# XiaokunSun/SemanticHuman

Measured on AMD Instinct MI355X. Metric: training meshes/sec at 6890 verts, batch=64, higher is better.
Workload: dtype f32

## Files before the change

include/sh_kernels.h:

```cpp
#ifndef SH_KERNELS_H
#define SH_KERNELS_H

#include <stddef.h>
#include <stdint.h>

#ifdef __cplusplus
extern "C" {
#endif

typedef void* sh_stream_t;

#if defined(__GNUC__)
#define SH_API __attribute__((visibility("default")))
#else
#define SH_API
#endif

enum sh_status {
    SH_OK = 0,
    SH_ERR_INVALID_ARG = -1,
    SH_ERR_UNSUPPORTED = -2,
    SH_ERR_WORKSPACE = -3,
    SH_ERR_LAUNCH = -4
};
// ... 64 lines not shown
                       float* dpre, int64_t dp_sv, int64_t dp_sb, int B, int R, int C, int act, int zero_row, int n_layers,
                       const float* const* weight, float* const* weight_t, const int* S, const int* Cin, const int* Cout,
                       sh_stream_t stream);

SH_API int sh_spmm(const int32_t* rowptr, const int32_t* col, const float* val,
            const float* x, int64_t x_sv, int64_t x_sb,
            float* y, int64_t y_sv, int64_t y_sb,
            const float* yprev, int64_t yp_sv, int64_t yp_sb, int act_prev, int zero_row,
            int B, int rows, int C, sh_stream_t stream);

typedef struct sh_csr_ref { const int32_t* rowptr; const int32_t* col; const float* val; } sh_csr_ref;
typedef struct sh_stack_step {
    int kind;
    int param;
    const int32_t* table;
    const int32_t* table_t;
    int R, S, n_in, cin, cout, act, zero_row;
    int n1, n2;
    sh_csr_ref sum1, sum2;
    sh_csr_ref m, mt;
    int m_rows, m_cols;
    int extend;
    const int32_t* rag_rows;
    const int32_t* rag_pos;
    int rag_L;
    const int32_t* fg_rows; const uint32_t* fg_pos; const int32_t* fg_out; int fg_n, fg_L;
    const int32_t* bg_rows; const uint32_t* bg_pos; const int32_t* bg_out; int bg_n, bg_L;
} sh_stack_step;

enum sh_stack_form {
    SH_FORM_FWD_P3 = 1,
    SH_FORM_FWD_GRP = 2,
    SH_FORM_FWD_IMG = 4,
    SH_FORM_FWD_IMG_ONLY = 8,
    SH_FORM_BWD_GIMG = 16,
    SH_FORM_BWD_THIN = 32,
    SH_FORM_BWD_P3 = 64,
    SH_FORM_BWD_RAG = 128,
    SH_FORM_BWD_GRP = 256,
    SH_FORM_BWD_RIDE = 512,
    SH_FORM_BWD_PRESUM_IMG = 1024,
    SH_FORM_BWD_P3W = 2048,
    SH_FORM_BWD_YIMG = 4096,
    SH_FORM_BWD_IN_IMG_ONLY = 8192,
    SH_FORM_BWD_GRAD_IMG_ONLY = 16384
};
SH_API int sh_stack_plan_f32(int n_steps, const sh_stack_step* steps, int c0, int B, int x_layout, int mma_mode, int keep_fp32,
                             int need_x_grad, int* forms);

SH_API int sh_stack_forward(int n_steps, const sh_stack_step* steps, const float* x, int x_layout, int rows0, int c0, int B,
                            const float* const* weights, const float* const* biases, float* const* outs, int out_layout,
                            int mma_mode, void* const* planes, const void* const* wfrag3, int keep_fp32, sh_stream_t stream);

SH_API int sh_stack_backward(int n_steps, const sh_stack_step* steps, const float* x, int x_layout, int rows0, int c0, int B,
                             const float* const* acts, const float* g, int out_layout, const float* const* weights,
                             float* const* gin, float* dpre_last, float* const* weight_t, void* const* workspace,
                             const size_t* workspace_bytes, float* const* dW, float* const* dbias, int need_x_grad,
                             int mma_mode, void* const* gin_planes, void* dpre_last_planes, const void* const* wfrag3_t,
                             const void* const* in_planes, int acts_fp32, sh_stream_t stream);

SH_API size_t sh_linear_workspace(int M, int N, int K);
SH_API int sh_linear_fwd(const float* x, const float* weight, const float* bias, float* y, int M, int N, int K,
                  void* workspace, size_t workspace_bytes, int mma_mode, sh_stream_t stream);
SH_API int sh_linear_bwd_data(const float* dy, const float* weight, float* dx, int M, int N, int K,
                       void* workspace, size_t workspace_bytes, int mma_mode, sh_stream_t stream);
SH_API int sh_linear_bwd_wgt(const float* dy, const float* x, float* dW, float* dbias, int M, int N, int K,
                      void* workspace, size_t workspace_bytes, int mma_mode, sh_stream_t stream);
SH_API int sh_linear_bwd_wgt_adam_ok(int M, int N, int K);
SH_API int sh_linear_bwd_wgt_adam(const void* dy, int dy_dtype, const void* x, int x_dtype, float* weight, void* weight_bf16, float* exp_avg,
                           float* exp_avg_sq, const float* step, const float* lr, double beta1, double beta2, double eps,
                           double weight_decay, float* dbias, int M, int N, int K, int mma_mode, sh_stream_t stream);

SH_API int sh_grouped_linear_fwd(int G, const float* x, int64_t x_rs, const int64_t* x_off, const float* const* w,
                          const float* const* bias, float* y, int64_t y_rs, const int64_t* y_off, int M,
                          const int* N, const int* K, sh_stream_t stream);
SH_API int sh_grouped_linear_bwd_data(int G, const float* dy, int64_t y_rs, const int64_t* y_off, const float* const* w,
                               float* dx, int64_t x_rs, const int64_t* x_off, int M, const int* N, const int* K,
                               sh_stream_t stream);
SH_API int sh_grouped_linear_bwd_wgt(int G, const float* dy, int64_t y_rs, const int64_t* y_off, const float* x,
                              int64_t x_rs, const int64_t* x_off, float* const* dW, float* const* dbias, int M,
                              const int* N, const int* K, sh_stream_t stream);

SH_API size_t sh_reduce_workspace(void);

SH_API int sh_l1_loss_fwd(const float* a, const float* b, int64_t n, float* loss, void* workspace, sh_stream_t stream);
SH_API int sh_l1_loss_bwd(const float* a, const float* b, int64_t n, const float* gscale, float* grad_b, sh_stream_t stream);

SH_API int sh_vertex_l2(const float* a, const float* b, int B, int N1, int N, float scale, float* out,
                 void* workspace, sh_stream_t stream);

SH_API int sh_edge_ratio_loss_fwd(const float* x_hat, const float* x, const int32_t* faces, int B, int N1, int F,
                           float* loss, void* workspace, sh_stream_t stream);
SH_API int sh_edge_ratio_loss_bwd(const float* x_hat, const float* x, const int32_t* faces,
                           const int32_t* vptr, const int32_t* vcorner, int B, int N1, int F,
                           const float* gscale, float* grad, sh_stream_t stream);

SH_API size_t sh_recon_loss_workspace(void);
SH_API int sh_recon_loss_fwd(const float* x_hat, const float* x, const int32_t* faces, int B, int N1, int F, float edge_w,
                      float* total, float* parts, void* workspace, sh_stream_t stream);
SH_API int sh_recon_loss_bwd(const float* x_hat, const float* x, const int32_t* vptr, const int32_t* vnbr, int B, int N1, int F,
                      float edge_w, const float* gscale, float* grad, sh_stream_t stream);

SH_API int sh_part_pairdist_tile_rows(void);
SH_API int sh_part_pairdist_loss_fwd(const float* x_rec, const float* x_gt, const float* bone, const float* scale,
                              const int32_t* part_ptr, const int32_t* part_vert, const int32_t* tile_ptr,
                              const int32_t* flags, const float* w_part, int B, int N1, int P, int T, int max_part,
                              int w_mode, float w_threshold, int relat, float* loss, float* part_sum, float* part_cnt,
                              void* workspace, size_t workspace_bytes, sh_stream_t stream);
SH_API int sh_part_pairdist_loss_bwd(const float* x_rec, const float* x_gt, const float* bone, const float* scale,
                              const int32_t* part_ptr, const int32_t* part_vert, const int32_t* tile_ptr,
                              const int32_t* flags, const float* w_part, int B, int N1, int P, int T, int max_part,
                              int w_mode, float w_threshold, int relat, const float* part_cnt, const float* gscale,
                              float* grad, sh_stream_t stream);
SH_API int sh_part_pairdist_loss_fwd_grad(const float* x_rec, const float* x_gt, const float* bone, const float* scale,
                                   const int32_t* part_ptr, const int32_t* part_vert, const int32_t* tile_ptr, const int32_t* flags,
                                   const float* w_part, int B, int N1, int P, int T, int max_part, int w_mode, float w_threshold,
                                   int relat, float* loss, float* part_sum, float* part_cnt, float* grad_raw, void* workspace,
                                   size_t workspace_bytes, sh_stream_t stream);
SH_API int sh_part_pairdist_loss_bwd_scale(const float* grad_raw, const int32_t* part_ptr, const int32_t* part_vert,
                                   const float* w_part, const float* part_cnt, const float* gscale, int B, int N1, int P,
                                   int n_part_verts, float* grad, sh_stream_t stream);

SH_API int sh_measure_girth(const float* v, int64_t v_sb, const int32_t* ring_ptr, const int32_t* ring_a,
                     const int32_t* ring_b, const float* ring_f, int B, int P, float* girth, sh_stream_t stream);
SH_API int sh_bone_length(const float* kps, const int32_t* bones, int B, int K, int P, float* length, sh_stream_t stream);
SH_API int sh_measure_girth_bwd(const float* v, int64_t v_sb, const int32_t* ring_ptr, const int32_t* ring_a, const int32_t* ring_b,
                                const float* ring_f, const int32_t* pt_ring, const int32_t* vt_ptr, const int32_t* vt_pt,
                                const float* vt_w, int n_vt, const float* g_girth, int B, int P, int rows, float* g_v, sh_stream_t stream);
SH_API int sh_bone_length_bwd(const float* kps, const int32_t* bones, const int32_t* jt_ptr, const int32_t* jt_bone, const float* jt_w,
                              int n_jt, const float* g_len, int B, int K, int P, float* g_kps, sh_stream_t stream);
SH_API int sh_joint_regress_bwd(const float* g_kps, const float* J, int B, int N, int K, int rows, float* g_x, sh_stream_t stream);

SH_API int sh_nearest_points_chunks(int B, int nq, int nt);
SH_API size_t sh_nearest_points_workspace(int B, int nq, int nt, int chunks);
SH_API int sh_nearest_points(const float* q, int64_t q_sb, int nq, const int32_t* q_count, const float* t, int64_t t_sb, int nt,
                             const int32_t* t_count, const uint8_t* t_mask, int64_t mask_sb, int B, int chunks, int32_t* idx,
                             float* d2, void* workspace, size_t workspace_bytes, sh_stream_t stream);
SH_API int sh_chamfer_fwd(const float* d2_sm, int M, const int32_t* s_count, const float* d2_ms, int rows, int n,
                          const uint8_t* v_mask, int64_t mask_sb, float tau2, float w_ms, int B, float* loss, int32_t* counts,
                          sh_stream_t stream);
SH_API int sh_chamfer_bwd(const float* x, int64_t x_sb, int rows, int n, const float* s, int64_t s_sb, int M, const int32_t* s_count,
                          const int32_t* idx_sm, const float* d2_sm, const int32_t* idx_ms, const float* d2_ms, const uint8_t* v_mask,
                          int64_t mask_sb, const int32_t* counts, float tau2, float w_ms, const float* gL, int B, float* g_x,
                          sh_stream_t stream);

#define SH_SURFACE_MARGIN (1.0f + 0x1p-10f)
SH_API int sh_nearest_surface_chunks(int B, int nq, int nF);
SH_API size_t sh_nearest_surface_workspace(int B, int nq, int nF, int chunks);
SH_API int sh_nearest_surface(const float* q, int64_t q_sb, int nq, const int32_t* q_count, const float* x, int64_t x_sb, int n,
                              const int32_t* faces, int nF, const uint8_t* v_mask, int64_t mask_sb, const float* bound, int B,
                              int chunks, int cull, int32_t* face, float* d2, float* uv, uint64_t* stats, void* workspace,
                              size_t workspace_bytes, sh_stream_t stream);
SH_API int sh_chamfer_surface_bwd(const float* x, int64_t x_sb, int rows, int n, const float* s, int64_t s_sb, int M,
                                  const int32_t* s_count, const int32_t* faces, int nF, const int32_t* face, const float* d2,
                                  const float* uv, const int32_t* idx_ms, const float* d2_ms, const uint8_t* v_mask, int64_t mask_sb,
                                  const int32_t* counts, float tau2, float w_ms, const float* gL, int B, float* g_x,
                                  sh_stream_t stream);

enum sh_align_mode { SH_ALIGN_TRANSLATION = 0, SH_ALIGN_RIGID = 1, SH_ALIGN_SIMILARITY = 2 };
#define SH_ALIGN_RANGE 2048
#define SH_ALIGN_PARTIAL 19
#define SH_ALIGN_MOMENTS 20
#define SH_ALIGN_JACOBI_SWEEPS 12
SH_API int sh_align_ranges(int M, int n, float w_ms);
SH_API size_t sh_align_partials_bytes(int B, int M, int n, float w_ms);
SH_API int sh_align_moments(const float* s, int64_t s_sb, int M, const int32_t* s_count, const float* x, int64_t x_sb, int rows, int n,
                            const uint8_t* v_mask, int64_t mask_sb, const int32_t* idx_sm, const float* d2_sm, const int32_t* idx_ms,
                            const float* d2_ms, float tau2, float w_ms, int B, double* partials, size_t partials_bytes,
                            sh_stream_t stream);
SH_API int sh_align_solve(const double* partials, int M, int n, const int32_t* s_count, float w_ms, int mode, int B,
                          const float* pose_in, const float* scale_in, float* pose_out, float* scale_out, float* inc, double* mom,
                          sh_stream_t stream);
SH_API int sh_transform_points(const float* src, int64_t src_sb, int M, const int32_t* count, const float* pose, int B, float* dst,
                               sh_stream_t stream);

enum sh_norm_flags {
    SH_NORM_ZEROMEAN = 1, SH_NORM_ZEROROOT = 2, SH_NORM_ONELENGTH = 4, SH_NORM_SMALL = 8, SH_NORM_GASS = 16, SH_NORM_NORMAL = 32
};
SH_API int sh_dataset_normalize(const float* raw, float* out, int n, int N, int dummy_rows, unsigned flags,
                         const float* j_root, const float* mean, const float* stdv, const float* center,
                         const float* scale, sh_stream_t stream);
SH_API int sh_gather_meshes(const float* src, int64_t row_elems, const int64_t* idx, int b, float* out, sh_stream_t stream);

SH_API int sh_adam_step(int n_tensors, float* const* params, const float* const* grads, float* const* exp_avg,
                 float* const* exp_avg_sq, float* const* steps, const int64_t* numel, const float* lr,
                 double beta1, double beta2, double eps, double weight_decay, sh_stream_t stream);
SH_API int sh_adam_bump(int n_tensors, float* const* steps, sh_stream_t stream);

SH_API int sh_joint_regress(const float* x, int64_t x_bs, const float* J, int B, int N, int K, float* kps, sh_stream_t stream);
SH_API int sh_joint_l1_loss_fwd(const float* x, int64_t x_bs, const float* J, const int32_t* keep, const float* target, int B,
                                int N, int K, int Kk, float* kps, float* loss, sh_stream_t stream);
SH_API int sh_joint_l1_loss_bwd(const float* kps, const int32_t* keep, const float* target, const float* J, int B, int N1, int N,
                                int K, int Kk, const float* gscale, float* grad, sh_stream_t stream);
SH_API int sh_part_volume_loss_fwd(const float* x_rec, const float* x_gt, int64_t x_bs, const int32_t* faces,
                                   const int32_t* pf_ptr, const int32_t* pf, int B, int P, float* vol, float* loss,
                                   sh_stream_t stream);
SH_API int sh_part_volume_loss_bwd(const float* x_rec, int64_t x_bs, const int32_t* faces, const int32_t* face_slot,
                                   const int32_t* vptr, const int32_t* vcorner, const float* vol, int B, int P, int N1,
                                   const float* gscale, float* grad, sh_stream_t stream);
SH_API int sh_zpart_reg(const float* z, const float* measure, const int32_t* part_idx, const int32_t* measure_idx, int B, int P,
                        int L, int M, int n, int relat, float* loss, float* dz, const float* gscale, sh_stream_t stream);
SH_API int sh_kps2skl(const float* kps, int B, int J, const int32_t* i0, const int32_t* i1, const int32_t* i2, int n_bones, int mode,
                      float* out, sh_stream_t stream);
SH_API int sh_skl2kps(const float* skl, int B, int n_bones, int mode, const int32_t* head, const int32_t* tail, int n_joints,
                      const int32_t* keep, int n_keep, float* out, sh_stream_t stream);
SH_API int sh_weighted_sum(int n, const float* const* terms, const float* weights, float* out, const float* gscale, float* grads,
                           sh_stream_t stream);

enum sh_dtype { SH_DTYPE_F32 = 0, SH_DTYPE_BF16 = 1 };

SH_API size_t sh_conv_wfrag_bytes(int S, int Cg, int Nout);
SH_API int sh_conv_wfrag_prep_multi(int n_layers, const float* const* weight, void* const* wfrag, const int* S,
                                    const int* Cin, const int* Cout, const int* transpose, sh_stream_t stream);

SH_API int sh_spiral_conv_fwd_bf16(const void* x, int x_dtype, int64_t x_sv, int64_t x_sb, const int32_t* table,
                                   const void* wfrag, const float* bias, void* y, int y_dtype, int64_t y_sv, int64_t y_sb,
                                   int B, int R, int S, int Cin, int Cout, int act, int zero_row, sh_stream_t stream);
SH_API int sh_spiral_conv_bwd_data_bf16(const void* dpre, int dp_dtype, int64_t dp_sv, int64_t dp_sb,
                                        const int32_t* table_t, const void* wfrag_t, void* dx, int dx_dtype,
                                        int64_t dx_sv, int64_t dx_sb, const void* yprev, int64_t yp_sv, int64_t yp_sb,
                                        int act_prev, int zero_row, int B, int n_in, int S, int Cin, int Cout,
                                        sh_stream_t stream);

SH_API int sh_spiral_conv_bwd_wgt_thin_ok(int B, int n_in, int S, int Cin, int Cout, int path_dtype);
SH_API int sh_spiral_conv_bwd_wgt_thin(const float* dpre_ext, int64_t dp_sv, int64_t dp_sb, const void* x, int x_dtype, int64_t x_sv,
                                int64_t x_sb, const int32_t* table_t, void* workspace, size_t workspace_bytes,
                                const float* weight, void* dx, int64_t dx_sv, int64_t dx_sb, void* dx_planes, int act_prev,
                                int zero_prev, int B, int R, int n_in, int S, int Cin, int Cout, int path_dtype, sh_stream_t stream);

SH_API size_t sh_spiral_conv_bwd_wgt_workspace_bf16(int B, int R, int S, int Cin, int Cout);
SH_API int sh_spiral_conv_bwd_wgt_bf16(const void* dpre, int dp_dtype, int64_t dp_sv, int64_t dp_sb, const void* x, int x_dtype,
                                       int64_t x_sv, int64_t x_sb, const int32_t* table, void* workspace,
                                       size_t workspace_bytes, int B, int R, int S, int Cin, int Cout, sh_stream_t stream);
SH_API int sh_spiral_conv_bwd_wgt_reduce_multi_bf16(int n_layers, const void* const* workspaces, float* const* dW,
                                                    float* const* dbias, const int* B, const int* R, const int* S,
                                                    const int* Cin, const int* Cout, sh_stream_t stream);

SH_API size_t sh_linear_workspace_bf16(int M, int N, int K);
SH_API int sh_cast_f32_to_bf16(const float* src, void* dst, int64_t n, sh_stream_t stream);
SH_API int sh_linear_fwd_bf16(const void* x, int x_dtype, const void* weight_bf16, const float* bias, void* y, int y_dtype,
// ... 92 lines not shown
```

semantichuman_amd/_lib.py:

```python
from __future__ import annotations

import ctypes
import os
from ctypes import c_char_p, c_float, c_int, c_int64, c_size_t, c_void_p

_HERE = os.path.dirname(os.path.abspath(__file__))
LIB_PATH = os.environ.get("SH_KERNEL_LIB") or os.path.join(_HERE, "lib", "libsh_kernels.so")

ACT_IDS = {"identity": 0, "relu": 1, "elu": 2, "leaky_relu": 3, "sigmoid": 4, "tanh": 5}

_P, _I, _L = c_void_p, c_int, c_int64
SIGNATURES = {
    "sh_version": (c_int, []),
    "sh_last_error": (c_char_p, []),
    "sh_build_id": (c_char_p, []),
    "sh_clock_probe": (c_int, [_P, _I, _I, _P]),
    "sh_profile_enable": (c_int, [_I]),
    "sh_profile_count": (c_int, []),
    "sh_profile_get": (c_int, [_I, c_char_p, _I, ctypes.POINTER(c_float)]),
    "sh_spiral_conv_fwd": (c_int, [_P, _L, _L, _P, _P, _P, _P, _L, _L, _I, _I, _I, _I, _I, _I, _I, _I, _P]),
    "sh_spiral_conv_bwd_data": (c_int, [_P, _L, _L, _P, _P, _P, _L, _L, _P, _L, _L, _I, _I, _I, _I, _I, _I, _I, _I, _P]),
    "sh_spiral_conv_bwd_data_z": (c_int, [_P, _L, _L, _I, _P, _P, _P, _L, _L, _P, _L, _L, _I, _I, _I, _I, _I, _I, _I, _I, _P]),
    "sh_weight_transpose": (c_int, [_P, _P, _I, _I, _I, _P]),
    "sh_spiral_conv_bwd_wgt_workspace": (c_size_t, [_I, _I, _I, _I, _I]),
    "sh_spiral_conv_bwd_wgt": (c_int, [_P, _L, _L, _P, _L, _L, _P, _P, _P, _P, c_size_t, _I, _I, _I, _I, _I, _I, _P]),
    "sh_spiral_conv_bwd_wgt_presum": (c_int, [_P, _L, _L, _P, _L, _L, _P, _P, _P, _P, c_size_t, _P, _P, _P, _P, _P, _I, _I, _I, _I, _I, _I, _I, _P]),
    "sh_spiral_conv_bwd_wgt_reduce_multi": (c_int, [_I, _P, _P, _P, _P, _P, _P, _P, _P, _P]),
    "sh_weight_transpose_multi": (c_int, [_I, _P, _P, _P, _P, _P, _P]),
    "sh_act_backward": (c_int, [_P, _L, _L, _P, _L, _L, _P, _L, _L, _I, _I, _I, _I, _I, _P]),
    "sh_act_backward_tr": (c_int, [_P, _L, _L, _P, _L, _L, _P, _L, _L, _I, _I, _I, _I, _I, _I, _P, _P, _P, _P, _P, _P]),
    "sh_spmm": (c_int, [_P, _P, _P, _P, _L, _L, _P, _L, _L, _P, _L, _L, _I, _I, _I, _I, _I, _P]),
    "sh_stack_plan_f32": (c_int, [_I, _P, _I, _I, _I, _I, _I, _I, _P]),
    "sh_stack_forward": (c_int, [_I, _P, _P, _I, _I, _I, _I, _P, _P, _P, _I, _I, _P, _P, _I, _P]),
    "sh_stack_backward": (c_int, [_I, _P, _P, _I, _I, _I, _I, _P, _P, _I, _P, _P, _P, _P, _P, _P, _P, _P, _I, _I, _P, _P, _P, _P, _I, _P]),
    "sh_linear_workspace": (c_size_t, [_I, _I, _I]),
    "sh_linear_fwd": (c_int, [_P, _P, _P, _P, _I, _I, _I, _P, c_size_t, _I, _P]),
    "sh_linear_bwd_data": (c_int, [_P, _P, _P, _I, _I, _I, _P, c_size_t, _I, _P]),
    "sh_linear_bwd_wgt": (c_int, [_P, _P, _P, _P, _I, _I, _I, _P, c_size_t, _I, _P]),
    "sh_linear_bwd_wgt_adam_ok": (c_int, [_I, _I, _I]),
    "sh_linear_bwd_wgt_adam": (c_int, [_P, _I, _P, _I] + [_P] * 6 + [ctypes.c_double] * 4 + [_P, _I, _I, _I, _I, _P]),
    "sh_adam_bump": (c_int, [_I, _P, _P]),
    "sh_grouped_linear_fwd": (c_int, [_I, _P, _L, _P, _P, _P, _P, _L, _P, _I, _P, _P, _P]),
    "sh_grouped_linear_bwd_data": (c_int, [_I, _P, _L, _P, _P, _P, _L, _P, _I, _P, _P, _P]),
    "sh_grouped_linear_bwd_wgt": (c_int, [_I, _P, _L, _P, _P, _L, _P, _P, _P, _I, _P, _P, _P]),
    "sh_reduce_workspace": (c_size_t, []),
    "sh_l1_loss_fwd": (c_int, [_P, _P, _L, _P, _P, _P]),
    "sh_l1_loss_bwd": (c_int, [_P, _P, _L, _P, _P, _P]),
    "sh_vertex_l2": (c_int, [_P, _P, _I, _I, _I, c_float, _P, _P, _P]),
    "sh_edge_ratio_loss_fwd": (c_int, [_P, _P, _P, _I, _I, _I, _P, _P, _P]),
    "sh_edge_ratio_loss_bwd": (c_int, [_P, _P, _P, _P, _P, _I, _I, _I, _P, _P, _P]),
    "sh_spiral_conv_bwd_wgt_thin_ok": (c_int, [_I, _I, _I, _I, _I, _I]),
    "sh_spiral_conv_bwd_wgt_thin": (c_int, [_P, _L, _L, _P, _I, _L, _L, _P, _P, c_size_t, _P, _P, _L, _L, _P, _I, _I, _I, _I, _I, _I, _I, _I, _I, _P]),
    "sh_recon_loss_workspace": (c_size_t, []),
    "sh_recon_loss_fwd": (c_int, [_P, _P, _P, _I, _I, _I, c_float, _P, _P, _P, _P]),
    "sh_recon_loss_bwd": (c_int, [_P, _P, _P, _P, _I, _I, _I, c_float, _P, _P, _P]),
    "sh_part_pairdist_tile_rows": (c_int, []),
    "sh_part_pairdist_loss_fwd": (c_int, [_P] * 9 + [_I] * 6 + [c_float, _I, _P, _P, _P, _P, c_size_t, _P]),
    "sh_part_pairdist_loss_bwd": (c_int, [_P] * 9 + [_I] * 6 + [c_float, _I, _P, _P, _P, _P]),
    "sh_part_pairdist_loss_fwd_grad": (c_int, [_P] * 9 + [_I] * 6 + [c_float, _I, _P, _P, _P, _P, _P, c_size_t, _P]),
    "sh_part_pairdist_loss_bwd_scale": (c_int, [_P] * 6 + [_I] * 4 + [_P, _P]),
    "sh_measure_girth": (c_int, [_P, _L, _P, _P, _P, _P, _I, _I, _P, _P]),
    "sh_bone_length": (c_int, [_P, _P, _I, _I, _I, _P, _P]),
    "sh_measure_girth_bwd": (c_int, [_P, _L, _P, _P, _P, _P, _P, _P, _P, _P, _I, _P, _I, _I, _I, _P, _P]),
    "sh_bone_length_bwd": (c_int, [_P, _P, _P, _P, _P, _I, _P, _I, _I, _I, _P, _P]),
    "sh_joint_regress_bwd": (c_int, [_P, _P, _I, _I, _I, _I, _P, _P]),
    "sh_nearest_points_chunks": (c_int, [_I, _I, _I]),
    "sh_nearest_points_workspace": (c_size_t, [_I, _I, _I, _I]),
    "sh_nearest_points": (c_int, [_P, _L, _I, _P, _P, _L, _I, _P, _P, _L, _I, _I, _P, _P, _P, c_size_t, _P]),
    "sh_chamfer_fwd": (c_int, [_P, _I, _P, _P, _I, _I, _P, _L, c_float, c_float, _I, _P, _P, _P]),
    "sh_chamfer_bwd": (c_int, [_P, _L, _I, _I, _P, _L, _I, _P, _P, _P, _P, _P, _P, _L, _P, c_float, c_float, _P, _I, _P, _P]),
    "sh_nearest_surface_chunks": (c_int, [_I, _I, _I]),
    "sh_nearest_surface_workspace": (c_size_t, [_I, _I, _I, _I]),
    "sh_nearest_surface": (c_int, [_P, _L, _I, _P, _P, _L, _I, _P, _I, _P, _L, _P, _I, _I, _I, _P, _P, _P, _P, _P, c_size_t, _P]),
    "sh_chamfer_surface_bwd": (c_int, [_P, _L, _I, _I, _P, _L, _I, _P, _P, _I, _P, _P, _P, _P, _P, _P, _L, _P, c_float, c_float, _P, _I, _P, _P]),
    "sh_align_ranges": (c_int, [_I, _I, c_float]),
    "sh_align_partials_bytes": (c_size_t, [_I, _I, _I, c_float]),
    "sh_align_moments": (c_int, [_P, _L, _I, _P, _P, _L, _I, _I, _P, _L, _P, _P, _P, _P, c_float, c_float, _I, _P, c_size_t, _P]),
    "sh_align_solve": (c_int, [_P, _I, _I, _P, c_float, _I, _I, _P, _P, _P, _P, _P, _P, _P]),
    "sh_transform_points": (c_int, [_P, _L, _I, _P, _P, _I, _P, _P]),
    "sh_dataset_normalize": (c_int, [_P, _P, _I, _I, _I, ctypes.c_uint, _P, _P, _P, _P, _P, _P]),
    "sh_gather_meshes": (c_int, [_P, _L, _P, _I, _P, _P]),
    "sh_adam_step": (c_int, [_I, _P, _P, _P, _P, _P, _P, _P] + [ctypes.c_double] * 4 + [_P]),
    "sh_joint_regress": (c_int, [_P, _L, _P, _I, _I, _I, _P, _P]),
    "sh_joint_l1_loss_fwd": (c_int, [_P, _L, _P, _P, _P, _I, _I, _I, _I, _P, _P, _P]),
    "sh_joint_l1_loss_bwd": (c_int, [_P, _P, _P, _P, _I, _I, _I, _I, _I, _P, _P, _P]),
    "sh_part_volume_loss_fwd": (c_int, [_P, _P, _L, _P, _P, _P, _I, _I, _P, _P, _P]),
    "sh_part_volume_loss_bwd": (c_int, [_P, _L, _P, _P, _P, _P, _P, _I, _I, _I, _P, _P, _P]),
    "sh_zpart_reg": (c_int, [_P, _P, _P, _P, _I, _I, _I, _I, _I, _I, _P, _P, _P, _P]),
    "sh_kps2skl": (c_int, [_P, _I, _I, _P, _P, _P, _I, _I, _P, _P]),
    "sh_skl2kps": (c_int, [_P, _I, _I, _I, _P, _P, _I, _P, _I, _P, _P]),
    "sh_weighted_sum": (c_int, [_I, _P, _P, _P, _P, _P, _P]),
    "sh_conv_wfrag_bytes": (c_size_t, [_I, _I, _I]),
    "sh_conv_wfrag_prep_multi": (c_int, [_I, _P, _P, _P, _P, _P, _P, _P]),
    "sh_spiral_conv_fwd_bf16": (c_int, [_P, _I, _L, _L, _P, _P, _P, _P, _I, _L, _L, _I, _I, _I, _I, _I, _I, _I, _P]),
# ... 162 lines not shown
```

semantichuman_amd/csrc/adam.hip:

```cpp
#include "sh_bf16.h"
#include "sh_adam.h"

#include <math.h>

namespace {

constexpr int AT = 60;
constexpr int ACH = 4096;
constexpr int ANT = 256;

struct AdamArgs {
    float* p[AT];
    const float* g[AT];
    float* m[AT];
    float* v[AT];
    float* step[AT];
    __bf16* shadow[AT];
    long n[AT];
    int blk_start[AT + 1];
    int nt, nontemporal;
    const float* lr;
    double beta1, beta2;
    float w1, b2, w2, eps, wd;
};

__global__ __launch_bounds__(ANT) void adam_kernel(const AdamArgs a) {
    __shared__ float sh[2];
    int t = 0;
    while (t + 1 < a.nt && (int)blockIdx.x >= a.blk_start[t + 1]) ++t;
    const long base = (long)((int)blockIdx.x - a.blk_start[t]) * ACH;
    const long n = a.n[t];
    if (threadIdx.x == 0) {
        sh_adam_coeffs(a.beta1, a.beta2, a.step[t][0], a.lr[0], sh[0], sh[1]);
    }
    __syncthreads();
    const float step_size = sh[0], bc2_sqrt = sh[1];
    float* __restrict__ p = a.p[t];
    const float* __restrict__ g = a.g[t];
    float* __restrict__ m = a.m[t];
    float* __restrict__ v = a.v[t];
    __bf16* __restrict__ sw = a.shadow[t];
    const bool vec = ((reinterpret_cast<uintptr_t>(p) | reinterpret_cast<uintptr_t>(g) | reinterpret_cast<uintptr_t>(m) |
                       reinterpret_cast<uintptr_t>(v)) & 15) == 0;
    if (vec && base + ACH <= n) {
#pragma unroll
        for (int i = 0; i < ACH / (4 * ANT); ++i) {
            const long o = base + 4L * (threadIdx.x + i * ANT);
            f32x4 pp, mm, vv, gg;
            if (a.nontemporal) {
                pp = __builtin_nontemporal_load(reinterpret_cast<const f32x4*>(p + o));
                mm = __builtin_nontemporal_load(reinterpret_cast<const f32x4*>(m + o));
                vv = __builtin_nontemporal_load(reinterpret_cast<const f32x4*>(v + o));
                gg = __builtin_nontemporal_load(reinterpret_cast<const f32x4*>(g + o));
            } else {
                pp = *reinterpret_cast<f32x4*>(p + o); mm = *reinterpret_cast<f32x4*>(m + o); vv = *reinterpret_cast<f32x4*>(v + o);
                gg = *reinterpret_cast<const f32x4*>(g + o);
            }
#pragma unroll
            for (int j = 0; j < 4; ++j) {
                float p1 = pp[j], m1 = mm[j], v1 = vv[j];
                adam_update(p1, gg[j], m1, v1, a.w1, a.b2, a.w2, a.eps, a.wd, step_size, bc2_sqrt);
                pp[j] = p1; mm[j] = m1; vv[j] = v1;
            }
            if (sw) *reinterpret_cast<bf16x4*>(sw + o) = sh_to_bf16x4(pp);
            if (a.nontemporal) {
                __builtin_nontemporal_store(pp, reinterpret_cast<f32x4*>(p + o));
                __builtin_nontemporal_store(mm, reinterpret_cast<f32x4*>(m + o));
                __builtin_nontemporal_store(vv, reinterpret_cast<f32x4*>(v + o));
            } else {
                *reinterpret_cast<f32x4*>(p + o) = pp;
                *reinterpret_cast<f32x4*>(m + o) = mm;
                *reinterpret_cast<f32x4*>(v + o) = vv;
            }
        }
    } else {
        constexpr int PER = ACH / ANT;
        float pp[PER], mm[PER], vv[PER], gg[PER];
#pragma unroll
        for (int i = 0; i < PER; ++i) {
            const long o = base + threadIdx.x + (long)i * ANT;
            const bool ok = o < n;
            pp[i] = ok ? p[o] : 0.f; mm[i] = ok ? m[o] : 0.f; vv[i] = ok ? v[o] : 0.f; gg[i] = ok ? g[o] : 0.f;
        }
#pragma unroll
        for (int i = 0; i < PER; ++i) {
            const long o = base + threadIdx.x + (long)i * ANT;
            if (o < n) {
                adam_update(pp[i], gg[i], mm[i], vv[i], a.w1, a.b2, a.w2, a.eps, a.wd, step_size, bc2_sqrt);
                p[o] = pp[i]; m[o] = mm[i]; v[o] = vv[i];
                if (sw) sw[o] = (__bf16)pp[i];
            }
        }
    }
}

__global__ void adam_bump_kernel(const AdamArgs a) {
    if ((int)threadIdx.x < a.nt) a.step[threadIdx.x][0] += 1.f;
}

}

extern "C" {

static int adam_impl(int n_tensors, float* const* params, const float* const* grads, float* const* exp_avg, float* const* exp_avg_sq,
                     float* const* steps, void* const* shadow, const int64_t* numel, const float* lr, double beta1, double beta2,
                     double eps, double weight_decay, sh_stream_t stream) {
    SH_REQUIRE(n_tensors >= 0, SH_ERR_INVALID_ARG, "sh_adam_step: negative tensor count");
    if (n_tensors == 0) return SH_OK;
    SH_REQUIRE(params && grads && exp_avg && exp_avg_sq && steps && numel && lr, SH_ERR_INVALID_ARG, "sh_adam_step: null pointer");
    SH_REQUIRE(beta1 >= 0 && beta1 < 1 && beta2 >= 0 && beta2 < 1 && eps >= 0 && weight_decay >= 0, SH_ERR_INVALID_ARG,
               "sh_adam_step: hyper-parameter out of range");
    hipStream_t st = static_cast<hipStream_t>(stream);
    static const int nontemporal = sh_env_int("SH_ADAM_NT", 1, 0, 1);
    for (int t0 = 0; t0 < n_tensors; t0 += AT) {
        AdamArgs a{};
        a.nt = n_tensors - t0 < AT ? n_tensors - t0 : AT;
        long blocks = 0;
        for (int i = 0; i < a.nt; ++i) {
            const int k = t0 + i;
            SH_REQUIRE(steps[k] && numel[k] >= 0 && (numel[k] == 0 || (params[k] && grads[k] && exp_avg[k] && exp_avg_sq[k])), SH_ERR_INVALID_ARG,
                       "sh_adam_step: tensor %d has a null pointer or a negative element count", k);
            a.p[i] = params[k]; a.g[i] = grads[k]; a.m[i] = exp_avg[k]; a.v[i] = exp_avg_sq[k]; a.step[i] = steps[k];
            a.shadow[i] = shadow ? static_cast<__bf16*>(shadow[k]) : nullptr;
            SH_REQUIRE(!a.shadow[i] || (reinterpret_cast<uintptr_t>(a.shadow[i]) & 7) == 0, SH_ERR_INVALID_ARG, "sh_adam_step_bf16: shadow %d misaligned", k);
            a.n[i] = numel[k];
            a.blk_start[i] = (int)blocks;
            blocks += (numel[k] + ACH - 1) / ACH;
            SH_REQUIRE(blocks < (1L << 31), SH_ERR_UNSUPPORTED, "sh_adam_step: too many elements in one launch");
        }
        a.blk_start[a.nt] = (int)blocks;
        a.nontemporal = nontemporal;
        a.lr = lr; a.beta1 = beta1; a.beta2 = beta2;
        a.w1 = (float)(1.0 - beta1); a.b2 = (float)beta2; a.w2 = (float)(1.0 - beta2); a.eps = (float)eps; a.wd = (float)weight_decay;
        if (blocks > 0) {
            long numel_sum = 0;
            for (int i = 0; i < a.nt; ++i) numel_sum += a.n[i];
            ShProfScope ps(st, "adam_kernel|tensors=%d blocks=%ld numel=%ld", a.nt, blocks, numel_sum);
            SH_LAUNCH_PS(ps, adam_kernel, dim3((unsigned)blocks), dim3(ANT), 0, st, a);
        }
        hipLaunchKernelGGL(adam_bump_kernel, dim3(1), dim3(64), 0, st, a);
        SH_CHECK_LAUNCH("adam_step");
    }
    return SH_OK;
}

int sh_adam_bump(int n_tensors, float* const* steps, sh_stream_t stream) {
    SH_REQUIRE(n_tensors >= 0, SH_ERR_INVALID_ARG, "sh_adam_bump: negative tensor count");
    if (n_tensors == 0) return SH_OK;
    SH_REQUIRE(steps, SH_ERR_INVALID_ARG, "sh_adam_bump: null pointer");
    hipStream_t st = static_cast<hipStream_t>(stream);
    for (int t0 = 0; t0 < n_tensors; t0 += AT) {
        AdamArgs a{};
        a.nt = n_tensors - t0 < AT ? n_tensors - t0 : AT;
        for (int i = 0; i < a.nt; ++i) {
            SH_REQUIRE(steps[t0 + i], SH_ERR_INVALID_ARG, "sh_adam_bump: tensor %d has a null step pointer", t0 + i);
            a.step[i] = steps[t0 + i];
        }
        hipLaunchKernelGGL(adam_bump_kernel, dim3(1), dim3(64), 0, st, a);
        SH_CHECK_LAUNCH("adam_bump");
    }
    return SH_OK;
}

int sh_adam_step(int n_tensors, float* const* params, const float* const* grads, float* const* exp_avg, float* const* exp_avg_sq,
                 float* const* steps, const int64_t* numel, const float* lr, double beta1, double beta2, double eps,
                 double weight_decay, sh_stream_t stream) {
    return adam_impl(n_tensors, params, grads, exp_avg, exp_avg_sq, steps, nullptr, numel, lr, beta1, beta2, eps, weight_decay, stream);
}

int sh_adam_step_bf16(int n_tensors, float* const* params, const float* const* grads, float* const* exp_avg, float* const* exp_avg_sq,
                      float* const* steps, void* const* shadow_bf16, const int64_t* numel, const float* lr, double beta1, double beta2,
                      double eps, double weight_decay, sh_stream_t stream) {
    return adam_impl(n_tensors, params, grads, exp_avg, exp_avg_sq, steps, shadow_bf16, numel, lr, beta1, beta2, eps, weight_decay, stream);
}

}
```

semantichuman_amd/csrc/linear.hip:

```cpp
#include "sh_bf16.h"
#include "sh_adam.h"

#include <type_traits>

namespace {

constexpr int LT = 64;
constexpr int LK = 32;
constexpr int LTHREADS = 256;

struct SGParams {
    const float* a; long a_sm, a_sr;
    const float* b; long b_sn, b_sr;
    float* c; long c_sm, c_sn;
    const float* bias;
    float* slab;
    int M, N, R;
    int rchunk, nsplit, n_mtiles, n_ntiles;
    int a_mode, b_mode;
};

__device__ __forceinline__ void sg_load(const float* base, long s_row, long s_r, int mode, int row0, int nrows, int r0, int rend,
                                        int tid, f32x4 (&reg)[2], unsigned& mask) {
    mask = 0;
// ... 155 lines not shown
        for (; k + 48 < nsplit; k += 64) {
            const float a = slab[(long)k * mn + i], b = slab[(long)(k + 16) * mn + i];
            const float d = slab[(long)(k + 32) * mn + i], e = slab[(long)(k + 48) * mn + i];
            s += (a + b) + (d + e);
        }
        for (; k < nsplit; k += 16) s += slab[(long)k * mn + i];
    }
    red[ry][ox] = s;
    __syncthreads();
    if (ry == 0 && i < mn) {
        float t = 0.f;
#pragma unroll
        for (int k = 0; k < 16; ++k) t += red[k][ox];
        c[i] = t + (bias ? bias[i % N] : 0.f);
    }
}

__global__ __launch_bounds__(256) void colsum_kernel(const float* __restrict__ x, int M, int N, float* __restrict__ out) {
    const int n = blockIdx.x * 256 + threadIdx.x;
    if (n >= N) return;
    float s = 0.f;
    for (int m = 0; m < M; ++m) s += x[(long)m * N + n];
    out[n] = s;
}

#ifndef SH_LS_DEPTH
#define SH_LS_DEPTH 2
#endif
constexpr int LS_DEPTH = SH_LS_DEPTH;

template <int J, int D, class F>
__device__ __forceinline__ bool ls_run_steps(int s, int n, F&& f) {
    f(s + J, std::integral_constant<int, J>{});
    if constexpr (J + 1 < D) {
        if (s + J + 1 >= n) return true;
        return ls_run_steps<J + 1, D>(s, n, f);
    }
    return false;
}

struct LSParams {
    const float* a;
    const float* w;
    const float* bias;
    float* out;
    float* slab;
    float* dbias;
    int M, N, K;
    int range, nsplit, groups;
    float* am;
    float* av;
    __bf16* shadow;
    ShAdamHyper ad;
};

template <int MT>
__global__ __launch_bounds__(LTHREADS) void linear_fwd_stream_kernel(const LSParams p) {
    const int lane = threadIdx.x & 63, wave = sh_wave_id();
    const int item = sh_xcd_remap(blockIdx.x, gridDim.x) * 4 + wave;
    if (item >= p.groups * p.nsplit) return;
    const int ng = item % p.groups, sp = item / p.groups;
    const int n0 = ng * 64, k_begin = sp * p.range;
    const int nsteps = (min(p.K, k_begin + p.range) - k_begin) >> 4;
    const int lr = lane & 15, kq = lane >> 4;
    const float* xrow[MT];
    const float* wrow[4];
#pragma unroll
    for (int mt = 0; mt < MT; ++mt) xrow[mt] = p.a + (long)min(16 * mt + lr, p.M - 1) * p.K + k_begin + 4 * kq;
#pragma unroll
    for (int nt = 0; nt < 4; ++nt) wrow[nt] = p.w + (long)(n0 + 16 * nt + lr) * p.K + k_begin + 4 * kq;
    f32x4 xa[LS_DEPTH][MT], wb[LS_DEPTH][4], acc[MT][4];
#pragma unroll
    for (int mt = 0; mt < MT; ++mt)
#pragma unroll
        for (int nt = 0; nt < 4; ++nt) acc[mt][nt] = (f32x4){0.f, 0.f, 0.f, 0.f};
    auto load = [&](int s, f32x4 (&x4)[MT], f32x4 (&w4)[4]) {
        const int off = 16 * (s < nsteps ? s : nsteps - 1);
#pragma unroll
        for (int mt = 0; mt < MT; ++mt) x4[mt] = *reinterpret_cast<const f32x4*>(xrow[mt] + off);
#pragma unroll
        for (int nt = 0; nt < 4; ++nt) w4[nt] = __builtin_nontemporal_load(reinterpret_cast<const f32x4*>(wrow[nt] + off));
    };
    auto mma = [&](const f32x4 (&x4)[MT], const f32x4 (&w4)[4]) {
#pragma unroll
        for (int t = 0; t < 4; ++t)
#pragma unroll
            for (int nt = 0; nt < 4; ++nt)
#pragma unroll
                for (int mt = 0; mt < MT; ++mt) acc[mt][nt] = __builtin_amdgcn_mfma_f32_16x16x4f32(w4[nt][t], x4[mt][t], acc[mt][nt], 0, 0, 0);
    };
    auto step = [&](int s, auto J) {
        constexpr int j = decltype(J)::value;
        load(s + LS_DEPTH - 1, xa[(j + LS_DEPTH - 1) % LS_DEPTH], wb[(j + LS_DEPTH - 1) % LS_DEPTH]);
        __builtin_amdgcn_sched_barrier(0);
        mma(xa[j], wb[j]);
    };
    if (nsteps > 0) {
#pragma unroll
        for (int d = 0; d < LS_DEPTH - 1; ++d) load(d, xa[d], wb[d]);
        for (int s = 0; s < nsteps; s += LS_DEPTH)
            if (ls_run_steps<0, LS_DEPTH>(s, nsteps, step)) break;
    }
#pragma unroll
    for (int mt = 0; mt < MT; ++mt) {
        const int m = 16 * mt + lr;
        if (m >= p.M) continue;
#pragma unroll
// ... 178 lines not shown
        }
    }
}

template <int MT>
__global__ __launch_bounds__(LTHREADS) void linear_bwd_data_stream_kernel(const LSParams p) {
    const int lane = threadIdx.x & 63, wave = sh_wave_id();
    const int item = sh_xcd_remap(blockIdx.x, gridDim.x) * 4 + wave;
    if (item >= p.groups * p.nsplit) return;
    const int kg = item % p.groups, sp = item / p.groups;
    const int k0 = kg * 64, n_begin = sp * p.range;
    const int nsteps = (min(p.N, n_begin + p.range) - n_begin) >> 4;
    const int la = lane & 15, rr = lane >> 4;
    const float* drow[MT];
#pragma unroll
    for (int mt = 0; mt < MT; ++mt) drow[mt] = p.a + (long)min(16 * mt + la, p.M - 1) * p.N + n_begin + 4 * rr;
    const float* wbase = p.w + (long)(n_begin + 4 * rr) * p.K + k0 + 4 * la;
    f32x4 dq[LS_DEPTH][MT], wq[LS_DEPTH][4], acc[4][MT];
#pragma unroll
    for (int t = 0; t < 4; ++t)
#pragma unroll
        for (int mt = 0; mt < MT; ++mt) acc[t][mt] = (f32x4){0.f, 0.f, 0.f, 0.f};
    auto load = [&](int s, f32x4 (&d4)[MT], f32x4 (&w4)[4]) {
        const int nb = 16 * (s < nsteps ? s : nsteps - 1);
#pragma unroll
        for (int mt = 0; mt < MT; ++mt) d4[mt] = *reinterpret_cast<const f32x4*>(drow[mt] + nb);
#pragma unroll
        for (int e = 0; e < 4; ++e) w4[e] = __builtin_nontemporal_load(reinterpret_cast<const f32x4*>(wbase + (long)(nb + e) * p.K));
    };
    auto mma = [&](const f32x4 (&d4)[MT], const f32x4 (&w4)[4]) {
#pragma unroll
        for (int e = 0; e < 4; ++e)
#pragma unroll
            for (int t = 0; t < 4; ++t)
#pragma unroll
                for (int mt = 0; mt < MT; ++mt) acc[t][mt] = __builtin_amdgcn_mfma_f32_16x16x4f32(w4[e][t], d4[mt][e], acc[t][mt], 0, 0, 0);
    };
    auto step = [&](int s, auto J) {
        constexpr int j = decltype(J)::value;
        load(s + LS_DEPTH - 1, dq[(j + LS_DEPTH - 1) % LS_DEPTH], wq[(j + LS_DEPTH - 1) % LS_DEPTH]);
        __builtin_amdgcn_sched_barrier(0);
        mma(dq[j], wq[j]);
    };
    if (nsteps > 0) {
#pragma unroll
        for (int d = 0; d < LS_DEPTH - 1; ++d) load(d, dq[d], wq[d]);
        for (int s = 0; s < nsteps; s += LS_DEPTH)
            if (ls_run_steps<0, LS_DEPTH>(s, nsteps, step)) break;
    }
#pragma unroll
    for (int mt = 0; mt < MT; ++mt) {
        const int m = 16 * mt + la;
        if (m >= p.M) continue;
        float* dst = (p.nsplit > 1 ? p.slab + ((long)sp * p.M + m) * p.K : p.out + (long)m * p.K) + k0 + 16 * rr;
#pragma unroll
        for (int jj = 0; jj < 4; ++jj)
            *reinterpret_cast<f32x4*>(dst + 4 * jj) = (f32x4){acc[0][mt][jj], acc[1][mt][jj], acc[2][mt][jj], acc[3][mt][jj]};
    }
}

template <int MT>
__global__ __launch_bounds__(LTHREADS) void linear_bwd_data_x3_kernel(const LSParams p) {
    const int lane = threadIdx.x & 63, wave = sh_wave_id();
    const int item = sh_xcd_remap(blockIdx.x, gridDim.x) * 4 + wave;
    if (item >= p.groups * p.nsplit) return;
    const int kg = item % p.groups, sp = item / p.groups;
    const int k0 = kg * 64, n_begin = sp * p.range;
    const int nsteps = (min(p.N, n_begin + p.range) - n_begin) >> 5;
    const int la = lane & 15, rr = lane >> 4;
    const float* drow[MT];
#pragma unroll
    for (int mt = 0; mt < MT; ++mt) drow[mt] = p.a + (long)min(16 * mt + la, p.M - 1) * p.N + n_begin + 4 * rr;
    const float* wbase = p.w + (long)(n_begin + 4 * rr) * p.K + k0 + 4 * la;
    f32x4 dq[2][MT][2], wq[2][8], acc[4][MT];
#pragma unroll
    for (int t = 0; t < 4; ++t)
#pragma unroll
        for (int mt = 0; mt < MT; ++mt) acc[t][mt] = (f32x4){0.f, 0.f, 0.f, 0.f};
    auto load = [&](int s, f32x4 (&d4)[MT][2], f32x4 (&w4)[8]) {
        const int nb = 32 * (s < nsteps ? s : nsteps - 1);
#pragma unroll
        for (int mt = 0; mt < MT; ++mt) {
            d4[mt][0] = *reinterpret_cast<const f32x4*>(drow[mt] + nb);
            d4[mt][1] = *reinterpret_cast<const f32x4*>(drow[mt] + nb + 16);
        }
#pragma unroll
        for (int j = 0; j < 8; ++j)
            w4[j] = __builtin_nontemporal_load(reinterpret_cast<const f32x4*>(wbase + (long)(nb + (j & 3) + 16 * (j >> 2)) * p.K));
    };
    auto mma = [&](const f32x4 (&d4)[MT][2], const f32x4 (&w4)[8]) {
        LinX3 ds[MT];
#pragma unroll
        for (int mt = 0; mt < MT; ++mt) ds[mt] = lin_split(d4[mt][0], d4[mt][1]);
#pragma unroll
        for (int t = 0; t < 4; ++t) {
            const LinX3 ws = lin_split((f32x4){w4[0][t], w4[1][t], w4[2][t], w4[3][t]}, (f32x4){w4[4][t], w4[5][t], w4[6][t], w4[7][t]});
#pragma unroll
            for (int mt = 0; mt < MT; ++mt) acc[t][mt] = lin_x3_mma(ws.h, ws.m, ws.l, ds[mt].h, ds[mt].m, ds[mt].l, acc[t][mt]);
        }
    };
    if (nsteps > 0) {
        load(0, dq[0], wq[0]);
        for (int s = 0; s < nsteps; s += 2) {
            load(s + 1, dq[1], wq[1]);
            __builtin_amdgcn_sched_barrier(0);
            mma(dq[0], wq[0]);
            if (s + 1 >= nsteps) break;
            load(s + 2, dq[0], wq[0]);
            __builtin_amdgcn_sched_barrier(0);
            mma(dq[1], wq[1]);
        }
    }
#pragma unroll
    for (int mt = 0; mt < MT; ++mt) {
        const int m = 16 * mt + la;
        if (m >= p.M) continue;
        float* dst = (p.nsplit > 1 ? p.slab + ((long)sp * p.M + m) * p.K : p.out + (long)m * p.K) + k0 + 16 * rr;
#pragma unroll
        for (int jj = 0; jj < 4; ++jj)
            *reinterpret_cast<f32x4*>(dst + 4 * jj) = (f32x4){acc[0][mt][jj], acc[1][mt][jj], acc[2][mt][jj], acc[3][mt][jj]};
    }
}

__global__ __launch_bounds__(LTHREADS) void linear_bwd_wgt_stream_kernel(const LSParams p) {
    const int lane = threadIdx.x & 63, wave = sh_wave_id();
    const int item = sh_xcd_remap(blockIdx.x, gridDim.x) * 4 + wave;
    const int ktiles = p.K >> 6;
    if (item >= (p.N >> 6) * ktiles) return;
    const int kt = item % ktiles, ntile = item / ktiles;
    const int n0 = ntile * 64, k0 = kt * 64;
    const int la = lane & 15, rr = lane >> 4;
    const int nsteps = (p.M + 3) >> 2;
    f32x4 acc[4][4];
#pragma unroll
    for (int a = 0; a < 4; ++a)
#pragma unroll
        for (int b = 0; b < 4; ++b) acc[a][b] = (f32x4){0.f, 0.f, 0.f, 0.f};
    f32x4 dq[4], xq[4];
    auto load = [&](int s, f32x4& d4, f32x4& x4) {
        s = s < nsteps ? s : nsteps - 1;
        const int m = 4 * s + rr;
        const int mc = m < p.M ? m : p.M - 1;
        d4 = *reinterpret_cast<const f32x4*>(p.a + (long)mc * p.N + n0 + 4 * la);
        x4 = *reinterpret_cast<const f32x4*>(p.w + (long)mc * p.K + k0 + 4 * la);
        if (m >= p.M) d4 = (f32x4){0.f, 0.f, 0.f, 0.f};
    };
    const bool own_bias = kt == 0 && p.dbias != nullptr;
    f32x4 bsum = {0.f, 0.f, 0.f, 0.f};
    auto mma = [&](const f32x4& d4, const f32x4& x4) {
#pragma unroll
        for (int tn = 0; tn < 4; ++tn)
#pragma unroll
            for (int tk = 0; tk < 4; ++tk) acc[tn][tk] = __builtin_amdgcn_mfma_f32_16x16x4f32(d4[tn], x4[tk], acc[tn][tk], 0, 0, 0);
        if (own_bias) bsum += d4;
    };
    load(0, dq[0], xq[0]); load(1, dq[1], xq[1]); load(2, dq[2], xq[2]);
    for (int s = 0; s < nsteps; s += 4) {
        load(s + 3, dq[3], xq[3]); __builtin_amdgcn_sched_barrier(0); mma(dq[0], xq[0]);
        if (s + 1 >= nsteps) break;
        load(s + 4, dq[0], xq[0]); __builtin_amdgcn_sched_barrier(0); mma(dq[1], xq[1]);
        if (s + 2 >= nsteps) break;
        load(s + 5, dq[1], xq[1]); __builtin_amdgcn_sched_barrier(0); mma(dq[2], xq[2]);
        if (s + 3 >= nsteps) break;
        load(s + 6, dq[2], xq[2]); __builtin_amdgcn_sched_barrier(0); mma(dq[3], xq[3]);
    }
    if (own_bias) {
#pragma unroll
        for (int j = 0; j < 4; ++j) {
            float v = bsum[j];
// ... 357 lines not shown
                if (hipFuncSetAttribute(reinterpret_cast<const void*>(linear_fwd_wide_x3_kernel), hipFuncAttributeMaxDynamicSharedMemorySize,
                                        160 * 1024) != hipSuccess) {
                    (void)hipGetLastError();
                    sh_set_error("linear_fwd: cannot raise the dynamic LDS limit to %zu bytes", smem);
                    return SH_ERR_LAUNCH;
                }
                attr_set = true;
            }
            LSParams s{};
            s.a = x; s.w = weight; s.bias = bias; s.out = y; s.M = M; s.N = N; s.K = K;
            ShProfScope ps(st, "linear_fwd_wide_x3_kernel|M=%d N=%d K=%d", M, N, K);
            SH_LAUNCH_PS(ps, linear_fwd_wide_x3_kernel, dim3(N / 64), dim3(LFW_WAVES * 64), smem, st, s);
            SH_CHECK_LAUNCH("linear_fwd_wide");
            return SH_OK;
        }
    }
    {
        const bool x3 = lin_x3(mma_mode) && K % 32 == 0 && (N / 64) % 4 == 0;
        static const int chunk_on = sh_env_int("SH_LIN_CHUNKED", 1, 0, 1);
        const LSPlan pl = plan_stream(M, N, K, x3 ? 32 : 16, chunk_on && M > 64);
        if (pl.ok && aligned16(x, weight, y) && (!bias || (reinterpret_cast<uintptr_t>(bias) & 15) == 0)) {
            LSParams s{};
            s.a = x; s.w = weight; s.bias = bias; s.out = y; s.M = M; s.N = N; s.K = K;
            return run_stream<true>(s, pl, N, workspace, workspace_bytes, static_cast<hipStream_t>(stream), "linear_fwd", x3);
        }
    }
    SGParams p{};
    p.a = x; p.a_sm = K; p.a_sr = 1;
    p.b = weight; p.b_sn = K; p.b_sr = 1;
    p.c = y; p.c_sm = N; p.c_sn = 1; p.bias = bias;
    p.M = M; p.N = N; p.R = K;
    return run_gemm(p, workspace, workspace_bytes, static_cast<hipStream_t>(stream), "linear_fwd");
}

int sh_linear_bwd_data(const float* dy, const float* weight, float* dx, int M, int N, int K, void* workspace,
                       size_t workspace_bytes, int mma_mode, sh_stream_t stream) {
    SH_REQUIRE(dy && weight && dx && M > 0 && N > 0 && K > 0, SH_ERR_INVALID_ARG, "sh_linear_bwd_data: bad argument");
    SH_REQUIRE(sh_mma_mode_valid(mma_mode), SH_ERR_INVALID_ARG, "sh_linear_bwd_data: unknown mma_mode %d", mma_mode);
    {
        const bool x3 = lin_x3(mma_mode) && N % 32 == 0;
        const LSPlan pl = plan_stream(M, K, N, x3 ? 32 : 16);
        if (pl.ok && aligned16(dy, weight, dx)) {
            LSParams s{};
            s.a = dy; s.w = weight; s.bias = nullptr; s.out = dx; s.M = M; s.N = N; s.K = K;
            return run_stream<false>(s, pl, K, workspace, workspace_bytes, static_cast<hipStream_t>(stream), "linear_bwd_data", x3);
        }
    }
    SGParams p{};
    p.a = dy; p.a_sm = N; p.a_sr = 1;
    p.b = weight; p.b_sn = 1; p.b_sr = K;
    p.c = dx; p.c_sm = K; p.c_sn = 1; p.bias = nullptr;
    p.M = M; p.N = K; p.R = N;
    return run_gemm(p, workspace, workspace_bytes, static_cast<hipStream_t>(stream), "linear_bwd_data");
}

static bool wgt_dma_attr() {
    static bool attr_set = false;
    if (!attr_set) {
        for (const void* k : {reinterpret_cast<const void*>(linear_bwd_wgt_dma_kernel<false>), reinterpret_cast<const void*>(linear_bwd_wgt_dma_kernel<true>),
                              reinterpret_cast<const void*>(linear_bwd_wgt_dma_kernel<false, true>), reinterpret_cast<const void*>(linear_bwd_wgt_dma_kernel<true, true>),
                              reinterpret_cast<const void*>(linear_bwd_wgt_dma_kernel<false, true, true, false>),
                              reinterpret_cast<const void*>(linear_bwd_wgt_dma_kernel<false, true, false, true>),
                              reinterpret_cast<const void*>(linear_bwd_wgt_dma_kernel<false, true, true, true>)})
            if (hipFuncSetAttribute(k, hipFuncAttributeMaxDynamicSharedMemorySize, 160 * 1024) != hipSuccess) {
                (void)hipGetLastError();
                sh_set_error("linear_bwd_wgt: cannot raise the dynamic LDS limit to %d bytes", LWD_LDS);
                return false;
            }
        attr_set = true;
    }
    return true;
}

int sh_linear_bwd_wgt(const float* dy, const float* x, float* dW, float* dbias, int M, int N, int K, void* workspace,
                      size_t workspace_bytes, int mma_mode, sh_stream_t stream) {
    SH_REQUIRE(dy && x && dW && M > 0 && N > 0 && K > 0, SH_ERR_INVALID_ARG, "sh_linear_bwd_wgt: bad argument");
    SH_REQUIRE(sh_mma_mode_valid(mma_mode), SH_ERR_INVALID_ARG, "sh_linear_bwd_wgt: unknown mma_mode %d", mma_mode);
    hipStream_t st = static_cast<hipStream_t>(stream);
    static const int stream_on = sh_env_int("SH_LIN_STREAM", 1, 0, 1);
    if (stream_on && M <= 64 && N % 64 == 0 && K % 64 == 0 && aligned16(dy, x, dW)) {
        LSParams s{};
        s.a = dy; s.w = x; s.out = dW; s.M = M; s.N = N; s.K = K;
        s.dbias = (dbias && (reinterpret_cast<uintptr_t>(dbias) & 15) == 0) ? dbias : nullptr;
        const int items = (N / 64) * (K / 64);
        static const int dma_on = sh_env_int("SH_LIN_WGT_DMA", 1, 0, 1);
        if (dma_on) {
            if (!wgt_dma_attr()) return SH_ERR_LAUNCH;
            const int wgs = (N / 64) * sh_cdiv(K / 64, 4);
            if (lin_x3(mma_mode)) {
                ShProfScope ps(st, "linear_bwd_wgt_x3_kernel|M=%d N=%d K=%d", M, N, K);
                SH_LAUNCH_PS(ps, linear_bwd_wgt_dma_kernel<true>, dim3(wgs), dim3(LTHREADS), LWD_LDS, st, s);
            } else {
                ShProfScope ps(st, "linear_bwd_wgt_dma_kernel|M=%d N=%d K=%d", M, N, K);
                SH_LAUNCH_PS(ps, linear_bwd_wgt_dma_kernel<false>, dim3(wgs), dim3(LTHREADS), LWD_LDS, st, s);
            }
        } else {
            ShProfScope ps(st, "linear_bwd_wgt_stream_kernel|M=%d N=%d K=%d", M, N, K);
            SH_LAUNCH_PS(ps, linear_bwd_wgt_stream_kernel, dim3(sh_cdiv(items, 4)), dim3(LTHREADS), 0, st, s);
        }
        if (dbias && !s.dbias) hipLaunchKernelGGL(colsum_kernel, dim3((unsigned)sh_cdiv(N, 256)), dim3(256), 0, st, dy, M, N, dbias);
        SH_CHECK_LAUNCH("linear_bwd_wgt");
        return SH_OK;
    }
    SGParams p{};
    p.a = dy; p.a_sm = 1; p.a_sr = N;
    p.b = x; p.b_sn = 1; p.b_sr = K;
// ... 60 lines not shown
```

semantichuman_amd/csrc/spmm_loss.hip:

```cpp
#include "sh_bf16.h"

namespace {

constexpr int RED_BLOCKS = 2048;

template <bool VEC, bool P3 = false>
__global__ __launch_bounds__(256) void spmm_kernel(const int* __restrict__ rowptr, const int* __restrict__ col,
                                                   const float* __restrict__ val, const float* __restrict__ x, long x_sv, long x_sb,
                                                   float* __restrict__ y, long y_sv, long y_sb, const float* __restrict__ yprev,
                                                   long yp_sv, long yp_sb, int act, int zero_row, int B, int rows, int C,
                                                   char* __restrict__ img = nullptr, long img_vb = 0, long img_bgb = 0) {
    const int CW = VEC ? C >> 2 : C;
    const int per_row = B * CW;
    const int parts = (per_row + 255) >> 8;
    const long items = (long)rows * parts;
    for (long it = blockIdx.x; it < items; it += gridDim.x) {
        const int r = (int)(it / parts), part = (int)(it - (long)r * parts);
        const int e0 = rowptr[r], e1 = rowptr[r + 1];
        const bool zero = r == zero_row;
        for (int j = part * 256 + threadIdx.x; j < per_row && j < (part + 1) * 256; j += 256) {
            const int b = j / CW, cw = j - b * CW;
            const int co = VEC ? 4 * cw : cw;
            const long xo = (long)b * x_sb + co;
            const long yo = (long)r * y_sv + (long)b * y_sb + co;
// ... 189 lines not shown

__global__ void edge_loss_partial_kernel(const float* __restrict__ xh, const float* __restrict__ x, const int* __restrict__ faces,
                                         int B, int N1, int F, float* __restrict__ part) {
    __shared__ float red[16];
    float s = 0.f;
    const long n = (long)B * F;
    for (long i = (long)blockIdx.x * blockDim.x + threadIdx.x; i < n; i += (long)gridDim.x * blockDim.x) {
        const long bb = i / F;
        const int f = (int)(i - bb * F);
        const int ia = faces[3 * f], ib = faces[3 * f + 1], ic = faces[3 * f + 2];
        const float* ph = xh + bb * N1 * 3;
        const float* pg = x + bb * N1 * 3;
        s += fabsf(edge_len(ph, ia, ib) / (edge_len(pg, ia, ib) + 0.00001f) - 1.f);
        s += fabsf(edge_len(ph, ib, ic) / (edge_len(pg, ib, ic) + 0.00001f) - 1.f);
        s += fabsf(edge_len(ph, ia, ic) / (edge_len(pg, ia, ic) + 0.00001f) - 1.f);
    }
    const float t = block_sum(s, red);
    if (threadIdx.x == 0) part[blockIdx.x] = t;
}

__device__ __forceinline__ void edge_grad(const float* ph, const float* pg, int i, int j, float* g) {
    const float dx = ph[3 * i] - ph[3 * j], dy = ph[3 * i + 1] - ph[3 * j + 1], dz = ph[3 * i + 2] - ph[3 * j + 2];
    const float len = sqrtf(dx * dx + dy * dy + dz * dz);
    const float t = edge_len(pg, i, j) + 0.00001f;
    const float r = len / t - 1.f;
    const float sg = r > 0.f ? 1.f : (r < 0.f ? -1.f : 0.f);
    if (len > 0.f) {
        const float k = sg / (len * t);
        g[0] += k * dx; g[1] += k * dy; g[2] += k * dz;
    }
}

__global__ void edge_loss_bwd_kernel(const float* __restrict__ xh, const float* __restrict__ x, const int* __restrict__ faces,
                                     const int* __restrict__ vptr, const int* __restrict__ vcorner, int B, int N1, int F,
                                     const float* __restrict__ gscale, float* __restrict__ grad) {
    const float sc = gscale[0] / ((float)B * (float)F);
    const long n = (long)B * N1;
    for (long i = (long)blockIdx.x * blockDim.x + threadIdx.x; i < n; i += (long)gridDim.x * blockDim.x) {
        const long bb = i / N1;
        const int v = (int)(i - bb * N1);
        const float* ph = xh + bb * N1 * 3;
        const float* pg = x + bb * N1 * 3;
        float g[3] = {0.f, 0.f, 0.f};
        for (int e = vptr[v]; e < vptr[v + 1]; ++e) {
            const int c = vcorner[e], f = c / 3, kx = c - 3 * f;
            const int o1 = faces[3 * f + (kx + 1) % 3], o2 = faces[3 * f + (kx + 2) % 3];
            edge_grad(ph, pg, v, o1, g);
            edge_grad(ph, pg, v, o2, g);
        }
        grad[i * 3] = sc * g[0]; grad[i * 3 + 1] = sc * g[1]; grad[i * 3 + 2] = sc * g[2];
    }
}

__global__ void recon_partial_kernel(const float* __restrict__ xh, const float* __restrict__ x, const int* __restrict__ faces,
                                     int B, int N1, int F, float* __restrict__ part) {
    __shared__ float red[16];
    float s = 0.f;
    const long n = (long)B * N1 * 3;
    for (long i = (long)blockIdx.x * blockDim.x + threadIdx.x; i < n; i += (long)gridDim.x * blockDim.x) s += fabsf(x[i] - xh[i]);
    const float t1 = block_sum(s, red);
    if (threadIdx.x == 0) part[blockIdx.x] = t1;
    __syncthreads();
    s = 0.f;
    const long nf = (long)B * F;
    for (long i = (long)blockIdx.x * blockDim.x + threadIdx.x; i < nf; i += (long)gridDim.x * blockDim.x) {
        const long bb = i / F;
        const int f = (int)(i - bb * F);
        const I3 fc = *reinterpret_cast<const I3*>(faces + 3 * f);
        const float* ph = xh + bb * N1 * 3;
        const float* pg = x + bb * N1 * 3;
        const P3 ha = ld3(ph, fc.a), hb = ld3(ph, fc.b), hc = ld3(ph, fc.c), ga = ld3(pg, fc.a), gb = ld3(pg, fc.b), gc = ld3(pg, fc.c);
        s += fabsf(edge_len3(ha, hb) / (edge_len3(ga, gb) + 0.00001f) - 1.f);
        s += fabsf(edge_len3(hb, hc) / (edge_len3(gb, gc) + 0.00001f) - 1.f);
        s += fabsf(edge_len3(ha, hc) / (edge_len3(ga, gc) + 0.00001f) - 1.f);
    }
    const float t2 = block_sum(s, red);
    if (threadIdx.x == 0) part[RED_BLOCKS + blockIdx.x] = t2;
}

__global__ void recon_final_kernel(const float* __restrict__ part, int np, double scale1, double scale2, float w, float* __restrict__ total,
                                   float* __restrict__ parts) {
    __shared__ double red[2][256];
    double s1 = 0.0, s2 = 0.0;
    for (int i = threadIdx.x; i < np; i += 256) { s1 += (double)part[i]; s2 += (double)part[RED_BLOCKS + i]; }
    red[0][threadIdx.x] = s1; red[1][threadIdx.x] = s2;
    __syncthreads();
    for (int o = 128; o > 0; o >>= 1) {
        if ((int)threadIdx.x < o) { red[0][threadIdx.x] += red[0][threadIdx.x + o]; red[1][threadIdx.x] += red[1][threadIdx.x + o]; }
        __syncthreads();
    }
    if (threadIdx.x == 0) {
        const float rec = (float)(red[0][0] * scale1), edge = (float)(red[1][0] * scale2);
        total[0] = rec + w * edge; parts[0] = rec; parts[1] = edge;
    }
}

__global__ __launch_bounds__(256) void recon_bwd_kernel(const float* __restrict__ xh, const float* __restrict__ x, const int* __restrict__ vptr,
                                                        const int* __restrict__ vnbr, int B, int N1, int F, float w,
                                                        const float* __restrict__ gscale, float* __restrict__ grad) {
    const float g0 = gscale[0];
    const float s1 = g0 / ((float)B * (float)N1 * 3.f), s2 = g0 * w / ((float)B * (float)F);
    const long n = (long)B * N1;
    for (long i = (long)blockIdx.x * blockDim.x + threadIdx.x; i < n; i += (long)gridDim.x * blockDim.x) {
        const long bb = i / N1;
        const int v = (int)(i - bb * N1);
        const float* ph = xh + bb * N1 * 3;
        const float* pg = x + bb * N1 * 3;
        const int p0 = 2 * vptr[v], p1 = 2 * vptr[v + 1];
        const P3 hv = ld3(ph, v), gv = ld3(pg, v);
        float g[3] = {0.f, 0.f, 0.f};
        for (int e = p0; e < p1; e += 4) {
            int o[4];
            P3 ho[4], go[4];
#pragma unroll
            for (int k = 0; k < 4; ++k) o[k] = vnbr[e + k < p1 ? e + k : p1 - 1];
#pragma unroll
            for (int k = 0; k < 4; ++k) { ho[k] = ld3(ph, o[k]); go[k] = ld3(pg, o[k]); }
#pragma unroll
            for (int k = 0; k < 4; ++k)
                if (e + k < p1) edge_grad3(hv, gv, ho[k], go[k], g);
        }
        const float df[3] = {hv.x - gv.x, hv.y - gv.y, hv.z - gv.z};
        P3 o3;
        o3.x = s2 * g[0] + (df[0] > 0.f ? s1 : (df[0] < 0.f ? -s1 : 0.f));
        o3.y = s2 * g[1] + (df[1] > 0.f ? s1 : (df[1] < 0.f ? -s1 : 0.f));
        o3.z = s2 * g[2] + (df[2] > 0.f ? s1 : (df[2] < 0.f ? -s1 : 0.f));
        *reinterpret_cast<P3*>(grad + i * 3) = o3;
    }
}

inline int grid_for(long n, int per_block) {
    long g = (n + per_block - 1) / per_block;
    if (g < 1) g = 1;
    return (int)(g < 2048 ? g : 2048);
}

}

extern "C" {

int sh_spmm(const int32_t* rowptr, const int32_t* col, const float* val, const float* x, int64_t x_sv, int64_t x_sb, float* y,
            int64_t y_sv, int64_t y_sb, const float* yprev, int64_t yp_sv, int64_t yp_sb, int act_prev, int zero_row, int B,
            int rows, int C, sh_stream_t stream) {
    return sh_spmm_p3(rowptr, col, val, x, x_sv, x_sb, y, y_sv, y_sb, nullptr, yprev, yp_sv, yp_sb, act_prev, zero_row, B, rows, C, stream);
}

int sh_spmm_p3(const int32_t* rowptr, const int32_t* col, const float* val, const float* x, int64_t x_sv, int64_t x_sb, float* y,
               int64_t y_sv, int64_t y_sb, void* y_planes, const float* yprev, int64_t yp_sv, int64_t yp_sb, int act_prev, int zero_row,
               int B, int rows, int C, sh_stream_t stream) {
    SH_REQUIRE(rowptr && col && val && x && (y || y_planes), SH_ERR_INVALID_ARG, "sh_spmm: null pointer");
    SH_REQUIRE(B > 0 && rows > 0 && C > 0, SH_ERR_INVALID_ARG, "sh_spmm: non-positive size");
    SH_REQUIRE(act_prev >= SH_ACT_IDENTITY && act_prev <= SH_ACT_TANH, SH_ERR_INVALID_ARG, "sh_spmm: unknown activation %d", act_prev);
    const bool vec = (C % 4 == 0) && (x_sv % 4 == 0) && (x_sb % 4 == 0) && (y_sv % 4 == 0) && (y_sb % 4 == 0) &&
                     ((reinterpret_cast<uintptr_t>(x) | reinterpret_cast<uintptr_t>(y)) % 16 == 0) &&
                     (!yprev || (yp_sv % 4 == 0 && yp_sb % 4 == 0 && reinterpret_cast<uintptr_t>(yprev) % 16 == 0));
    static const int grid_cap = sh_env_int("SH_SPMM_GRID", 4096, 64, 1 << 20);
    const long items = (long)rows * (((long)B * (vec ? C / 4 : C) + 255) / 256);
    const int grid = (int)(items < grid_cap ? items : grid_cap);
    hipStream_t st = static_cast<hipStream_t>(stream);
    if (y_planes) {
        SH_REQUIRE(vec && y_sb == C && y_sv == (int64_t)B * C && sh_p3_bytes(1, B, C) && (reinterpret_cast<uintptr_t>(y_planes) & 15) == 0, SH_ERR_UNSUPPORTED,
                   "sh_spmm_p3: B=%d C=%d has no plane image (vertex-major y; B %% 16 == 0; C == 16 or C %% 32 == 0; 16-byte aligned tensors)", B, C);
        const long bgb = C == 16 ? 1536 : (long)(C / 32) * 3072;
        ShProfScope ps(st, "spmm_kernel<true, p3>|rows=%d B=%d C=%d f32=%d", rows, B, C, y ? 1 : 0);
        static const int x8_mode = sh_env_int("SH_SPMM_P3X8", 1, 0, 2);
        const bool x8 = x8_mode == 2 || (x8_mode == 1 && (C >= 128 || (C == 64 && B >= 256)));
        if (x8) {
            const long items8 = (long)rows * (((long)B * (C / 8) + 255) / 256);
            const int grid8 = (int)(items8 < grid_cap ? items8 : grid_cap);
            SH_LAUNCH_PS(ps, spmm_p3x8_kernel, dim3(grid8), dim3(256), 0, st, rowptr, col, val, x, x_sv, x_sb, y, y_sv, y_sb, yprev, yp_sv, yp_sb,
                         act_prev, zero_row, B, rows, C, static_cast<char*>(y_planes), bgb * (B / 16), bgb);
        } else
        SH_LAUNCH_PS(ps, (spmm_kernel<true, true>), dim3(grid), dim3(256), 0, st, rowptr, col, val, x, x_sv, x_sb, y, y_sv, y_sb,
                     yprev, yp_sv, yp_sb, act_prev, zero_row, B, rows, C, static_cast<char*>(y_planes), bgb * (B / 16), bgb);
        SH_CHECK_LAUNCH("spmm");
        return SH_OK;
    }
    ShProfScope ps(st, "spmm_kernel<%s>|rows=%d B=%d C=%d", vec ? "true" : "false", rows, B, C);
    if (vec)
        SH_LAUNCH_PS(ps, (spmm_kernel<true, false>), dim3(grid), dim3(256), 0, st, rowptr, col, val, x, x_sv, x_sb, y, y_sv, y_sb,
// ... 32 lines not shown
                 sh_stream_t stream) {
    SH_REQUIRE(a && b && out && workspace && B > 0 && N > 0 && N1 >= N, SH_ERR_INVALID_ARG, "sh_vertex_l2: bad argument");
    hipStream_t st = static_cast<hipStream_t>(stream);
    float* part = static_cast<float*>(workspace);
    const long n = (long)B * N;
    const int nb = grid_for(n, 1024) < RED_BLOCKS ? grid_for(n, 1024) : RED_BLOCKS;
    hipLaunchKernelGGL(vertex_l2_partial_kernel, dim3(nb), dim3(256), 0, st, a, b, B, N1, N, scale, part);
    hipLaunchKernelGGL(final_sum_kernel, dim3(1), dim3(256), 0, st, part, nb, 1.0 / (double)n, out);
    SH_CHECK_LAUNCH("vertex_l2");
    return SH_OK;
}

int sh_edge_ratio_loss_fwd(const float* x_hat, const float* x, const int32_t* faces, int B, int N1, int F, float* loss,
                           void* workspace, sh_stream_t stream) {
    SH_REQUIRE(x_hat && x && faces && loss && workspace && B > 0 && N1 > 0 && F > 0, SH_ERR_INVALID_ARG,
               "sh_edge_ratio_loss_fwd: bad argument");
    hipStream_t st = static_cast<hipStream_t>(stream);
    float* part = static_cast<float*>(workspace);
    const long n = (long)B * F;
    const int nb = grid_for(n, 1024) < RED_BLOCKS ? grid_for(n, 1024) : RED_BLOCKS;
    hipLaunchKernelGGL(edge_loss_partial_kernel, dim3(nb), dim3(256), 0, st, x_hat, x, faces, B, N1, F, part);
    hipLaunchKernelGGL(final_sum_kernel, dim3(1), dim3(256), 0, st, part, nb, 1.0 / (double)n, loss);
    SH_CHECK_LAUNCH("edge_ratio_loss_fwd");
    return SH_OK;
}

size_t sh_recon_loss_workspace(void) { return (size_t)2 * RED_BLOCKS * sizeof(float); }

int sh_recon_loss_fwd(const float* x_hat, const float* x, const int32_t* faces, int B, int N1, int F, float edge_w, float* total,
                      float* parts, void* workspace, sh_stream_t stream) {
    SH_REQUIRE(x_hat && x && faces && total && parts && workspace && B > 0 && N1 > 0 && F > 0, SH_ERR_INVALID_ARG,
               "sh_recon_loss_fwd: bad argument");
    hipStream_t st = static_cast<hipStream_t>(stream);
    float* part = static_cast<float*>(workspace);
    const long n = (long)B * N1 * 3;
    const int nb = grid_for(n, 1024) < RED_BLOCKS ? grid_for(n, 1024) : RED_BLOCKS;
    hipLaunchKernelGGL(recon_partial_kernel, dim3(nb), dim3(256), 0, st, x_hat, x, faces, B, N1, F, part);
    hipLaunchKernelGGL(recon_final_kernel, dim3(1), dim3(256), 0, st, part, nb, 1.0 / (double)n, 1.0 / ((double)B * F), edge_w, total, parts);
    SH_CHECK_LAUNCH("recon_loss_fwd");
    return SH_OK;
}

int sh_recon_loss_bwd(const float* x_hat, const float* x, const int32_t* vptr, const int32_t* vnbr, int B, int N1, int F, float edge_w,
                      const float* gscale, float* grad, sh_stream_t stream) {
    SH_REQUIRE(x_hat && x && vptr && vnbr && gscale && grad && B > 0 && N1 > 0 && F > 0, SH_ERR_INVALID_ARG,
               "sh_recon_loss_bwd: bad argument");
    const long n = (long)B * N1;
    hipLaunchKernelGGL(recon_bwd_kernel, dim3(grid_for(n, 256)), dim3(256), 0, static_cast<hipStream_t>(stream), x_hat, x, vptr, vnbr, B,
                       N1, F, edge_w, gscale, grad);
    SH_CHECK_LAUNCH("recon_loss_bwd");
    return SH_OK;
}

int sh_edge_ratio_loss_bwd(const float* x_hat, const float* x, const int32_t* faces, const int32_t* vptr, const int32_t* vcorner,
                           int B, int N1, int F, const float* gscale, float* grad, sh_stream_t stream) {
    SH_REQUIRE(x_hat && x && faces && vptr && vcorner && gscale && grad && B > 0 && N1 > 0 && F > 0, SH_ERR_INVALID_ARG,
               "sh_edge_ratio_loss_bwd: bad argument");
    const long n = (long)B * N1;
    hipLaunchKernelGGL(edge_loss_bwd_kernel, dim3(grid_for(n, 256)), dim3(256), 0, static_cast<hipStream_t>(stream), x_hat, x, faces,
                       vptr, vcorner, B, N1, F, gscale, grad);
    SH_CHECK_LAUNCH("edge_ratio_loss_bwd");
    return SH_OK;
}

}
```

semantichuman_amd/csrc/stack_exec.hip:

```cpp
#include "sh_common.h"

namespace {

struct Lay { long sv, sb; };
inline Lay lay(int layout, int rows, int B, int C) {
    return layout == 0 ? Lay{(long)B * C, (long)C} : Lay{(long)C, (long)rows * C};
}
inline int out_rows(const sh_stack_step& s) { return s.kind == 0 ? s.R : s.m_rows; }
inline bool is_last_step(int i, int n) { return i == n - 1; }
inline int in_rows(const sh_stack_step& s) { return s.kind == 0 ? s.n_in : s.m_cols; }

int check_tensor_sizes(int n, const sh_stack_step* st, int rows0, int c0, int B, const char* what) {
    long rows = rows0;
    int c = c0;
    for (int i = 0; i <= n; ++i) {
        long extra = 0;
        if (i > 0 && st[i - 1].kind == 0) extra = (long)st[i - 1].n1 + st[i - 1].n2;
        SH_REQUIRE((rows + extra) * (long)B * c < (1L << 32), SH_ERR_UNSUPPORTED,
                   "%s: the tensor %s step %d has %ld rows x %d batch entries x %d channels >= 2^32 elements - split the batch", what,
                   i < n ? "entering" : "leaving", i < n ? i : n - 1, rows + extra, B, c);
        if (i == n) break;
        rows = st[i].kind == 0 ? st[i].R : (st[i].extend ? (long)st[i].m_cols + st[i].m_rows : st[i].m_rows);
        if (st[i].kind == 0) c = st[i].cout;
    }
// ... 128 lines not shown
    SH_REQUIRE(sh_mma_mode_valid(mma_mode), SH_ERR_INVALID_ARG, "sh_stack_forward: unknown mma_mode %d", mma_mode);
    SH_REQUIRE(keep_fp32 >= 0 && keep_fp32 <= 2, SH_ERR_INVALID_ARG, "sh_stack_forward: keep_fp32 = %d (0, 1 or 2)", keep_fp32);
    Forms f[64];
    plan_f32(n_steps, steps, B, x_layout, mma_mode == SH_MMA_PLANES3 && planes && wfrag3, keep_fp32, false, f);
    for (int i = 0; i < n_steps; ++i) {
        SH_REQUIRE(outs[i], SH_ERR_INVALID_ARG, "sh_stack_forward: no output buffer for step %d", i);
        SH_REQUIRE(!f[i].f_img || planes[i], SH_ERR_INVALID_ARG, "sh_stack_forward: step %d writes the image of its output: planes[%d] is NULL", i, i);
        SH_REQUIRE(!f[i].f_p3 || wfrag3[i], SH_ERR_INVALID_ARG, "sh_stack_forward: step %d runs on planes: wfrag3[%d] is NULL", i, i);
    }
    const float* cur = x;
    Lay cl = lay(x_layout, rows0, B, c0);
    int c = c0;
    for (int i = 0; i < n_steps; ++i) {
        const sh_stack_step& s = steps[i];
        const Forms& q = f[i];
        const int co = s.kind == 0 ? s.cout : c;
        const Lay ol = lay(i == n_steps - 1 ? out_layout : 0, out_rows(s), B, co);
        void* img = q.f_img ? planes[i] : nullptr;
        if (s.kind == 0) {
            const float* bias = biases ? biases[s.param] : nullptr;
            float* y = q.f_img_only ? nullptr : outs[i];
            if (q.f_grp)
                rc = sh_spiral_conv_p3_grp(planes[i - 1], s.fg_rows, s.fg_pos, s.fg_out, s.fg_n, s.fg_L, wfrag3[i], bias, y, ol.sv, ol.sb, img, nullptr,
                                           0, 0, nullptr, s.act, s.zero_row, 0, B, s.R, s.S, s.cin, s.cout, stream);
            else if (q.f_p3)
                rc = sh_spiral_conv_fwd_p3(planes[i - 1], s.table, wfrag3[i], bias, y, ol.sv, ol.sb, img, B, s.R, s.S, s.cin, s.cout, s.act,
                                           s.zero_row, stream);
            else
                rc = sh_spiral_conv_fwd_img(cur, cl.sv, cl.sb, s.table, weights[s.param], bias, outs[i], ol.sv, ol.sb, img, B, s.R, s.S, s.cin,
                                            s.cout, s.act, s.zero_row, mma_mode, stream);
        } else if (s.extend) {
            SH_REQUIRE(i > 0 && !is_last_step(i, n_steps) && outs[i] == outs[i - 1] && cl.sb == c, SH_ERR_INVALID_ARG,
                       "sh_stack_forward: step %d appends to its input, which must be the vertex-major output buffer of step %d", i, i - 1);
            SH_REQUIRE(!img || planes[i] == planes[i - 1], SH_ERR_INVALID_ARG, "sh_stack_forward: step %d appends to its input: same image buffer", i);
            float* dst = q.f_img_only ? nullptr : outs[i] + (long)s.m_cols * cl.sv;
            rc = sh_spmm_p3(s.m.rowptr, s.m.col, s.m.val, cur, cl.sv, cl.sb, dst, cl.sv, cl.sb,
                            img ? static_cast<char*>(img) + sh_p3_bytes(s.m_cols, B, c) : nullptr, nullptr, 0, 0, 0, -1, B, s.m_rows, c, stream);
        } else {
            rc = sh_spmm_p3(s.m.rowptr, s.m.col, s.m.val, cur, cl.sv, cl.sb, q.f_img_only ? nullptr : outs[i], ol.sv, ol.sb, img, nullptr, 0, 0, 0,
                            -1, B, s.m_rows, c, stream);
        }
        if (rc != SH_OK) return rc;
        cur = outs[i]; cl = ol; c = co;
    }
    return SH_OK;
}

int sh_stack_backward(int n_steps, const sh_stack_step* steps, const float* x, int x_layout, int rows0, int c0, int B,
                      const float* const* acts, const float* g, int out_layout, const float* const* weights,
                      float* const* gin, float* dpre_last, float* const* weight_t, void* const* workspace,
                      const size_t* workspace_bytes, float* const* dW, float* const* dbias, int need_x_grad, int mma_mode,
                      void* const* gin_planes, void* dpre_last_planes, const void* const* wfrag3_t, const void* const* in_planes,
                      int acts_fp32, sh_stream_t stream) {
    int rc = check_steps(n_steps, steps, c0, "sh_stack_backward");
    if (rc != SH_OK) return rc;
    if (B > 0 && (rc = check_tensor_sizes(n_steps, steps, rows0, c0, B, "sh_stack_backward")) != SH_OK) return rc;
    SH_REQUIRE(x && acts && g && weights && gin && dW && B > 0, SH_ERR_INVALID_ARG, "sh_stack_backward: null pointer or empty batch");
    SH_REQUIRE(n_steps <= 64, SH_ERR_UNSUPPORTED, "sh_stack_backward: more than 64 steps");
    SH_REQUIRE(sh_mma_mode_valid(mma_mode), SH_ERR_INVALID_ARG, "sh_stack_backward: unknown mma_mode %d", mma_mode);
    const bool planes3 = mma_mode == SH_MMA_PLANES3 && gin_planes && wfrag3_t;
    SH_REQUIRE(acts_fp32 == 1 || (acts_fp32 == 2 && planes3 && in_planes), SH_ERR_INVALID_ARG,
               "sh_stack_backward: acts_fp32 = %d (1: every activation has its fp32 rows; 2, three-plane form with gin_planes, wfrag3_t and "
               "in_planes: the forward pass ran with keep_fp32 == 2)", acts_fp32);
    const int last = n_steps - 1;
    Forms f[64];
    plan_f32(n_steps, steps, B, x_layout, planes3, acts_fp32, need_x_grad != 0, f);
    for (int i = 0; i < n_steps; ++i) {
        SH_REQUIRE(!f[i].b_gimg || (wfrag3_t[i] && (i == last ? dpre_last_planes : gin_planes[i + 1])), SH_ERR_INVALID_ARG,
                   "sh_stack_backward: step %d runs backward-data on planes: wfrag3_t[%d] and the image buffer of its gradient (%s) are required",
                   i, i, i == last ? "dpre_last_planes" : "gin_planes[i + 1]");
        SH_REQUIRE(!in_planes || !(f[i].b_p3w || f[i].b_yimg) || in_planes[i], SH_ERR_INVALID_ARG,
                   "sh_stack_backward: step %d reads the image of its input: in_planes[%d] is NULL", i, i);
    }
    const Switches& sw = switches();
    int cin_of[64];
    {
        int c = c0;
        for (int i = 0; i < n_steps; ++i) { cin_of[i] = c; if (steps[i].kind == 0) c = steps[i].cout; }
    }
    const float* tr_w[32]; float* tr_wt[32]; int tr_S[32], tr_Ci[32], tr_Co[32];
    int n_tr = 0;
    for (int i = 0; i < n_steps; ++i) {
        if (steps[i].kind != 0 || !(i > 0 || need_x_grad) || (f[i].b_gimg && !f[i].b_thin)) continue;
        SH_REQUIRE(weight_t && weight_t[i], SH_ERR_INVALID_ARG, "sh_stack_backward: no weight_t buffer for step %d", i);
        SH_REQUIRE(n_tr < 32, SH_ERR_UNSUPPORTED, "sh_stack_backward: more than 32 conv steps");
        tr_w[n_tr] = weights[steps[i].param]; tr_wt[n_tr] = weight_t[i]; tr_S[n_tr] = steps[i].S; tr_Ci[n_tr] = steps[i].cin; tr_Co[n_tr] = steps[i].cout;
        ++n_tr;
    }
    if (n_tr && !(sw.tr_ride && steps[last].kind == 0)) {
        rc = sh_weight_transpose_multi(n_tr, tr_w, tr_wt, tr_S, tr_Ci, tr_Co, stream);
        if (rc != SH_OK) return rc;
        n_tr = 0;
    }
    const float* cur; Lay cl;
    void* cur_img = nullptr;
    bool cur_img_done = false;
    {
        const sh_stack_step& s = steps[last];
        if (s.kind == 0) {
            SH_REQUIRE(dpre_last, SH_ERR_INVALID_ARG, "sh_stack_backward: no dpre_last buffer");
            const Lay ol = lay(out_layout, s.R, B, s.cout), dl = lay(0, 0, B, s.cout);
            cur_img = f[last].b_gimg ? dpre_last_planes : nullptr;
            const bool img_in = cur_img && s.cout % 4 == 0 && s.cout > 8;
            rc = sh_act_backward_tr_img(g, ol.sv, ol.sb, acts[last], ol.sv, ol.sb, dpre_last, dl.sv, dl.sb, img_in ? cur_img : nullptr, B, s.R,
                                        s.cout, s.act, s.zero_row, n_tr, tr_w, tr_wt, tr_S, tr_Ci, tr_Co, stream);
            if (rc != SH_OK) return rc;
            cur = dpre_last; cl = dl;
            cur_img_done = img_in;
        } else {
            cur = g; cl = lay(out_layout, s.m_rows, B, cin_of[last]);
        }
    }
    const void* job_ws[64]; float* job_dW[64]; float* job_db[64]; int jB[64], jR[64], jS[64], jCi[64], jCo[64], jK[64];
    int njobs = 0;
    for (int i = last; i >= 0; --i) {
        const sh_stack_step& s = steps[i];
        const Forms& q = f[i];
        const bool want_in = i > 0 || need_x_grad;
        const float* inp = i == 0 ? x : acts[i - 1];
        const Lay il = i == 0 ? lay(x_layout, rows0, B, c0) : lay(0, 0, B, cin_of[i]);
        float* gi = want_in ? gin[i] : nullptr;
        SH_REQUIRE(!want_in || gi, SH_ERR_INVALID_ARG, "sh_stack_backward: no gradient buffer for the input of step %d", i);
        const Lay gl = il;
        const float* yprev = nullptr; Lay yl{0, 0}; int act_prev = 0, zero_prev = -1;
        if (i > 0 && steps[i - 1].kind == 0) {
            yprev = acts[i - 1]; yl = lay(0, 0, B, steps[i - 1].cout); act_prev = steps[i - 1].act; zero_prev = steps[i - 1].zero_row;
        }
        void* gi_img = (i > 0 && steps[i - 1].kind == 0 && f[i - 1].b_gimg) ? gin_planes[i] : nullptr;
        float* gi_f = (gi_img && f[i - 1].b_grad_img_only) ? nullptr : gi;
        bool gi_img_done = false;
        if (s.kind == 0) {
            SH_REQUIRE(workspace && workspace[i], SH_ERR_INVALID_ARG, "sh_stack_backward: no workspace for step %d", i);
            const bool wgrad = dW[s.param] != nullptr;
            SH_REQUIRE(wgrad || !dbias || !dbias[s.param], SH_ERR_INVALID_ARG,
                       "sh_stack_backward: parameter %d has a dbias buffer but no dW buffer", s.param);
            const bool thin = wgrad && q.b_thin;
            const int bd = thin ? BD_F32 : q.b_data;
            const bool p3 = bd != BD_F32, rag = bd >= BD_RAG;
            const bool ride = wgrad && q.b_ride;
            char* pimg0 = (p3 && q.b_presum_img) ? static_cast<char*>(cur_img) : nullptr;
            float* mut0 = const_cast<float*>(cur);
            if (ride && s.n1 && s.n2) {
                rc = sh_spmm_p3(s.sum1.rowptr, s.sum1.col, s.sum1.val, cur, cl.sv, cl.sb, mut0 + (long)s.R * cl.sv, cl.sv, cl.sb,
                                pimg0 ? pimg0 + sh_p3_bytes(s.R, B, s.cout) : nullptr, nullptr, 0, 0, 0, -1, B, s.n1, s.cout, stream);
                if (rc != SH_OK) return rc;
            }
            const bool p3w = wgrad && q.b_p3w && in_planes && workspace_bytes[i] >= sh_spiral_conv_bwd_wgt_p3_workspace(B, s.R, s.S, s.cin, s.cout);
            SH_REQUIRE(!q.b_in_img_only || p3w, SH_ERR_INVALID_ARG,
                       "sh_stack_backward: step %d: the forward pass kept only the image of its input (keep_fp32 == 2) but this pass cannot run "
                       "the step on images (a frozen layer, or a workspace smaller than sh_spiral_conv_bwd_wgt_p3_workspace)", i);
            if (wgrad && !thin) {
                const sh_csr_ref& lm = s.n2 ? s.sum2 : s.sum1;
                const int ln = ride ? (s.n2 ? s.n2 : s.n1) : 0;
                float* lout = mut0 + (long)(s.R + (s.n2 ? s.n1 : 0)) * cl.sv;
                void* limg = (ln && pimg0) ? pimg0 + sh_p3_bytes(s.R + (s.n2 ? s.n1 : 0), B, s.cout) : nullptr;
                if (p3w) {
                    if (!cur_img_done) {
                        rc = sh_to_p3(cur, cl.sv, cl.sb, cur_img, B, s.R, s.cout, stream);
                        if (rc != SH_OK) return rc;
// ... 273 lines not shown
```

semantichuman_amd/linear.py:

```python
from __future__ import annotations

import torch

from . import ops


class _LatentLinear(torch.autograd.Function):
    @staticmethod
    def forward(ctx, x, weight, bias):
        from . import _lib
        x = x.contiguous()
        ctx.save_for_backward(x, weight)
        ctx.has_bias = bias is not None
        ctx.mma = _lib.get_f32_mma_mode()
        return ops.linear_fwd(x, weight.contiguous(), bias, ctx.mma)

    @staticmethod
    def backward(ctx, dy):
        x, weight = ctx.saved_tensors
        dy = dy.contiguous()
        dx = ops.linear_bwd_data(dy, weight, ctx.mma) if ctx.needs_input_grad[0] else None
        dW = db = None
        if ctx.needs_input_grad[1] or (ctx.has_bias and ctx.needs_input_grad[2]):
            want_bias = ctx.has_bias and ctx.needs_input_grad[2]
            param = _fused_param(weight, dy, x) if ctx.needs_input_grad[1] else None
            if param is not None:
                db = _fused_apply(param, dy, x, want_bias, ctx.mma)
            else:
                dW, db = ops.linear_bwd_wgt(dy, x, want_bias=want_bias, mma=ctx.mma)
        return dx, dW, db


_FUSED_UPDATE = {}


def _fused_param(weight, dy, x):
    key = weight.data_ptr()
    fused = _FUSED_UPDATE.get(key)
    if fused is None:
        return None
    param, opt = fused[0](), fused[1]()
    if param is None or opt is None:
        _FUSED_UPDATE.pop(key, None)
        return None
    if param.data_ptr() == key and param.shape == weight.shape and param.grad is None and weight.is_contiguous() and \
            ops.linear_bwd_wgt_adam_ok(dy.shape[0], dy.shape[1], x.shape[1]):
        return param
    return None


def _fused_apply(param, dy, x, want_bias, mma):
    _, opt_ref, gi = _FUSED_UPDATE[param.data_ptr()]
    opt = opt_ref()
    return opt._fused_update(opt.param_groups[gi], param, dy, x, want_bias, mma)


def latent_linear(x: torch.Tensor, weight: torch.Tensor, bias) -> torch.Tensor:
    if x.dim() != 2:
        raise RuntimeError("latent_linear expects a 2-D input, got %s" % (tuple(x.shape),))
    return _LatentLinear.apply(x, weight, bias)


class _LatentLinearBF16(torch.autograd.Function):

    @staticmethod
    def forward(ctx, x, weight, bias, out_dtype):
        from . import shadow
        x = x.contiguous()
        w16 = shadow.get(weight)
        ctx.save_for_backward(x, weight)
        ctx.has_bias = bias is not None
        return ops.linear_fwd_bf16(x, w16, bias, out_dtype)

    @staticmethod
    def backward(ctx, dy):
        from . import shadow
        x, weight = ctx.saved_tensors
        dy = dy.contiguous()
        dx = ops.linear_bwd_data_bf16(dy, shadow.get(weight), x.dtype) if ctx.needs_input_grad[0] else None
        dW = db = None
        if ctx.needs_input_grad[1] or (ctx.has_bias and ctx.needs_input_grad[2]):
            want_bias = ctx.has_bias and ctx.needs_input_grad[2]
            param = _fused_param(weight, dy, x) if ctx.needs_input_grad[1] else None
            if param is not None:
                db = _fused_apply(param, dy, x, want_bias, None)
            else:
                dW, db = ops.linear_bwd_wgt_bf16(dy, x, want_bias=want_bias)
        return dx, dW, db, None


def latent_linear_bf16(x: torch.Tensor, weight: torch.Tensor, bias, out_dtype) -> torch.Tensor:
    if x.dim() != 2:
        raise RuntimeError("latent_linear_bf16 expects a 2-D input, got %s" % (tuple(x.shape),))
    return _LatentLinearBF16.apply(x, weight, bias, out_dtype)


class _GroupedLinear(torch.autograd.Function):

    @staticmethod
    def forward(ctx, x, x_off, y_cols, y_off, G, *params):
        weights, biases = list(params[:G]), list(params[G:])
        x = x.contiguous()
        weights_c = [w.contiguous() for w in weights]
        ctx.save_for_backward(x, *weights_c)
        ctx.meta = (tuple(x_off), y_cols, tuple(y_off), G, [b is not None for b in biases])
        return ops.grouped_linear_fwd(x, x_off, weights_c, biases if any(b is not None for b in biases) else None, y_cols, y_off)

    @staticmethod
    def backward(ctx, dy):
        x, *weights = ctx.saved_tensors
        x_off, y_cols, y_off, G, has_bias = ctx.meta
        dy = dy.contiguous()
        dx = ops.grouped_linear_bwd_data(dy, y_off, weights, x.shape[1], x_off) if ctx.needs_input_grad[0] else None
# ... 20 lines not shown
```

semantichuman_amd/losses.py:

```python
from __future__ import annotations

import numpy as np
import torch

from . import ops


class _L1Loss(torch.autograd.Function):
    @staticmethod
    def forward(ctx, a, b):
        a, b = a.contiguous(), b.contiguous()
        ctx.save_for_backward(a, b)
        return ops.l1_loss_fwd(a, b)

    @staticmethod
    def backward(ctx, g):
        a, b = ctx.saved_tensors
        gb = ops.l1_loss_bwd(a, b, g.contiguous())
        ga = -gb if ctx.needs_input_grad[0] else None
        return ga, (gb if ctx.needs_input_grad[1] else None)


def l1_loss(a: torch.Tensor, b: torch.Tensor) -> torch.Tensor:
    if a.shape != b.shape:
        raise RuntimeError("l1_loss: shape mismatch %s vs %s" % (tuple(a.shape), tuple(b.shape)))
    return _L1Loss.apply(a, b)


class FaceTables:

    def __init__(self, faces, n_rows: int, device):
        f = np.ascontiguousarray(np.asarray(faces, dtype=np.int32))
        corners = np.arange(f.size, dtype=np.int32)
        order = np.argsort(f.ravel(), kind="stable")
        vptr = np.zeros(n_rows + 1, dtype=np.int32)
        np.cumsum(np.bincount(f.ravel(), minlength=n_rows), out=vptr[1:])
        self.n_faces = f.shape[0]
        self.faces = torch.from_numpy(f).to(device)
        self.vptr = torch.from_numpy(vptr).to(device)
        self.vcorner = torch.from_numpy(corners[order]).to(device)
        cs = corners[order]
        ff, kk = cs // 3, cs % 3
        nbr = np.stack([f[ff, (kk + 1) % 3], f[ff, (kk + 2) % 3]], axis=1).astype(np.int32)
        self.vnbr = torch.from_numpy(np.ascontiguousarray(nbr.reshape(-1))).to(device)


class _EdgeRatioLoss(torch.autograd.Function):
    @staticmethod
    def forward(ctx, x_hat, x, ft: FaceTables):
        x_hat, x = x_hat.contiguous(), x.contiguous()
        ctx.save_for_backward(x_hat, x)
        ctx.ft = ft
        return ops.edge_ratio_loss_fwd(x_hat, x, ft.faces)

    @staticmethod
    def backward(ctx, g):
        x_hat, x = ctx.saved_tensors
        ft = ctx.ft
        return ops.edge_ratio_loss_bwd(x_hat, x, ft.faces, ft.vptr, ft.vcorner, g.contiguous()), None, None


def edge_ratio_loss(x_hat, x, ft: FaceTables):
    return _EdgeRatioLoss.apply(x_hat, x.detach(), ft)


class _ReconLoss(torch.autograd.Function):
    @staticmethod
    def forward(ctx, x_hat, x, ft: FaceTables, edge_w: float):
        x_hat, x = x_hat.contiguous(), x.contiguous()
        ctx.save_for_backward(x_hat, x)
        ctx.ft, ctx.edge_w = ft, float(edge_w)
        ctx.set_materialize_grads(False)
        total, parts = ops.recon_loss_fwd(x_hat, x, ft.faces, edge_w)
        ctx.mark_non_differentiable(parts)
        return total, parts

    @staticmethod
    def backward(ctx, g, _unused):
        x_hat, x = ctx.saved_tensors
        ft = ctx.ft
        return ops.recon_loss_bwd(x_hat, x, ft.n_faces, ft.vptr, ft.vnbr, ctx.edge_w, g.contiguous()), None, None, None


def recon_loss(x_hat, x, ft: FaceTables, edge_w: float):
    return _ReconLoss.apply(x_hat, x.detach(), ft, edge_w)


def vertex_l2_mm(x_hat, x, dummy_node: bool = True, mm_constant: float = 1000.0):
    n_real = x.shape[1] - 1 if dummy_node else x.shape[1]
    return ops.vertex_l2(x_hat.detach().contiguous(), x.detach().contiguous(), n_real, mm_constant)


def eval_l1(x_hat, x, dummy_node: bool = True):
    full = ops.l1_loss_fwd(x_hat.detach().contiguous(), x.detach().contiguous())
    if not dummy_node:
        return full
    n1 = x.shape[1]
    tail = (x_hat.detach()[:, -1] - x.detach()[:, -1]).abs().sum()
    return (full * (x.numel()) - tail) / float(x.shape[0] * (n1 - 1) * x.shape[2])
```

semantichuman_amd/models.py:

```python
from __future__ import annotations

import os

import numpy as np
import torch
import torch.nn as nn

from . import _lib, mesh_ops, ops
from .mesh_ops import CSR
from .linear import grouped_linear, latent_linear, latent_linear_bf16
from .stack import ConvStep, SpmmStep, Stack, prepare_p3_frags, prepare_wfrags, run_stack, run_stack_bf16


def _as_csr(m) -> CSR:
    if isinstance(m, CSR):
        return m
    if torch.is_tensor(m):
        m = m.detach().cpu().numpy()
    return mesh_ops.dense_to_csr(m)


def _as_table(s) -> np.ndarray:
    if torch.is_tensor(s):
        s = s.detach().cpu().numpy()
    return mesh_ops.spirals_to_table(s)


class SpiralConv(nn.Module):

    def __init__(self, in_c, spiral_size, out_c, activation='elu', bias=True, device=None):
        super().__init__()
        self.in_c, self.out_c, self.device = in_c, out_c, device
        self.spiral_size = spiral_size
        self.conv = nn.Linear(in_c * spiral_size, out_c, bias=bias)
        self.act_name = activation
        self.act_id = ops.act_id(activation)
        self._cache_key, self._cache_stack = None, None
        self._cache_obj = None

    def _stack_for(self, spiral_adj) -> Stack:
        adj = spiral_adj.detach()
        o = self._cache_obj
        if (o is not None and o[0]() is spiral_adj and o[1] == spiral_adj._version and o[2] == spiral_adj.data_ptr()
                and o[3] == tuple(spiral_adj.shape)):
            return self._cache_stack
        if adj.is_cuda and torch.cuda.is_current_stream_capturing():
            raise RuntimeError("SpiralConv.forward: this spiral_adj tensor has not been seen before; its content check needs a "
                               "host read, which a hipGraph capture does not allow - call forward once with the same tensor "
                               "object before capturing")
        hit = (self._cache_key is not None and self._cache_key.shape == adj.shape[1:] and self._cache_key.device == adj.device
               and self._cache_key.dtype == adj.dtype)
        if hit:
            hit = bool((adj == self._cache_key).all())
        if not hit:
            if adj.shape[0] > 1 and not bool((adj == adj[:1]).all()):
                raise NotImplementedError("per-sample spiral indices are not supported (the reference always "
                                          "passes one index repeated over the batch, models.py:122)")
            table = _as_table(adj[:1])
            st = ConvStep(param=0, table=table, n_in=table.shape[0], cin=self.in_c, cout=self.out_c, act=self.act_id)
            self._cache_stack = Stack([st]).to(spiral_adj.device)
            self._cache_key = adj[0].clone()
# ... 66 lines not shown
    return Stack(steps, input_dummy_dead=False)


class SpiralAutoencoder(nn.Module):

    def __init__(self, filters_enc, filters_dec, latent_size, sizes, spiral_sizes, spirals, D, U, device,
                 VAE_flag=False, activation='elu'):
        super().__init__()
        self.latent_size, self.sizes, self.spirals = latent_size, sizes, spirals
        self.filters_enc, self.filters_dec, self.spiral_sizes = filters_enc, filters_dec, spiral_sizes
        self.D, self.U, self.device = D, U, device
        self.activation, self.VAE_flag = activation, VAE_flag
        levels = len(spiral_sizes) - 1
        enc_layout, dec_layout = conv_layout(filters_enc, filters_dec, spiral_sizes, activation)
        self.conv = nn.ModuleList([SpiralConv(c, S, o, activation=a, device=device) for (c, S, o, a, _) in enc_layout])
        feat = enc_layout[-1][2]
        self.fc_latent_enc = nn.Linear((sizes[-1] + 1) * feat, (2 if VAE_flag else 1) * latent_size)
        self.fc_latent_dec = nn.Linear(latent_size, (sizes[-1] + 1) * filters_dec[0][0])
        self.dconv = nn.ModuleList([SpiralConv(c, S, o, activation=a, device=device) for (c, S, o, a, _) in dec_layout])

        tables = [_as_table(spirals[l]) for l in range(levels)]
        for l in range(levels):
            if tables[l].shape != (sizes[l] + 1, spiral_sizes[l]):
                raise ValueError("spirals[%d] has shape %s, expected %s" % (l, tables[l].shape, (sizes[l] + 1, spiral_sizes[l])))
        Ds = [_as_csr(D[l]) for l in range(levels)]
        Us = [_as_csr(U[l]) for l in range(levels)]
        self._enc_stack = build_encoder_stack(enc_layout, tables, Ds, sizes)
        self._dec_stack = build_decoder_stack(dec_layout, tables, Us, sizes)
        if device is not None:
            self.to(device)

    def _apply(self, fn, *a, **k):
        out = super()._apply(fn, *a, **k)
        dev = self.fc_latent_enc.weight.device
        if self._enc_stack.device != dev:
            self._enc_stack.to(dev)
            self._dec_stack.to(dev)
            self.device = dev
        return out

    def set_compute_dtype(self, dtype):
        if dtype not in (torch.float32, torch.bfloat16):
            raise ValueError("compute dtype must be torch.float32 or torch.bfloat16")
        self.compute_dtype = dtype
        return self

    def encode(self, x, VAE_flag=None, _wf=None):
        bsize = x.size(0)
        if getattr(self, "compute_dtype", torch.float32) == torch.bfloat16:
            h = run_stack_bf16(self._enc_stack, x, "bm", "bm", torch.bfloat16, self.conv, _wf)
            z = latent_linear_bf16(h.reshape(bsize, -1), self.fc_latent_enc.weight, self.fc_latent_enc.bias, torch.float32)
        else:
            h = run_stack(self._enc_stack, x, "bm", "bm", self.conv)
            z = latent_linear(h.reshape(bsize, -1), self.fc_latent_enc.weight, self.fc_latent_enc.bias)
        if VAE_flag if VAE_flag is not None else self.VAE_flag:
            self.z_mu = z[..., :self.latent_size]
            self.z_var = z[..., self.latent_size:]
            std = torch.exp(self.z_var / 2)
            z = torch.randn_like(std).mul(std).add_(self.z_mu)
        return z

    def decode(self, z, _wf=None):
        bsize = z.size(0)
        if getattr(self, "compute_dtype", torch.float32) == torch.bfloat16:
            h = latent_linear_bf16(z.float(), self.fc_latent_dec.weight, self.fc_latent_dec.bias, torch.bfloat16)
            return run_stack_bf16(self._dec_stack, h.view(bsize, self.sizes[-1] + 1, -1), "bm", "bm", torch.float32, self.dconv, _wf)
        h = latent_linear(z, self.fc_latent_dec.weight, self.fc_latent_dec.bias).view(bsize, self.sizes[-1] + 1, -1)
        return run_stack(self._dec_stack, h, "bm", "bm", self.dconv)

    def forward(self, x):
        wf = None
        if getattr(self, "compute_dtype", torch.float32) == torch.float32 and x.is_cuda and _lib.get_f32_mma_mode() == "planes3":
            grad = torch.is_grad_enabled() and any(p.requires_grad for p in self.parameters())
            prepare_p3_frags([(self._enc_stack, self.conv, x.shape[2]), (self._dec_stack, self.dconv, self.filters_dec[0][0])],
                             x.shape[0], grad)
        if getattr(self, "compute_dtype", torch.float32) == torch.bfloat16 and x.is_cuda:
            wf = prepare_wfrags([(self._enc_stack, self.conv), (self._dec_stack, self.dconv)])
        try:
            z = self.encode(x, self.VAE_flag, wf)
            return self.decode(z, wf), z
        finally:
            self._enc_stack.__dict__.pop("_p3_next", None)
            self._dec_stack.__dict__.pop("_p3_next", None)


class SpiralAutoencoder_multiz_partkps(nn.Module):

    def __init__(self, kps_index_list, vert_part_index_dict, filters_enc, filters_dec, latent_size, part_kps_latent_size,
                 sizes, spiral_sizes, spirals, D, U, device, VAE_flag=False, activation='elu', newskl_list=None):
        super().__init__()
        from . import constants
        self.newskl_list = constants.NEWSKL_LIST if newskl_list is None else newskl_list
        self.kps_keep = constants.kps_keep(self.newskl_list)
        self.kps_index_list, self.vert_part_index_dict = kps_index_list, vert_part_index_dict
        self.part_kps_latent_size, self.latent_size = part_kps_latent_size, latent_size
        self.sizes, self.spirals, self.spiral_sizes = sizes, spirals, spiral_sizes
        self.filters_enc, self.filters_dec = filters_enc, filters_dec
        self.D, self.U, self.device, self.activation, self.VAE_flag = D, U, device, activation, VAE_flag
        levels = len(spiral_sizes) - 1
        enc_layout, dec_layout = conv_layout(filters_enc, filters_dec, spiral_sizes, activation)
        self.conv = nn.ModuleList([SpiralConv(c, S, o, activation=a, device=device) for (c, S, o, a, _) in enc_layout])
        feat = enc_layout[-1][2]
        parts = [np.asarray(v) for v in vert_part_index_dict.values()]
        self.fc_latent_enc_list = nn.ModuleList([nn.Linear(len(v) * feat, (2 if VAE_flag else 1) * latent_size) for v in parts])
        self.fc_latent_dec_list = nn.ModuleList([nn.Linear(latent_size + part_kps_latent_size, len(v) * filters_dec[0][0])
                                                 for v in parts])
        self.kps_enc_list = nn.ModuleList([nn.Linear(len(k) * 3, part_kps_latent_size) for k in kps_index_list])
# ... 98 lines not shown
```

semantichuman_amd/ops.py:

```python
from __future__ import annotations

import torch

from . import _lib
from ._lib import ACT_IDS, check, ptr, stream_ptr


def _dims(t: torch.Tensor, layout: str, dtypes=(torch.float32,)):
    if t.dim() != 3 or not t.is_contiguous() or t.dtype not in dtypes:
        raise ValueError("expected a contiguous %s 3-D tensor, got %s %s" % ("/".join(str(d) for d in dtypes), tuple(t.shape), t.dtype))
    if not t.is_cuda:
        raise RuntimeError("semantichuman_amd kernels need a HIP device tensor (got %s); there is no CPU path" % t.device)
    if layout == "bm":
        B, R, C = t.shape
        return B, R, C, C, R * C
    if layout == "vm":
        R, B, C = t.shape
        return B, R, C, B * C, C
    raise ValueError("layout must be 'bm' or 'vm'")


def _check_index_range(t):
    if t.numel() >= 2 ** 32:
        raise RuntimeError("semantichuman_amd: gathered tensors are addressed with 32-bit element offsets; "
# ... 233 lines not shown
    _check2d(dy, x)
    M = dy.shape[0]
    dWs = [torch.empty_like(w) for w in weights]
    dbs = [torch.empty((w.shape[0],), dtype=torch.float32, device=w.device) if wb else None for w, wb in zip(weights, want_bias)]
    G, xo, yo, N, K = _glin_args(x_off, y_off, [w.shape[0] for w in weights], [w.shape[1] for w in weights])
    check(_lib.load().sh_grouped_linear_bwd_wgt(G, ptr(dy), dy.shape[1], yo, ptr(x), x.shape[1], xo, _ptr_array(dWs),
                                                _ptr_array(dbs), M, N, K, stream_ptr()), "sh_grouped_linear_bwd_wgt")
    return dWs, dbs


def _ws(device):
    return torch.empty(_lib.load().sh_reduce_workspace() // 4, dtype=torch.float32, device=device)


def l1_loss_fwd(a, b):
    assert a.shape == b.shape and a.is_contiguous() and b.is_contiguous() and a.is_cuda
    out = torch.empty((), dtype=torch.float32, device=a.device)
    check(_lib.load().sh_l1_loss_fwd(ptr(a), ptr(b), a.numel(), ptr(out), ptr(_ws(a.device)), stream_ptr()), "sh_l1_loss_fwd")
    return out


def l1_loss_bwd(a, b, gscale):
    g = torch.empty_like(b)
    check(_lib.load().sh_l1_loss_bwd(ptr(a), ptr(b), a.numel(), ptr(gscale), ptr(g), stream_ptr()), "sh_l1_loss_bwd")
    return g


def vertex_l2(a, b, n_real, scale=1000.0):
    assert a.shape == b.shape and a.dim() == 3 and a.shape[2] == 3 and a.is_contiguous() and b.is_contiguous()
    out = torch.empty((), dtype=torch.float32, device=a.device)
    check(_lib.load().sh_vertex_l2(ptr(a), ptr(b), a.shape[0], a.shape[1], n_real, scale, ptr(out), ptr(_ws(a.device)),
                                   stream_ptr()), "sh_vertex_l2")
    return out


def edge_ratio_loss_fwd(x_hat, x, faces):
    assert x_hat.shape == x.shape and x.shape[2] == 3 and x_hat.is_contiguous() and x.is_contiguous()
    out = torch.empty((), dtype=torch.float32, device=x.device)
    check(_lib.load().sh_edge_ratio_loss_fwd(ptr(x_hat), ptr(x), ptr(faces), x.shape[0], x.shape[1], faces.shape[0], ptr(out),
                                             ptr(_ws(x.device)), stream_ptr()), "sh_edge_ratio_loss_fwd")
    return out


def recon_loss_fwd(x_hat, x, faces, edge_w):
    assert x_hat.shape == x.shape and x.shape[2] == 3 and x_hat.is_contiguous() and x.is_contiguous() and x.is_cuda
    total = torch.empty((), dtype=torch.float32, device=x.device)
    parts = torch.empty((2,), dtype=torch.float32, device=x.device)
    ws = torch.empty(_lib.load().sh_recon_loss_workspace() // 4, dtype=torch.float32, device=x.device)
    check(_lib.load().sh_recon_loss_fwd(ptr(x_hat), ptr(x), ptr(faces), x.shape[0], x.shape[1], faces.shape[0], float(edge_w),
                                        ptr(total), ptr(parts), ptr(ws), stream_ptr()), "sh_recon_loss_fwd")
    return total, parts


def recon_loss_bwd(x_hat, x, n_faces, vptr, vnbr, edge_w, gscale):
    g = torch.empty_like(x_hat)
    check(_lib.load().sh_recon_loss_bwd(ptr(x_hat), ptr(x), ptr(vptr), ptr(vnbr), x.shape[0], x.shape[1], int(n_faces),
                                        float(edge_w), ptr(gscale), ptr(g), stream_ptr()), "sh_recon_loss_bwd")
    return g


def edge_ratio_loss_bwd(x_hat, x, faces, vptr, vcorner, gscale):
    g = torch.empty_like(x_hat)
    check(_lib.load().sh_edge_ratio_loss_bwd(ptr(x_hat), ptr(x), ptr(faces), ptr(vptr), ptr(vcorner), x.shape[0], x.shape[1],
                                             faces.shape[0], ptr(gscale), ptr(g), stream_ptr()), "sh_edge_ratio_loss_bwd")
    return g


def measure_girth(v, rings):
    ptr_, a, b, f = rings
    if not (v.is_cuda and v.dtype == torch.float32 and v.dim() == 3 and v.shape[2] == 3 and v.stride(2) == 1
            and v.stride(1) == 3):
        raise RuntimeError("semantichuman_amd.measure_girth needs fp32 HIP vertices [B, rows, 3] (got %s %s %s); there is "
                           "no CPU path" % (v.device, v.dtype, tuple(v.shape)))
    B, P = v.shape[0], ptr_.numel() - 1
    out = torch.empty((B, P), dtype=torch.float32, device=v.device)
    check(_lib.load().sh_measure_girth(ptr(v), v.stride(0) if B > 1 else v.shape[1] * 3, ptr(ptr_), ptr(a), ptr(b), ptr(f),
                                       B, P, ptr(out), stream_ptr()), "sh_measure_girth")
    return out


def bone_length(kps, bones):
    if not (kps.is_cuda and kps.dtype == torch.float32 and kps.dim() == 3 and kps.shape[2] == 3 and kps.is_contiguous()):
        raise RuntimeError("semantichuman_amd.bone_length needs contiguous fp32 HIP joints [B, K, 3]; there is no CPU path")
    B, K, P = kps.shape[0], kps.shape[1], bones.shape[0]
    out = torch.empty((B, P), dtype=torch.float32, device=kps.device)
    check(_lib.load().sh_bone_length(ptr(kps), ptr(bones), B, K, P, ptr(out), stream_ptr()), "sh_bone_length")
    return out


def measure_girth_bwd(v, rings, g_girth):
    ptr_, a, b, f = rings.tables()
    pt_ring, vt_ptr, vt_pt, vt_w, n_vt = rings.transposed()
    B, rows, P = v.shape[0], v.shape[1], ptr_.numel() - 1
    out = torch.empty((B, rows, 3), dtype=torch.float32, device=v.device)
    check(_lib.load().sh_measure_girth_bwd(ptr(v), v.stride(0) if B > 1 else rows * 3, ptr(ptr_), ptr(a), ptr(b), ptr(f), ptr(pt_ring),
                                           ptr(vt_ptr), ptr(vt_pt), ptr(vt_w), n_vt, ptr(g_girth), B, P, rows, ptr(out), stream_ptr()),
          "sh_measure_girth_bwd")
    return out


def bone_length_bwd(kps, bones, g_len):
    jt_ptr, jt_bone, jt_w, n_jt = bones.transposed()
    B, K, P = kps.shape[0], kps.shape[1], bones.n_bones
    out = torch.empty((B, K, 3), dtype=torch.float32, device=kps.device)
    check(_lib.load().sh_bone_length_bwd(ptr(kps), ptr(bones.table), ptr(jt_ptr), ptr(jt_bone), ptr(jt_w), n_jt, ptr(g_len), B, K, P,
                                         ptr(out), stream_ptr()), "sh_bone_length_bwd")
# ... 368 lines not shown
```

semantichuman_amd/optim.py:

```python
from __future__ import annotations

import ctypes

import torch

from . import _lib


class Adam(torch.optim.Optimizer):
    def __init__(self, params, lr=1e-3, betas=(0.9, 0.999), eps=1e-8, weight_decay=0, amsgrad=False):
        if amsgrad:
            raise NotImplementedError("semantichuman_amd.optim.Adam: amsgrad is not used by the reference and not built")
        if not 0.0 <= lr or not 0.0 <= eps or not 0.0 <= weight_decay or not all(0.0 <= b < 1.0 for b in betas):
            raise ValueError("invalid Adam hyper-parameters lr=%r betas=%r eps=%r weight_decay=%r" % (lr, betas, eps, weight_decay))
        super().__init__(params, dict(lr=lr, betas=tuple(betas), eps=eps, weight_decay=weight_decay, amsgrad=False))
        self._lr_dev = {}
        self._early = set()
        self._hooks = []
        self._side = None
        self._fused = []
        self._fused_done = []
        self._release_foreign_fusions()

    def _release_foreign_fusions(self):
        import warnings
        from . import linear
        for group in self.param_groups:
            for p in group["params"]:
                ent = linear._FUSED_UPDATE.get(p.data_ptr()) if p.is_cuda else None
                if ent is None or ent[0]() is not p:
                    continue
                other = ent[1]()
                if other is not None and other is not self:
                    warnings.warn("semantichuman_amd.optim.Adam: a parameter of this optimizer was registered for the fused weight-"
                                  "gradient update of another optimizer; that registration is removed (call "
                                  "fuse_linear_weight_gradients on the new optimizer to fuse again)", stacklevel=3)
                    other._drop_fusion_of(p)
                linear._FUSED_UPDATE.pop(p.data_ptr(), None)

    def _drop_fusion_of(self, p):
        self._fused = [r for r in self._fused if r() is not None and r() is not p]

    def __del__(self):
        try:
            self.remove_fusion()
        except Exception:
            pass

    def _state_of(self, p):
        st = self.state[p]
        if not st:
            if not (p.is_cuda and p.dtype == torch.float32 and p.is_contiguous()):
                raise RuntimeError("semantichuman_amd.optim.Adam updates contiguous fp32 HIP parameters (got %s %s); there "
                                   "is no CPU path" % (p.device, p.dtype))
            st["step"] = torch.zeros((), dtype=torch.float32, device=p.device)
            st["exp_avg"] = torch.zeros_like(p, memory_format=torch.preserve_format)
            st["exp_avg_sq"] = torch.zeros_like(p, memory_format=torch.preserve_format)
        elif not (st["step"].is_cuda and st["step"].dtype == torch.float32):
            st["step"] = torch.as_tensor(float(st["step"]), dtype=torch.float32, device=p.device)
        return st

    def _lr_tensor(self, group, device):
        cur = self._lr_dev.get(id(group))
        lr = float(group["lr"])
        if cur is None or cur[0].device != device:
            cur = (torch.full((), lr, dtype=torch.float32, device=device), lr)
        elif cur[1] != lr:
            cur[0].fill_(lr)
            cur = (cur[0], lr)
        self._lr_dev[id(group)] = cur
        return cur[0]

    def sync_lr(self):
        for group in self.param_groups:
            ps = [p for p in group["params"] if p.is_cuda]
            if ps:
                self._lr_tensor(group, ps[0].device)

    def _apply(self, group, params, bump_only=()):
        params = [p for p in params if p.grad is not None]
        if not params and not bump_only:
            return
        n_upd = len(params)
        params = params + list(bump_only)
        n = len(params)
        arr = lambda: (ctypes.c_void_p * n)()
        P, G, M, V, S, N = arr(), arr(), arr(), arr(), arr(), (ctypes.c_int64 * n)()
        W16, any16 = arr(), False
        from . import shadow
        keep = []
        for i, p in enumerate(params):
            if i >= n_upd:
                S[i], N[i] = self.state[p]["step"].data_ptr(), 0
                continue
            g = p.grad
            if g.is_sparse or g.dtype != torch.float32 or g.device != p.device:
                raise RuntimeError("semantichuman_amd.optim.Adam needs dense fp32 gradients on the parameter's device")
            if not g.is_contiguous():
                g = g.contiguous()
                keep.append(g)
            st = self._state_of(p)
            P[i], G[i], M[i], V[i], S[i] = p.data_ptr(), g.data_ptr(), st["exp_avg"].data_ptr(), st["exp_avg_sq"].data_ptr(), \
                st["step"].data_ptr()
            N[i] = p.numel()
            w16 = shadow.lookup(p)
            if w16 is not None:
                W16[i], any16 = w16.data_ptr(), True
        lr = self._lr_tensor(group, params[0].device)
        b1, b2 = group["betas"]
        if any16:
            _lib.check(_lib.load().sh_adam_step_bf16(n, P, G, M, V, S, W16, N, _lib.ptr(lr), float(b1), float(b2), float(group["eps"]),
                                                     float(group["weight_decay"]), _lib.stream_ptr()), "sh_adam_step_bf16")
        else:
            _lib.check(_lib.load().sh_adam_step(n, P, G, M, V, S, N, _lib.ptr(lr), float(b1), float(b2), float(group["eps"]),
                                                float(group["weight_decay"]), _lib.stream_ptr()), "sh_adam_step")

    def overlap_backward(self, min_numel=1 << 20):
        self.remove_overlap()
        for group in self.param_groups:
            for p in group["params"]:
                if p.requires_grad and p.numel() >= min_numel:
                    self._hooks.append(p.register_post_accumulate_grad_hook(lambda q, g=group: self._on_grad(g, q)))
        return self

    def remove_overlap(self):
        for h in self._hooks:
            h.remove()
        self._hooks = []

    def _on_grad(self, group, p):
        if self._side is None:
            self._side = torch.cuda.Stream(device=p.device)
        self._side.wait_stream(torch.cuda.current_stream(p.device))
        with torch.cuda.stream(self._side):
            self._apply(group, [p])
        self._early.add(id(p))

    def fuse_linear_weight_gradients(self, modules):
        import weakref
        from . import linear
        for mod in modules:
            w = mod.weight
            group = next((g for g in self.param_groups if any(q is w for q in g["params"])), None)
            if group is None:
                raise ValueError("fuse_linear_weight_gradients: a module's weight is not a parameter of this optimizer")
            if not (w.is_cuda and w.dtype == torch.float32 and w.is_contiguous() and w.dim() == 2):
                raise RuntimeError("fuse_linear_weight_gradients: contiguous 2-D fp32 HIP weights only")
            prev = linear._FUSED_UPDATE.get(w.data_ptr())
            if prev is not None and prev[0]() is w and prev[1]() not in (None, self):
                prev[1]()._drop_fusion_of(w)
            linear._FUSED_UPDATE[w.data_ptr()] = (weakref.ref(w), weakref.ref(self), self.param_groups.index(group))
            if not any(r() is w for r in self._fused):
                self._fused.append(weakref.ref(w))
        return self

    def remove_fusion(self):
        from . import linear
        for r in self._fused:
            w = r()
            if w is None:
                continue
            ent = linear._FUSED_UPDATE.get(w.data_ptr())
            if ent is not None and ent[1]() in (None, self):
# ... 32 lines not shown
```

semantichuman_amd/stack.py:

```python
from __future__ import annotations

import ctypes
import os
from dataclasses import dataclass, field
from typing import Optional

import numpy as np
import torch

from . import _lib, mesh_ops, ops
from .mesh_ops import CSR, TransposedTable

NATIVE = os.environ.get("SH_STACK_NATIVE", "1") != "0"
_LAYOUT_ID = {"vm": 0, "bm": 1}
_P3_RAGGED = os.environ.get("SH_P3_RAGGED", "1").strip() != "0"
DEBUG_POISON = os.environ.get("SH_DEBUG_POISON", "0").strip() == "1"
_P3_GROUPED = os.environ.get("SH_P3_GROUPED", "1").strip() != "0"
_ALIGN = 64


def _round(n: int) -> int:
    return (n + _ALIGN - 1) // _ALIGN * _ALIGN

OVERLAP_WGRAD = os.environ.get("SH_OVERLAP_WGRAD", "0") != "0"
OVERLAP_PRESUM = os.environ.get("SH_OVERLAP_PRESUM", "0") != "0"
FULL_WGRAD = os.environ.get("SH_FULL_WGRAD", "0").strip() == "1"


def _dev(a: np.ndarray, device):
    return torch.from_numpy(np.ascontiguousarray(a)).to(device)


def _csr_dev(m: CSR, device):
    return (_dev(m.rowptr, device), _dev(m.col, device), _dev(m.val, device))


@dataclass
class ConvStep:
    param: int
    table: np.ndarray
    n_in: int
    cin: int
    cout: int
    act: int
    dead_dummy_grad: bool = False
    dummy_in: int = -1
    kind: str = "conv"
    R: int = 0
    S: int = 0
    zero_row: int = -1
    tt: Optional[TransposedTable] = None
    n_extra: int = 0
    dev: dict = field(default_factory=dict)

    def finalize(self):
        self.R, self.S = self.table.shape
        self.zero_row = self.R - 1
        dummy = self.dummy_in if self.dummy_in >= 0 else self.n_in - 1
        self.tt = mesh_ops.transpose_table_dense(self.table, self.n_in, none_row=self.zero_row,
                                                 skip_row=dummy if self.dead_dummy_grad else -1)
        self.n_extra = self.tt.n_extra
        self.rag = mesh_ops.transpose_table_ragged(self.table, self.n_in, none_row=self.zero_row,
                                                   skip_row=dummy if self.dead_dummy_grad else -1) if _P3_RAGGED else None
        self.fgrp = self.bgrp = None
        if _P3_GROUPED:
            lib = _lib.load()
            m = lib.sh_spiral_conv_p3_grp_members(16, self.S, self.cin, self.cout)
            if m:
                pos = np.ascontiguousarray(np.broadcast_to(np.arange(self.S, dtype=np.int32), self.table.shape))
                self.fgrp = mesh_ops.group_lists(self.table, pos, members=m)
            m = lib.sh_spiral_conv_p3_grp_members(16, self.S, self.cout, self.cin)
# ... 259 lines not shown
        plans[key] = plan
        return plan

    @staticmethod
    def _ptr_array(tensors):
        return (ctypes.c_void_p * len(tensors))(*[0 if t is None else t.data_ptr() for t in tensors])

    def _p3_prepare(self, plan, weights, with_backward: bool, device):
        planes = torch.empty(max(256, plan["pl_total"]), dtype=torch.uint8, device=device)
        pre = self.__dict__.pop("_p3_next", None)
        if pre is not None and pre[2] == id(plan) and (pre[3] or not with_backward):
            return planes, pre[0], pre[1]
        wf3 = torch.empty(max(256, plan["wf3_total"]), dtype=torch.uint8, device=device)
        convert_p3_frags([(self, plan, weights, wf3, 0)], with_backward)
        return planes, wf3, 0

    def native_forward(self, x, in_layout, out_layout, weights, biases, mma: str = "exact", with_backward: bool = False, frozen=None):
        B = x.shape[0] if in_layout == "bm" else x.shape[1]
        rows0 = x.shape[1] if in_layout == "bm" else x.shape[0]
        c0 = x.shape[2]
        if not (x.is_contiguous() and x.dtype == torch.float32):
            raise ValueError("expected a contiguous fp32 3-D tensor, got %s %s" % (tuple(x.shape), x.dtype))
        if x.numel() >= 2 ** 32:
            raise RuntimeError("semantichuman_amd: gathered tensors are addressed with 32-bit element offsets; "
                               "%d elements is too large - split the batch" % x.numel())
        plan = self._plan(B, c0)
        n = len(self.steps)
        arena = torch.empty(max(1, plan["f_total"]), dtype=torch.float32, device=x.device)
        if DEBUG_POISON:
            arena.fill_(float("nan"))
        out = ops.alloc(B, plan["out_rows"][-1], plan["out_ch"][-1], out_layout, x.device)
        outs = plan["f_off"] + np.uint64(arena.data_ptr())
        outs[n - 1] = out.data_ptr()
        p3 = None
        keep = 1 if with_backward else 0
        any_frozen = bool(frozen) and any(frozen)
        any_trained = not frozen or not all(frozen)
        planes_p = wf3_p = None
        if mma == "planes3" and plan["wf3_total"]:
            planes, wf3, wbase = self._p3_prepare(plan, weights, with_backward, x.device)
            p3 = (planes if (with_backward and any_trained and plan["in_img"].any()) else None, wf3, wbase)
            if p3[0] is not None and not any_frozen:
                keep = 2
            pl = (plan["pl_off"] + np.uint64(planes.data_ptr())) * plan["pl_mask"]
            wf = (plan["wf3_off"] + np.uint64(wf3.data_ptr() + wbase)) * plan["wf3_mask"]
            planes_p, wf3_p = pl.ctypes.data, wf.ctypes.data
        _lib.check(_lib.load().sh_stack_forward(n, self._native_steps(), _lib.ptr(x), _LAYOUT_ID[in_layout], rows0, c0, B,
                                                self._ptr_array(weights), self._ptr_array(biases), outs.ctypes.data,
                                                _LAYOUT_ID[out_layout], _lib.mma_id(mma), planes_p, wf3_p, keep, _lib.stream_ptr()),
                   "sh_stack_forward")
        return out, arena, p3

    def native_backward(self, x, in_layout, out_layout, arena, out, g, weights, need_x_grad, need_bias, mma: str = "exact", p3=None,
                        frozen=None):
        B = x.shape[0] if in_layout == "bm" else x.shape[1]
        rows0 = x.shape[1] if in_layout == "bm" else x.shape[0]
        c0 = x.shape[2]
        plan = self._plan(B, c0)
        n = len(self.steps)
        dev = x.device
        work = torch.empty(max(1, plan["b_total"]), dtype=torch.float32, device=dev)
        if DEBUG_POISON:
            work.fill_(float("nan"))
        flat = torch.empty(max(1, plan["p_total"]), dtype=torch.float32, device=dev)
        gx = ops.alloc(B, rows0, c0, in_layout, dev) if need_x_grad else None
        acts = plan["f_off"] + np.uint64(arena.data_ptr())
        acts[n - 1] = out.data_ptr()
        wbase, fbase = np.uint64(work.data_ptr()), np.uint64(flat.data_ptr())
        gin = (plan["g_off"] + wbase) * plan["g_mask"]
        gin[0] = gx.data_ptr() if need_x_grad else 0
        wt = (plan["wt_off"] + wbase) * plan["wt_mask"]
        ws = (plan["ws_off"] + wbase) * plan["ws_mask"]
        assert len(need_bias) == plan["npar"] == len(weights)
        frozen = list(frozen) if frozen else [False] * plan["npar"]
        assert not any(f and nb for f, nb in zip(frozen, need_bias))
        dW = (plan["dW_off"] + fbase) * np.array([0 if f else 1 for f in frozen], dtype=np.uint64)
        db = (plan["db_off"] + fbase) * np.array([1 if nb else 0 for nb in need_bias], dtype=np.uint64)
        gpl_p = wf3t_p = inpl_p = None
        dpl = ctypes.c_void_p(0)
        if mma == "planes3" and p3 is not None and p3[0] is not None:
            inpl = np.zeros(n, dtype=np.uint64)
            inpl[1:] = (plan["pl_off"][:n - 1] + np.uint64(p3[0].data_ptr())) * plan["in_img"][1:]
            inpl_p = inpl.ctypes.data
        if mma == "planes3" and p3 is not None:
            gimg = torch.empty(max(256, plan["gpl_total"]), dtype=torch.uint8, device=dev)
            gpl = (plan["gpl_off"] + np.uint64(gimg.data_ptr())) * plan["gpl_mask"]
            wf = (plan["wf3t_off"] + np.uint64(p3[1].data_ptr() + p3[2])) * plan["wf3t_mask"]
            gpl_p, wf3t_p = gpl.ctypes.data, wf.ctypes.data
            if plan["dpl_mask"]:
                dpl = ctypes.c_void_p(gimg.data_ptr() + int(plan["dpl_off"]))
        _lib.check(_lib.load().sh_stack_backward(
            n, self._native_steps(), _lib.ptr(x), _LAYOUT_ID[in_layout], rows0, c0, B, acts.ctypes.data, _lib.ptr(g),
            _LAYOUT_ID[out_layout], self._ptr_array(weights), gin.ctypes.data, ctypes.c_void_p(int(wbase) + 4 * plan["dpre_last_off"]),
            wt.ctypes.data, ws.ctypes.data, plan["ws_bytes"].ctypes.data, dW.ctypes.data, db.ctypes.data, 1 if need_x_grad else 0,
            _lib.mma_id(mma), gpl_p, dpl, wf3t_p, inpl_p, 2 if (inpl_p is not None and not any(frozen)) else 1, _lib.stream_ptr()),
            "sh_stack_backward")
        grads = {}
        for j, shp in enumerate(plan["shapes"]):
            if shp is None or frozen[j]:
                continue
            o = int(plan["dW_off_f"][j])
            dWj = flat[o:o + shp[0] * shp[1]].view(shp)
            o = int(plan["db_off_f"][j])
            grads[j] = (dWj, flat[o:o + shp[0]] if need_bias[j] else None)
        return gx, grads

    def _plan_bf16(self, B: int, c0: int, x_is_f32: bool, out_is_f32: bool):
        key = ("bf16", B, c0, x_is_f32, out_is_f32)
        plans = self.__dict__.setdefault("_plans", {})
        if key in plans:
            return plans[key]
        lib = _lib.load()
        al = lambda nbytes: (int(nbytes) + 255) // 256 * 256
        n = len(self.steps)
        cin_of, c = [], c0
        for st in self.steps:
            cin_of.append(c)
            c = st.cout if st.kind == "conv" else c
        out_rows = [st.R if st.kind == "conv" else st.csr.rows for st in self.steps]
        out_ch = [st.cout if st.kind == "conv" else cin_of[i] for i, st in enumerate(self.steps)]
        f_off, wf_off, wf_mask, o = np.zeros(n, dtype=np.uint64), np.zeros(n, dtype=np.uint64), np.zeros(n, dtype=np.uint64), 0
        for i in range(n - 1):
            if self._extends(i):
                f_off[i] = f_off[i - 1]
                continue
            f_off[i] = o
            o += al(self._buffer_rows(i) * B * out_ch[i] * 2)
        for i, st in enumerate(self.steps):
            if st.kind == "conv":
                wf_off[i], wf_mask[i] = o, 1
                o += al(lib.sh_conv_wfrag_bytes(st.S, st.cin, st.cout))
        f_total = o
        last = self.steps[-1]
        o = 0
        if last.kind == "conv":
            o += al((last.R + last.n_extra) * B * last.cout * (4 if out_is_f32 else 2))
        gin_size = [0] * n
        for i in range(1, n):
            st, prev = self.steps[i], self.steps[i - 1]
            rows_in = st.n_in if st.kind == "conv" else st.csr.cols
            gin_size[i] = (rows_in + (prev.n_extra if prev.kind == "conv" else 0)) * B * cin_of[i] * 2
        region = [al(max([gin_size[i] for i in range(1, n) if i % 2 == par] + [0])) for par in (0, 1)]
        region_off = [o, o + region[0]]
        o += region[0] + region[1]
        g_off, g_mask = np.zeros(n, dtype=np.uint64), np.zeros(n, dtype=np.uint64)
        for i in range(1, n):
            g_off[i], g_mask[i] = region_off[i % 2], 1
        wt_off, wt_mask = np.zeros(n, dtype=np.uint64), np.zeros(n, dtype=np.uint64)
# ... 237 lines not shown
                raise RuntimeError("semantichuman_amd: conv weights must be contiguous fp32 HIP tensors")
            w_p.append(w.data_ptr()); o_p.append(buf.data_ptr() + base + off)
            S.append(st.S); Ci.append(st.cin); Co.append(st.cout); tr.append(t)
    n = len(w_p)
    if not n:
        return
    arr = lambda vals, ct: (ct * n)(*vals)
    _lib.check(lib.sh_conv_wfrag3_prep_multi(n, arr(w_p, ctypes.c_void_p), arr(o_p, ctypes.c_void_p), arr(S, ctypes.c_int),
                                             arr(Ci, ctypes.c_int), arr(Co, ctypes.c_int), arr(tr, ctypes.c_int), _lib.stream_ptr()),
               "sh_conv_wfrag3_prep_multi")


def prepare_p3_frags(stacks_convs_c0, B: int, with_backward: bool):
    if B % 16:
        return
    items, total = [], 0
    for stack, convs, c0 in stacks_convs_c0:
        plan = stack._plan(B, c0)
        if not plan["wf3_total"]:
            continue
        items.append((stack, plan, [m.conv.weight for m in convs], None, total))
        total += (int(plan["wf3_total"]) + 255) // 256 * 256
    if not items:
        return
    buf = torch.empty(total, dtype=torch.uint8, device=items[0][2][0].device)
    items = [(st, pl, ws, buf, off) for st, pl, ws, _, off in items]
    convert_p3_frags(items, with_backward)
    for st, pl, ws, _, off in items:
        st._p3_next = (buf, off, id(pl), with_backward)


def _frozen_mask(needs_input_grad, first: int, n: int):
    if FULL_WGRAD:
        return [False] * n
    return [not (needs_input_grad[first + 2 * j] or needs_input_grad[first + 2 * j + 1]) for j in range(n)]


class StackFunction(torch.autograd.Function):

    @staticmethod
    def forward(ctx, stack: Stack, in_layout: str, out_layout: str, x, *params):
        weights, biases = list(params[0::2]), list(params[1::2])
        x = x.contiguous()
        need = any(ctx.needs_input_grad[3:])
        ctx.stack, ctx.layouts = stack, (in_layout, out_layout)
        ctx.has_bias = [b is not None for b in biases]
        ctx.native = NATIVE and not (OVERLAP_WGRAD or OVERLAP_PRESUM)
        ctx.mma = _lib.get_f32_mma_mode()
        ctx.frozen = _frozen_mask(ctx.needs_input_grad, 4, len(weights))
        if ctx.native:
            out, arena, ctx.p3 = stack.native_forward(x, in_layout, out_layout, weights, biases, ctx.mma, with_backward=need or ctx.needs_input_grad[3],
                                                      frozen=ctx.frozen)
            ctx.save_for_backward(x, out, arena, *weights)
            return out
        out, acts = stack.run_forward(x, in_layout, out_layout, weights, biases, keep=need)
        ctx.acts = acts[:-1]
        ctx.save_for_backward(x, out, *weights)
        return out

    @staticmethod
    def backward(ctx, g):
        stack = ctx.stack
        in_layout, out_layout = ctx.layouts
        g = g.contiguous()
        need_bias = [hb and ctx.needs_input_grad[5 + 2 * j] for j, hb in enumerate(ctx.has_bias)]
        if ctx.native:
            x, out, arena, *weights = ctx.saved_tensors
            gx, grads = stack.native_backward(x, in_layout, out_layout, arena, out, g, weights, ctx.needs_input_grad[3], need_bias,
                                              ctx.mma, ctx.p3, ctx.frozen)
            ctx.p3 = None
        else:
            x, out, *weights = ctx.saved_tensors
            was = _lib.get_f32_mma_mode()
            _lib.set_f32_mma_mode(ctx.mma)
            try:
                gx, grads = stack.run_backward(x, in_layout, out_layout, ctx.acts + [out], g, weights,
                                               ctx.needs_input_grad[3], need_bias, ctx.frozen)
            finally:
                _lib.set_f32_mma_mode(was)
            ctx.acts = None
        res = [None, None, None, gx]
        for j in range(len(weights)):
            dW, db = grads.get(j, (None, None))
            res += [dW, db]
        return tuple(res)


class WFrags:

    def __init__(self, stacks_and_weights, with_backward: bool):
        lib = _lib.load()
        jobs, total = [], 0
        al = lambda n: (n + 255) // 256 * 256
        for stack, weights in stacks_and_weights:
            for i, st in enumerate(stack.steps):
                if st.kind != "conv":
                    continue
                for tr in ((0, 1) if with_backward else (0,)):
                    nb = lib.sh_conv_wfrag_bytes(st.S, st.cout if tr else st.cin, st.cin if tr else st.cout)
                    jobs.append((stack, i, st, weights[st.param], tr, total))
                    total += al(nb)
        dev = stacks_and_weights[0][1][0].device
        self.buf = torch.empty(max(256, total), dtype=torch.uint8, device=dev)
        base = self.buf.data_ptr()
        self.fwd = {id(stack): np.zeros(len(stack.steps), dtype=np.uint64) for stack, _ in stacks_and_weights}
        self.bwd = {id(stack): np.zeros(len(stack.steps), dtype=np.uint64) for stack, _ in stacks_and_weights} if with_backward else None
        for stack, i, st, w, tr, off in jobs:
            (self.bwd if tr else self.fwd)[id(stack)][i] = base + off
            if not (w.is_cuda and w.dtype == torch.float32 and w.is_contiguous()):
                raise RuntimeError("semantichuman_amd: conv weights must be contiguous fp32 HIP tensors (bf16 working copies are made from them)")
        n = len(jobs)
        arr = lambda vals, ct: (ct * n)(*vals)
        _lib.check(lib.sh_conv_wfrag_prep_multi(
            n, arr([j[3].data_ptr() for j in jobs], ctypes.c_void_p), arr([base + j[5] for j in jobs], ctypes.c_void_p),
            arr([j[2].S for j in jobs], ctypes.c_int), arr([j[2].cin for j in jobs], ctypes.c_int),
            arr([j[2].cout for j in jobs], ctypes.c_int), arr([j[4] for j in jobs], ctypes.c_int), _lib.stream_ptr()),
            "sh_conv_wfrag_prep_multi")


def prepare_wfrags(stacks_and_convs):
    pairs = [(stack, [m.conv.weight for m in convs]) for stack, convs in stacks_and_convs]
    with_backward = torch.is_grad_enabled() and any(w.requires_grad for _, ws in pairs for w in ws)
# ... 65 lines not shown
```

Before: 47620.

## Fold last-layer activation grad into producer kernels and fuse loss/Adam tails

Adds a BackwardLink so the layer consuming the stack output, or the recon loss backward, writes the stack's pre-activation gradient (and its plane image) straight into the stack backward workspace. The stack backward then skips its own activation-derivative pass and the weight transposes. It also fuses the recon-loss partial and final reductions into one kernel using a last-block ticket, and folds the Adam step bump into the Adam kernel the same way. The aim is fewer launches and less memory traffic per step, at the cost of heavier autograd plumbing and a runtime error if the gradient has other contributors.

```diff
diff --git a/include/sh_kernels.h b/include/sh_kernels.h
--- a/include/sh_kernels.h
+++ b/include/sh_kernels.h
@@ -140,6 +140,8 @@
                             const float* const* weights, const float* const* biases, float* const* outs, int out_layout,
                             int mma_mode, void* const* planes, const void* const* wfrag3, int keep_fp32, sh_stream_t stream);
 
+#define SH_STACK_BWD_G_IS_DPRE 0x100
+#define SH_STACK_BWD_TR_DONE 0x200
 SH_API int sh_stack_backward(int n_steps, const sh_stack_step* steps, const float* x, int x_layout, int rows0, int c0, int B,
                              const float* const* acts, const float* g, int out_layout, const float* const* weights,
                              float* const* gin, float* dpre_last, float* const* weight_t, void* const* workspace,
@@ -154,6 +156,9 @@
                        void* workspace, size_t workspace_bytes, int mma_mode, sh_stream_t stream);
 SH_API int sh_linear_bwd_wgt(const float* dy, const float* x, float* dW, float* dbias, int M, int N, int K,
                       void* workspace, size_t workspace_bytes, int mma_mode, sh_stream_t stream);
+SH_API int sh_linear_bwd_data_act_ok(int M, int N, int K, int C, int mma_mode);
+SH_API int sh_linear_bwd_data_act(const float* dy, const float* weight, const float* y, int act, int zero_row, int C, float* dpre,
+                           void* dpre_planes, int M, int N, int K, int mma_mode, sh_stream_t stream);
 SH_API int sh_linear_bwd_wgt_adam_ok(int M, int N, int K);
 SH_API int sh_linear_bwd_wgt_adam(const void* dy, int dy_dtype, const void* x, int x_dtype, float* weight, void* weight_bf16, float* exp_avg,
                            float* exp_avg_sq, const float* step, const float* lr, double beta1, double beta2, double eps,
@@ -188,6 +193,12 @@
                       float* total, float* parts, void* workspace, sh_stream_t stream);
 SH_API int sh_recon_loss_bwd(const float* x_hat, const float* x, const int32_t* vptr, const int32_t* vnbr, int B, int N1, int F,
                       float edge_w, const float* gscale, float* grad, sh_stream_t stream);
+SH_API int sh_recon_loss_fwd_fused(const float* x_hat, const float* x, const int32_t* faces, int B, int N1, int F, float edge_w,
+                            float* total, float* parts, void* workspace, unsigned* ticket, sh_stream_t stream);
+SH_API int sh_recon_loss_bwd_dpre(const float* x_hat, const float* x, const int32_t* vptr, const int32_t* vnbr, int B, int N1, int F,
+                           float edge_w, const float* gscale, float* dpre, int act, int zero_row, int n_layers,
+                           const float* const* weight, float* const* weight_t, const int* S, const int* Cin, const int* Cout,
+                           sh_stream_t stream);
 
 SH_API int sh_part_pairdist_tile_rows(void);
 SH_API int sh_part_pairdist_loss_fwd(const float* x_rec, const float* x_gt, const float* bone, const float* scale,
@@ -274,6 +285,9 @@
                  float* const* exp_avg_sq, float* const* steps, const int64_t* numel, const float* lr,
                  double beta1, double beta2, double eps, double weight_decay, sh_stream_t stream);
 SH_API int sh_adam_bump(int n_tensors, float* const* steps, sh_stream_t stream);
+SH_API int sh_adam_step_ticket(int n_tensors, float* const* params, const float* const* grads, float* const* exp_avg,
+                        float* const* exp_avg_sq, float* const* steps, void* const* shadow_bf16, const int64_t* numel, const float* lr,
+                        double beta1, double beta2, double eps, double weight_decay, unsigned* ticket, sh_stream_t stream);
 
 SH_API int sh_joint_regress(const float* x, int64_t x_bs, const float* J, int B, int N, int K, float* kps, sh_stream_t stream);
 SH_API int sh_joint_l1_loss_fwd(const float* x, int64_t x_bs, const float* J, const int32_t* keep, const float* target, int B,
diff --git a/semantichuman_amd/_lib.py b/semantichuman_amd/_lib.py
--- a/semantichuman_amd/_lib.py
+++ b/semantichuman_amd/_lib.py
@@ -40,6 +40,11 @@
     "sh_linear_bwd_wgt_adam_ok": (c_int, [_I, _I, _I]),
     "sh_linear_bwd_wgt_adam": (c_int, [_P, _I, _P, _I] + [_P] * 6 + [ctypes.c_double] * 4 + [_P, _I, _I, _I, _I, _P]),
     "sh_adam_bump": (c_int, [_I, _P, _P]),
+    "sh_adam_step_ticket": (c_int, [_I, _P, _P, _P, _P, _P, _P, _P, _P] + [ctypes.c_double] * 4 + [_P, _P]),
+    "sh_recon_loss_fwd_fused": (c_int, [_P, _P, _P, _I, _I, _I, c_float, _P, _P, _P, _P, _P]),
+    "sh_recon_loss_bwd_dpre": (c_int, [_P, _P, _P, _P, _I, _I, _I, c_float, _P, _P, _I, _I, _I, _P, _P, _P, _P, _P, _P]),
+    "sh_linear_bwd_data_act_ok": (c_int, [_I, _I, _I, _I, _I]),
+    "sh_linear_bwd_data_act": (c_int, [_P, _P, _P, _I, _I, _I, _P, _P, _I, _I, _I, _I, _P]),
     "sh_grouped_linear_fwd": (c_int, [_I, _P, _L, _P, _P, _P, _P, _L, _P, _I, _P, _P, _P]),
     "sh_grouped_linear_bwd_data": (c_int, [_I, _P, _L, _P, _P, _P, _L, _P, _I, _P, _P, _P]),
     "sh_grouped_linear_bwd_wgt": (c_int, [_I, _P, _L, _P, _P, _L, _P, _P, _P, _I, _P, _P, _P]),
diff --git a/semantichuman_amd/csrc/adam.hip b/semantichuman_amd/csrc/adam.hip
--- a/semantichuman_amd/csrc/adam.hip
+++ b/semantichuman_amd/csrc/adam.hip
@@ -22,6 +22,7 @@
     const float* lr;
     double beta1, beta2;
     float w1, b2, w2, eps, wd;
+    unsigned* ticket;
 };
 
 __global__ __launch_bounds__(ANT) void adam_kernel(const AdamArgs a) {
@@ -92,6 +93,20 @@
             }
         }
     }
+    if (a.ticket) {
+        __shared__ int is_last;
+        __syncthreads();
+        if (threadIdx.x == 0) {
+            __threadfence();
+            is_last = atomicAdd(a.ticket, 1u) == gridDim.x - 1;
+        }
+        __syncthreads();
+        if (is_last) {
+            __threadfence();
+            if ((int)threadIdx.x < a.nt) a.step[threadIdx.x][0] += 1.f;
+            if (threadIdx.x == 0) *a.ticket = 0u;
+        }
+    }
 }
 
 __global__ void adam_bump_kernel(const AdamArgs a) {
@@ -104,7 +119,7 @@
 
 static int adam_impl(int n_tensors, float* const* params, const float* const* grads, float* const* exp_avg, float* const* exp_avg_sq,
                      float* const* steps, void* const* shadow, const int64_t* numel, const float* lr, double beta1, double beta2,
-                     double eps, double weight_decay, sh_stream_t stream) {
+                     double eps, double weight_decay, sh_stream_t stream, unsigned* ticket = nullptr) {
     SH_REQUIRE(n_tensors >= 0, SH_ERR_INVALID_ARG, "sh_adam_step: negative tensor count");
     if (n_tensors == 0) return SH_OK;
     SH_REQUIRE(params && grads && exp_avg && exp_avg_sq && steps && numel && lr, SH_ERR_INVALID_ARG, "sh_adam_step: null pointer");
@@ -132,13 +147,14 @@
         a.nontemporal = nontemporal;
         a.lr = lr; a.beta1 = beta1; a.beta2 = beta2;
         a.w1 = (float)(1.0 - beta1); a.b2 = (float)beta2; a.w2 = (float)(1.0 - beta2); a.eps = (float)eps; a.wd = (float)weight_decay;
+        a.ticket = blocks > 0 ? ticket : nullptr;
         if (blocks > 0) {
             long numel_sum = 0;
             for (int i = 0; i < a.nt; ++i) numel_sum += a.n[i];
             ShProfScope ps(st, "adam_kernel|tensors=%d blocks=%ld numel=%ld", a.nt, blocks, numel_sum);
             SH_LAUNCH_PS(ps, adam_kernel, dim3((unsigned)blocks), dim3(ANT), 0, st, a);
         }
-        hipLaunchKernelGGL(adam_bump_kernel, dim3(1), dim3(64), 0, st, a);
+        if (!a.ticket) hipLaunchKernelGGL(adam_bump_kernel, dim3(1), dim3(64), 0, st, a);
         SH_CHECK_LAUNCH("adam_step");
     }
     return SH_OK;
@@ -174,4 +190,11 @@
     return adam_impl(n_tensors, params, grads, exp_avg, exp_avg_sq, steps, shadow_bf16, numel, lr, beta1, beta2, eps, weight_decay, stream);
 }
 
-}
+int sh_adam_step_ticket(int n_tensors, float* const* params, const float* const* grads, float* const* exp_avg, float* const* exp_avg_sq,
+                        float* const* steps, void* const* shadow_bf16, const int64_t* numel, const float* lr, double beta1, double beta2,
+                        double eps, double weight_decay, unsigned* ticket, sh_stream_t stream) {
+    SH_REQUIRE(ticket, SH_ERR_INVALID_ARG, "sh_adam_step_ticket: null ticket");
+    return adam_impl(n_tensors, params, grads, exp_avg, exp_avg_sq, steps, shadow_bf16, numel, lr, beta1, beta2, eps, weight_decay, stream, ticket);
+}
+
+}
diff --git a/semantichuman_amd/csrc/linear.hip b/semantichuman_amd/csrc/linear.hip
--- a/semantichuman_amd/csrc/linear.hip
+++ b/semantichuman_amd/csrc/linear.hip
@@ -231,7 +231,33 @@
     float* av;
     __bf16* shadow;
     ShAdamHyper ad;
+    const float* ep_y;
+    float* ep_dp;
+    char* ep_img;
+    long ep_img_vb, ep_img_bgb;
+    int ep_C, ep_act, ep_zero_row;
 };
+
+__device__ __forceinline__ void ls_put_dx_act(const LSParams& p, int m, int k, f32x4 g) {
+    const f32x4 yv = *reinterpret_cast<const f32x4*>(p.ep_y + (long)m * p.K + k);
+    const int C = p.ep_C, r = k / C, co = k - r * C;
+    const bool zero = r == p.ep_zero_row;
+    f32x4 o;
+#pragma unroll
+    for (int j = 0; j < 4; ++j) o[j] = zero ? 0.f : g[j] * sh_act_grad_from_out(yv[j], p.ep_act);
+    if (p.ep_dp) *reinterpret_cast<f32x4*>(p.ep_dp + ((long)r * p.M + m) * C + co) = o;
+    if (p.ep_img) {
+        u32x2 ph, pm, pl;
+        sh_split3_quad(o, ph, pm, pl);
+        const bool c16 = C == 16;
+        char* d = p.ep_img + (long)r * p.ep_img_vb + (long)(m >> 4) * p.ep_img_bgb +
+                  (c16 ? ((co >> 3) * 16 + (m & 15)) * 16 : (co >> 5) * 3072 + (((co & 31) >> 3) * 16 + (m & 15)) * 16) + ((co >> 2) & 1) * 8;
+        const int pb = c16 ? 512 : 1024;
+        *reinterpret_cast<u32x2*>(d) = ph;
+        *reinterpret_cast<u32x2*>(d + pb) = pm;
+        *reinterpret_cast<u32x2*>(d + 2 * pb) = pl;
+    }
+}
 
 template <int MT>
 __global__ __launch_bounds__(LTHREADS) void linear_fwd_stream_kernel(const LSParams p) {
@@ -516,6 +542,12 @@
     for (int mt = 0; mt < MT; ++mt) {
         const int m = 16 * mt + la;
         if (m >= p.M) continue;
+        if (p.ep_y) {
+#pragma unroll
+            for (int jj = 0; jj < 4; ++jj)
+                ls_put_dx_act(p, m, k0 + 16 * rr + 4 * jj, (f32x4){acc[0][mt][jj], acc[1][mt][jj], acc[2][mt][jj], acc[3][mt][jj]});
+            continue;
+        }
         float* dst = (p.nsplit > 1 ? p.slab + ((long)sp * p.M + m) * p.K : p.out + (long)m * p.K) + k0 + 16 * rr;
 #pragma unroll
         for (int jj = 0; jj < 4; ++jj)
@@ -579,6 +611,12 @@
     for (int mt = 0; mt < MT; ++mt) {
         const int m = 16 * mt + la;
         if (m >= p.M) continue;
+        if (p.ep_y) {
+#pragma unroll
+            for (int jj = 0; jj < 4; ++jj)
+                ls_put_dx_act(p, m, k0 + 16 * rr + 4 * jj, (f32x4){acc[0][mt][jj], acc[1][mt][jj], acc[2][mt][jj], acc[3][mt][jj]});
+            continue;
+        }
         float* dst = (p.nsplit > 1 ? p.slab + ((long)sp * p.M + m) * p.K : p.out + (long)m * p.K) + k0 + 16 * rr;
 #pragma unroll
         for (int jj = 0; jj < 4; ++jj)
@@ -1042,6 +1080,36 @@
     p.c = dx; p.c_sm = K; p.c_sn = 1; p.bias = nullptr;
     p.M = M; p.N = K; p.R = N;
     return run_gemm(p, workspace, workspace_bytes, static_cast<hipStream_t>(stream), "linear_bwd_data");
+}
+
+int sh_linear_bwd_data_act_ok(int M, int N, int K, int C, int mma_mode) {
+    if (M <= 0 || N <= 0 || K <= 0 || C <= 0 || C % 4 || K % C || !sh_mma_mode_valid(mma_mode)) return 0;
+    const bool x3 = lin_x3(mma_mode) && N % 32 == 0;
+    const LSPlan pl = plan_stream(M, K, N, x3 ? 32 : 16);
+    return pl.ok && pl.nsplit == 1 ? 1 : 0;
+}
+
+int sh_linear_bwd_data_act(const float* dy, const float* weight, const float* y, int act, int zero_row, int C, float* dpre, void* dpre_planes,
+                           int M, int N, int K, int mma_mode, sh_stream_t stream) {
+    SH_REQUIRE(dy && weight && y && (dpre || dpre_planes) && M > 0 && N > 0 && K > 0, SH_ERR_INVALID_ARG, "sh_linear_bwd_data_act: bad argument");
+    SH_REQUIRE(sh_mma_mode_valid(mma_mode), SH_ERR_INVALID_ARG, "sh_linear_bwd_data_act: unknown mma_mode %d", mma_mode);
+    SH_REQUIRE(act >= SH_ACT_IDENTITY && act <= SH_ACT_TANH, SH_ERR_INVALID_ARG, "sh_linear_bwd_data_act: unknown activation %d", act);
+    SH_REQUIRE(sh_linear_bwd_data_act_ok(M, N, K, C, mma_mode), SH_ERR_UNSUPPORTED,
+               "sh_linear_bwd_data_act: M=%d N=%d K=%d C=%d: the unsplit streaming kernel does not serve this shape", M, N, K, C);
+    SH_REQUIRE(aligned16(dy, weight, y) && (!dpre || (reinterpret_cast<uintptr_t>(dpre) & 15) == 0), SH_ERR_INVALID_ARG,
+               "sh_linear_bwd_data_act: tensors must be 16-byte aligned");
+    const bool x3 = lin_x3(mma_mode) && N % 32 == 0;
+    const LSPlan pl = plan_stream(M, K, N, x3 ? 32 : 16);
+    LSParams s{};
+    s.a = dy; s.w = weight; s.bias = nullptr; s.out = nullptr; s.M = M; s.N = N; s.K = K;
+    s.ep_y = y; s.ep_dp = dpre; s.ep_img = static_cast<char*>(dpre_planes); s.ep_C = C; s.ep_act = act; s.ep_zero_row = zero_row;
+    if (dpre_planes) {
+        SH_REQUIRE(sh_p3_bytes(1, M, C) && (reinterpret_cast<uintptr_t>(dpre_planes) & 15) == 0, SH_ERR_UNSUPPORTED,
+                   "sh_linear_bwd_data_act: M=%d C=%d has no plane image (M %% 16 == 0; C 16 or %% 32 == 0)", M, C);
+        s.ep_img_bgb = C == 16 ? 1536 : (long)(C / 32) * 3072;
+        s.ep_img_vb = s.ep_img_bgb * (M / 16);
+    }
+    return run_stream<false>(s, pl, K, nullptr, 0, static_cast<hipStream_t>(stream), "linear_bwd_data_act", x3);
 }
 
 static bool wgt_dma_attr() {
diff --git a/semantichuman_amd/csrc/spmm_loss.hip b/semantichuman_amd/csrc/spmm_loss.hip
--- a/semantichuman_amd/csrc/spmm_loss.hip
+++ b/semantichuman_amd/csrc/spmm_loss.hip
@@ -265,9 +265,8 @@
     }
 }
 
-__global__ void recon_partial_kernel(const float* __restrict__ xh, const float* __restrict__ x, const int* __restrict__ faces,
-                                     int B, int N1, int F, float* __restrict__ part) {
-    __shared__ float red[16];
+__device__ __forceinline__ void recon_partial_body(const float* __restrict__ xh, const float* __restrict__ x, const int* __restrict__ faces,
+                                                   int B, int N1, int F, float* part, float* red) {
     float s = 0.f;
     const long n = (long)B * N1 * 3;
     for (long i = (long)blockIdx.x * blockDim.x + threadIdx.x; i < n; i += (long)gridDim.x * blockDim.x) s += fabsf(x[i] - xh[i]);
@@ -291,9 +290,14 @@
     if (threadIdx.x == 0) part[RED_BLOCKS + blockIdx.x] = t2;
 }
 
-__global__ void recon_final_kernel(const float* __restrict__ part, int np, double scale1, double scale2, float w, float* __restrict__ total,
-                                   float* __restrict__ parts) {
-    __shared__ double red[2][256];
+__global__ void recon_partial_kernel(const float* __restrict__ xh, const float* __restrict__ x, const int* __restrict__ faces,
+                                     int B, int N1, int F, float* __restrict__ part) {
+    __shared__ float red[16];
+    recon_partial_body(xh, x, faces, B, N1, F, part, red);
+}
+
+__device__ __forceinline__ void recon_final_body(const float* part, int np, double scale1, double scale2, float w, float* __restrict__ total,
+                                                 float* __restrict__ parts, double (*red)[256]) {
     double s1 = 0.0, s2 = 0.0;
     for (int i = threadIdx.x; i < np; i += 256) { s1 += (double)part[i]; s2 += (double)part[RED_BLOCKS + i]; }
     red[0][threadIdx.x] = s1; red[1][threadIdx.x] = s2;
@@ -306,6 +310,31 @@
         const float rec = (float)(red[0][0] * scale1), edge = (float)(red[1][0] * scale2);
         total[0] = rec + w * edge; parts[0] = rec; parts[1] = edge;
     }
+}
+
+__global__ void recon_final_kernel(const float* __restrict__ part, int np, double scale1, double scale2, float w, float* __restrict__ total,
+                                   float* __restrict__ parts) {
+    __shared__ double red[2][256];
+    recon_final_body(part, np, scale1, scale2, w, total, parts, red);
+}
+
+__global__ __launch_bounds__(256) void recon_fwd_fused_kernel(const float* __restrict__ xh, const float* __restrict__ x,
+                                                              const int* __restrict__ faces, int B, int N1, int F, float* part, double scale1,
+                                                              double scale2, float w, float* __restrict__ total, float* __restrict__ parts,
+                                                              unsigned* ticket) {
+    __shared__ float red[16];
+    __shared__ double redd[2][256];
+    __shared__ int is_last;
+    recon_partial_body(xh, x, faces, B, N1, F, part, red);
+    if (threadIdx.x == 0) {
+        __threadfence();
+        is_last = atomicAdd(ticket, 1u) == gridDim.x - 1;
+    }
+    __syncthreads();
+    if (!is_last) return;
+    __threadfence();
+    recon_final_body(part, (int)gridDim.x, scale1, scale2, w, total, parts, redd);
+    if (threadIdx.x == 0) *ticket = 0u;
 }
 
 __global__ __launch_bounds__(256) void recon_bwd_kernel(const float* __restrict__ xh, const float* __restrict__ x, const int* __restrict__ vptr,
@@ -339,6 +368,70 @@
         o3.y = s2 * g[1] + (df[1] > 0.f ? s1 : (df[1] < 0.f ? -s1 : 0.f));
         o3.z = s2 * g[2] + (df[2] > 0.f ? s1 : (df[2] < 0.f ? -s1 : 0.f));
         *reinterpret_cast<P3*>(grad + i * 3) = o3;
+    }
+}
+
+struct ReconTr { const float* w[4]; float* wt[4]; int S[4], Cin[4], Cout[4], block0[4]; int nd; };
+constexpr int RB_TV = 16, RB_TB = 16;
+__global__ __launch_bounds__(256) void recon_bwd_dpre_kernel(const float* __restrict__ xh, const float* __restrict__ x, const int* __restrict__ vptr,
+                                                             const int* __restrict__ vnbr, int B, int N1, int F, float w,
+                                                             const float* __restrict__ gscale, float* __restrict__ dpre, int act, int zero_row,
+                                                             int grid_main, const ReconTr tr) {
+    if ((int)blockIdx.x >= grid_main) {
+        const int blk = (int)blockIdx.x - grid_main;
+        int d = 0;
+        while (d + 1 < tr.nd && tr.block0[d + 1] <= blk) ++d;
+        const int S = tr.S[d], Cin = tr.Cin[d], Cout = tr.Cout[d];
+        const long n = (long)S * Cin * Cout, i = (long)(blk - tr.block0[d]) * 256 + threadIdx.x;
+        if (i < n) {
+            const int co = (int)(i % Cout);
+            const long t = i / Cout;
+            const int s = (int)(t % S), ci = (int)(t / S);
+            tr.wt[d][i] = tr.w[d][(long)co * S * Cin + (long)s * Cin + ci];
+        }
+        return;
+    }
+    __shared__ float tile[RB_TV][RB_TB * 3 + 1], ytile[RB_TV][RB_TB * 3 + 1];
+    const int nbt = (B + RB_TB - 1) / RB_TB;
+    const int vt = (int)blockIdx.x / nbt, bt = (int)blockIdx.x - vt * nbt;
+    const int v0 = vt * RB_TV, b0 = bt * RB_TB;
+    const float g0 = gscale[0];
+    const float s1 = g0 / ((float)B * (float)N1 * 3.f), s2 = g0 * w / ((float)B * (float)F);
+    const int vl = threadIdx.x & (RB_TV - 1), bl = threadIdx.x >> 4;
+    const int v = v0 + vl, bb = b0 + bl;
+    if (v < N1 && bb < B) {
+        const float* ph = xh + (long)bb * N1 * 3;
+        const float* pg = x + (long)bb * N1 * 3;
+        const int p0 = 2 * vptr[v], p1 = 2 * vptr[v + 1];
+        const P3 hv = ld3(ph, v), gv = ld3(pg, v);
+        float g[3] = {0.f, 0.f, 0.f};
+        for (int e = p0; e < p1; e += 4) {
+            int o[4];
+            P3 ho[4], go[4];
+#pragma unroll
+            for (int k = 0; k < 4; ++k) o[k] = vnbr[e + k < p1 ? e + k : p1 - 1];
+#pragma unroll
+            for (int k = 0; k < 4; ++k) { ho[k] = ld3(ph, o[k]); go[k] = ld3(pg, o[k]); }
+#pragma unroll
+            for (int k = 0; k < 4; ++k)
+                if (e + k < p1) edge_grad3(hv, gv, ho[k], go[k], g);
+        }
+        const float df[3] = {hv.x - gv.x, hv.y - gv.y, hv.z - gv.z};
+        const float yv[3] = {hv.x, hv.y, hv.z};
+#pragma unroll
+        for (int c = 0; c < 3; ++c) {
+            tile[vl][bl * 3 + c] = s2 * g[c] + (df[c] > 0.f ? s1 : (df[c] < 0.f ? -s1 : 0.f));
+            ytile[vl][bl * 3 + c] = yv[c];
+        }
+    }
+    __syncthreads();
+    const int nb = min(RB_TB, B - b0) * 3;
+    for (int i = threadIdx.x; i < RB_TV * RB_TB * 3; i += 256) {
+        const int r = i / (RB_TB * 3), k = i - r * (RB_TB * 3);
+        if (v0 + r < N1 && k < nb) {
+            const float o = tile[r][k] * sh_act_grad_from_out(ytile[r][k], act);
+            dpre[((long)(v0 + r) * B + b0) * 3 + k] = (v0 + r == zero_row) ? 0.f : o;
+        }
     }
 }
 
@@ -477,6 +570,47 @@
     return SH_OK;
 }
 
+int sh_recon_loss_fwd_fused(const float* x_hat, const float* x, const int32_t* faces, int B, int N1, int F, float edge_w, float* total,
+                            float* parts, void* workspace, unsigned* ticket, sh_stream_t stream) {
+    SH_REQUIRE(x_hat && x && faces && total && parts && workspace && ticket && B > 0 && N1 > 0 && F > 0, SH_ERR_INVALID_ARG,
+               "sh_recon_loss_fwd_fused: bad argument");
+    hipStream_t st = static_cast<hipStream_t>(stream);
+    float* part = static_cast<float*>(workspace);
+    const long n = (long)B * N1 * 3;
+    const int nb = grid_for(n, 1024) < RED_BLOCKS ? grid_for(n, 1024) : RED_BLOCKS;
+    ShProfScope ps(st, "recon_fwd_fused_kernel|B=%d N1=%d F=%d blocks=%d", B, N1, F, nb);
+    SH_LAUNCH_PS(ps, recon_fwd_fused_kernel, dim3(nb), dim3(256), 0, st, x_hat, x, faces, B, N1, F, part, 1.0 / (double)n,
+                 1.0 / ((double)B * F), edge_w, total, parts, ticket);
+    SH_CHECK_LAUNCH("recon_loss_fwd_fused");
+    return SH_OK;
+}
+
+int sh_recon_loss_bwd_dpre(const float* x_hat, const float* x, const int32_t* vptr, const int32_t* vnbr, int B, int N1, int F, float edge_w,
+                           const float* gscale, float* dpre, int act, int zero_row, int n_layers, const float* const* weight,
+                           float* const* weight_t, const int* S, const int* Cin, const int* Cout, sh_stream_t stream) {
+    SH_REQUIRE(x_hat && x && vptr && vnbr && gscale && dpre && B > 0 && N1 > 0 && F > 0, SH_ERR_INVALID_ARG,
+               "sh_recon_loss_bwd_dpre: bad argument");
+    SH_REQUIRE(act >= SH_ACT_IDENTITY && act <= SH_ACT_TANH, SH_ERR_INVALID_ARG, "sh_recon_loss_bwd_dpre: unknown activation %d", act);
+    SH_REQUIRE(n_layers >= 0 && n_layers <= 4 && (n_layers == 0 || (weight && weight_t && S && Cin && Cout)), SH_ERR_INVALID_ARG,
+               "sh_recon_loss_bwd_dpre: bad transpose list (at most 4 layers)");
+    ReconTr tr{};
+    int tr_blocks = 0;
+    for (int i = 0; i < n_layers; ++i) {
+        SH_REQUIRE(weight[i] && weight_t[i] && S[i] > 0 && Cin[i] > 0 && Cout[i] > 0, SH_ERR_INVALID_ARG, "sh_recon_loss_bwd_dpre: bad layer %d", i);
+        tr.w[i] = weight[i]; tr.wt[i] = weight_t[i]; tr.S[i] = S[i]; tr.Cin[i] = Cin[i]; tr.Cout[i] = Cout[i]; tr.block0[i] = tr_blocks;
+        tr_blocks += (int)(((long)S[i] * Cin[i] * Cout[i] + 255) / 256);
+    }
+    tr.nd = n_layers;
+    const long gm = (long)((N1 + RB_TV - 1) / RB_TV) * ((B + RB_TB - 1) / RB_TB);
+    SH_REQUIRE(gm + tr_blocks < (1L << 31), SH_ERR_UNSUPPORTED, "sh_recon_loss_bwd_dpre: too many workgroups");
+    hipStream_t st = static_cast<hipStream_t>(stream);
+    ShProfScope ps(st, "recon_bwd_dpre_kernel|B=%d N1=%d F=%d tr=%d", B, N1, F, n_layers);
+    SH_LAUNCH_PS(ps, recon_bwd_dpre_kernel, dim3((unsigned)(gm + tr_blocks)), dim3(256), 0, st, x_hat, x, vptr, vnbr, B, N1, F, edge_w, gscale,
+                 dpre, act, zero_row, (int)gm, tr);
+    SH_CHECK_LAUNCH("recon_loss_bwd_dpre");
+    return SH_OK;
+}
+
 int sh_edge_ratio_loss_bwd(const float* x_hat, const float* x, const int32_t* faces, const int32_t* vptr, const int32_t* vcorner,
                            int B, int N1, int F, const float* gscale, float* grad, sh_stream_t stream) {
     SH_REQUIRE(x_hat && x && faces && vptr && vcorner && gscale && grad && B > 0 && N1 > 0 && F > 0, SH_ERR_INVALID_ARG,
diff --git a/semantichuman_amd/csrc/stack_exec.hip b/semantichuman_amd/csrc/stack_exec.hip
--- a/semantichuman_amd/csrc/stack_exec.hip
+++ b/semantichuman_amd/csrc/stack_exec.hip
@@ -204,9 +204,13 @@
                       const size_t* workspace_bytes, float* const* dW, float* const* dbias, int need_x_grad, int mma_mode,
                       void* const* gin_planes, void* dpre_last_planes, const void* const* wfrag3_t, const void* const* in_planes,
                       int acts_fp32, sh_stream_t stream) {
+    const bool g_is_dpre = (acts_fp32 & SH_STACK_BWD_G_IS_DPRE) != 0, tr_done = (acts_fp32 & SH_STACK_BWD_TR_DONE) != 0;
+    acts_fp32 &= ~(SH_STACK_BWD_G_IS_DPRE | SH_STACK_BWD_TR_DONE);
     int rc = check_steps(n_steps, steps, c0, "sh_stack_backward");
     if (rc != SH_OK) return rc;
     if (B > 0 && (rc = check_tensor_sizes(n_steps, steps, rows0, c0, B, "sh_stack_backward")) != SH_OK) return rc;
+    SH_REQUIRE(!g_is_dpre || (n_steps > 0 && steps[n_steps - 1].kind == 0 && g == dpre_last), SH_ERR_INVALID_ARG,
+               "sh_stack_backward: SH_STACK_BWD_G_IS_DPRE needs a conv as the last step and g == dpre_last");
     SH_REQUIRE(x && acts && g && weights && gin && dW && B > 0, SH_ERR_INVALID_ARG, "sh_stack_backward: null pointer or empty batch");
     SH_REQUIRE(n_steps <= 64, SH_ERR_UNSUPPORTED, "sh_stack_backward: more than 64 steps");
     SH_REQUIRE(sh_mma_mode_valid(mma_mode), SH_ERR_INVALID_ARG, "sh_stack_backward: unknown mma_mode %d", mma_mode);
@@ -239,7 +243,8 @@
         tr_w[n_tr] = weights[steps[i].param]; tr_wt[n_tr] = weight_t[i]; tr_S[n_tr] = steps[i].S; tr_Ci[n_tr] = steps[i].cin; tr_Co[n_tr] = steps[i].cout;
         ++n_tr;
     }
-    if (n_tr && !(sw.tr_ride && steps[last].kind == 0)) {
+    if (tr_done) n_tr = 0;
+    if (n_tr && (g_is_dpre || !(sw.tr_ride && steps[last].kind == 0))) {
         rc = sh_weight_transpose_multi(n_tr, tr_w, tr_wt, tr_S, tr_Ci, tr_Co, stream);
         if (rc != SH_OK) return rc;
         n_tr = 0;
@@ -254,9 +259,11 @@
             const Lay ol = lay(out_layout, s.R, B, s.cout), dl = lay(0, 0, B, s.cout);
             cur_img = f[last].b_gimg ? dpre_last_planes : nullptr;
             const bool img_in = cur_img && s.cout % 4 == 0 && s.cout > 8;
-            rc = sh_act_backward_tr_img(g, ol.sv, ol.sb, acts[last], ol.sv, ol.sb, dpre_last, dl.sv, dl.sb, img_in ? cur_img : nullptr, B, s.R,
-                                        s.cout, s.act, s.zero_row, n_tr, tr_w, tr_wt, tr_S, tr_Ci, tr_Co, stream);
-            if (rc != SH_OK) return rc;
+            if (!g_is_dpre) {
+                rc = sh_act_backward_tr_img(g, ol.sv, ol.sb, acts[last], ol.sv, ol.sb, dpre_last, dl.sv, dl.sb, img_in ? cur_img : nullptr, B, s.R,
+                                            s.cout, s.act, s.zero_row, n_tr, tr_w, tr_wt, tr_S, tr_Ci, tr_Co, stream);
+                if (rc != SH_OK) return rc;
+            }
             cur = dpre_last; cl = dl;
             cur_img_done = img_in;
         } else {
diff --git a/semantichuman_amd/linear.py b/semantichuman_amd/linear.py
--- a/semantichuman_amd/linear.py
+++ b/semantichuman_amd/linear.py
@@ -7,9 +7,10 @@
 
 class _LatentLinear(torch.autograd.Function):
     @staticmethod
-    def forward(ctx, x, weight, bias):
+    def forward(ctx, x, weight, bias, link=None):
         from . import _lib
-        x = x.contiguous()
+        ctx.link = link
+        x = x.contiguous().reshape(x.shape[0], -1)
         ctx.save_for_backward(x, weight)
         ctx.has_bias = bias is not None
         ctx.mma = _lib.get_f32_mma_mode()
@@ -19,7 +20,19 @@
     def backward(ctx, dy):
         x, weight = ctx.saved_tensors
         dy = dy.contiguous()
-        dx = ops.linear_bwd_data(dy, weight, ctx.mma) if ctx.needs_input_grad[0] else None
+        link, ctx.link = ctx.link, None
+        dx = None
+        if ctx.needs_input_grad[0]:
+            last = link.last if link is not None else None
+            if last is not None and ops.linear_bwd_data_act_ok(dy.shape[0], dy.shape[1], x.shape[1], last.cout, ctx.mma):
+                dpre, img, _ = link.open(max_transposes=0)
+                ops.linear_bwd_data_act(dy, weight, x, last.act, last.zero_row, last.cout, dpre, img, ctx.mma)
+                link.exclusive = last.act != 0
+                dx = link.state[2]
+            else:
+                dx = ops.linear_bwd_data(dy, weight, ctx.mma)
+                if link is not None:
+                    dx = dx.view(dx.shape[0], last.R, last.cout)
         dW = db = None
         if ctx.needs_input_grad[1] or (ctx.has_bias and ctx.needs_input_grad[2]):
             want_bias = ctx.has_bias and ctx.needs_input_grad[2]
@@ -28,7 +41,7 @@
                 db = _fused_apply(param, dy, x, want_bias, ctx.mma)
             else:
                 dW, db = ops.linear_bwd_wgt(dy, x, want_bias=want_bias, mma=ctx.mma)
-        return dx, dW, db
+        return dx, dW, db, None
 
 
 _FUSED_UPDATE = {}
@@ -55,10 +68,10 @@
     return opt._fused_update(opt.param_groups[gi], param, dy, x, want_bias, mma)
 
 
-def latent_linear(x: torch.Tensor, weight: torch.Tensor, bias) -> torch.Tensor:
-    if x.dim() != 2:
-        raise RuntimeError("latent_linear expects a 2-D input, got %s" % (tuple(x.shape),))
-    return _LatentLinear.apply(x, weight, bias)
+def latent_linear(x: torch.Tensor, weight: torch.Tensor, bias, link=None) -> torch.Tensor:
+    if x.dim() != (2 if link is None else 3):
+        raise RuntimeError("latent_linear expects a 2-D input (3-D with a link), got %s" % (tuple(x.shape),))
+    return _LatentLinear.apply(x, weight, bias, link)
 
 
 class _LatentLinearBF16(torch.autograd.Function):
diff --git a/semantichuman_amd/losses.py b/semantichuman_amd/losses.py
--- a/semantichuman_amd/losses.py
+++ b/semantichuman_amd/losses.py
@@ -3,7 +3,12 @@
 import numpy as np
 import torch
 
+import os
+
 from . import ops
+
+FUSE_RECON_FINAL = os.environ.get("SH_FUSE_RECON_FINAL", "0").strip() == "1"
+FUSE_LOSS_DPRE = os.environ.get("SH_FUSE_LOSS_DPRE", "1").strip() != "0"
 
 
 class _L1Loss(torch.autograd.Function):
@@ -71,7 +76,13 @@
         ctx.save_for_backward(x_hat, x)
         ctx.ft, ctx.edge_w = ft, float(edge_w)
         ctx.set_materialize_grads(False)
-        total, parts = ops.recon_loss_fwd(x_hat, x, ft.faces, edge_w)
+        link = getattr(x_hat.grad_fn, "link", None) if FUSE_LOSS_DPRE else None
+        ctx.link = link if (link is not None and link.last.act == 0 and link.last.cout == 3 and link.last.R == x_hat.shape[1]) else None
+        tick = ops.ticket(ft, x.device) if FUSE_RECON_FINAL else None
+        if tick is not None:
+            total, parts = ops.recon_loss_fwd_fused(x_hat, x, ft.faces, edge_w, tick)
+        else:
+            total, parts = ops.recon_loss_fwd(x_hat, x, ft.faces, edge_w)
         ctx.mark_non_differentiable(parts)
         return total, parts
 
@@ -79,6 +90,12 @@
     def backward(ctx, g, _unused):
         x_hat, x = ctx.saved_tensors
         ft = ctx.ft
+        link, ctx.link = ctx.link, None
+        if link is not None:
+            dpre, _, tr = link.open(max_transposes=4)
+            ops.recon_loss_bwd_dpre(x_hat, x, ft.n_faces, ft.vptr, ft.vnbr, ctx.edge_w, g.contiguous(), dpre, link.last.act,
+                                    link.last.zero_row, tr or ())
+            return link.state[2], None, None, None
         return ops.recon_loss_bwd(x_hat, x, ft.n_faces, ft.vptr, ft.vnbr, ctx.edge_w, g.contiguous()), None, None, None
 
 
diff --git a/semantichuman_amd/models.py b/semantichuman_amd/models.py
--- a/semantichuman_amd/models.py
+++ b/semantichuman_amd/models.py
@@ -7,6 +7,7 @@
 import torch.nn as nn
 
 from . import _lib, mesh_ops, ops
+from . import stack as stack_mod
 from .mesh_ops import CSR
 from .linear import grouped_linear, latent_linear, latent_linear_bf16
 from .stack import ConvStep, SpmmStep, Stack, prepare_p3_frags, prepare_wfrags, run_stack, run_stack_bf16
@@ -179,7 +180,11 @@
             z = latent_linear_bf16(h.reshape(bsize, -1), self.fc_latent_enc.weight, self.fc_latent_enc.bias, torch.float32)
         else:
             h = run_stack(self._enc_stack, x, "bm", "bm", self.conv)
-            z = latent_linear(h.reshape(bsize, -1), self.fc_latent_enc.weight, self.fc_latent_enc.bias)
+            link = getattr(h.grad_fn, "link", None) if stack_mod.FUSE_FC_ACT else None
+            if link is not None:
+                z = latent_linear(h, self.fc_latent_enc.weight, self.fc_latent_enc.bias, link)
+            else:
+                z = latent_linear(h.reshape(bsize, -1), self.fc_latent_enc.weight, self.fc_latent_enc.bias)
         if VAE_flag if VAE_flag is not None else self.VAE_flag:
             self.z_mu = z[..., :self.latent_size]
             self.z_var = z[..., self.latent_size:]
diff --git a/semantichuman_amd/ops.py b/semantichuman_amd/ops.py
--- a/semantichuman_amd/ops.py
+++ b/semantichuman_amd/ops.py
@@ -309,6 +309,49 @@
     return total, parts
 
 
+def ticket(holder, device):
+    t = holder.__dict__.get("_sh_ticket")
+    if t is None or t.device != device:
+        if torch.cuda.is_current_stream_capturing():
+            return None
+        t = holder.__dict__["_sh_ticket"] = torch.zeros(1, dtype=torch.int32, device=device)
+    return t
+
+
+def recon_loss_fwd_fused(x_hat, x, faces, edge_w, tick):
+    assert x_hat.shape == x.shape and x.shape[2] == 3 and x_hat.is_contiguous() and x.is_contiguous() and x.is_cuda
+    total = torch.empty((), dtype=torch.float32, device=x.device)
+    parts = torch.empty((2,), dtype=torch.float32, device=x.device)
+    ws = torch.empty(_lib.load().sh_recon_loss_workspace() // 4, dtype=torch.float32, device=x.device)
+    check(_lib.load().sh_recon_loss_fwd_fused(ptr(x_hat), ptr(x), ptr(faces), x.shape[0], x.shape[1], faces.shape[0], float(edge_w),
+                                              ptr(total), ptr(parts), ptr(ws), ptr(tick), stream_ptr()), "sh_recon_loss_fwd_fused")
+    return total, parts
+
+
+def recon_loss_bwd_dpre(x_hat, x, n_faces, vptr, vnbr, edge_w, gscale, dpre, act, zero_row, transposes=()):
+    import ctypes
+    n = len(transposes)
+    arr = lambda vals, ct: (ct * max(1, n))(*vals)
+    check(_lib.load().sh_recon_loss_bwd_dpre(
+        ptr(x_hat), ptr(x), ptr(vptr), ptr(vnbr), x.shape[0], x.shape[1], int(n_faces), float(edge_w), ptr(gscale), ptr(dpre), int(act),
+        int(zero_row), n, arr([t[0].data_ptr() for t in transposes], ctypes.c_void_p), arr([t[1].data_ptr() for t in transposes], ctypes.c_void_p),
+        arr([t[2] for t in transposes], ctypes.c_int), arr([t[3] for t in transposes], ctypes.c_int),
+        arr([t[4] for t in transposes], ctypes.c_int), stream_ptr()), "sh_recon_loss_bwd_dpre")
+
+
+def linear_bwd_data_act_ok(M, N, K, C, mma=None):
+    return bool(_lib.load().sh_linear_bwd_data_act_ok(int(M), int(N), int(K), int(C), _lib.mma_id(mma)))
+
+
+def linear_bwd_data_act(dy, weight, y, act, zero_row, C, dpre=None, dpre_planes=None, mma=None):
+    _check2d(dy, weight)
+    M, N = dy.shape
+    K = weight.shape[1]
+    assert y.is_contiguous() and y.numel() == M * K and (dpre is not None or dpre_planes is not None)
+    check(_lib.load().sh_linear_bwd_data_act(ptr(dy), ptr(weight), ptr(y), int(act), int(zero_row), int(C), ptr(dpre), ptr(dpre_planes),
+                                             M, N, K, _lib.mma_id(mma), stream_ptr()), "sh_linear_bwd_data_act")
+
+
 def recon_loss_bwd(x_hat, x, n_faces, vptr, vnbr, edge_w, gscale):
     g = torch.empty_like(x_hat)
     check(_lib.load().sh_recon_loss_bwd(ptr(x_hat), ptr(x), ptr(vptr), ptr(vnbr), x.shape[0], x.shape[1], int(n_faces),
diff --git a/semantichuman_amd/optim.py b/semantichuman_amd/optim.py
--- a/semantichuman_amd/optim.py
+++ b/semantichuman_amd/optim.py
@@ -4,7 +4,11 @@
 
 import torch
 
-from . import _lib
+import os
+
+from . import _lib, ops
+
+FUSE_ADAM_BUMP = os.environ.get("SH_FUSE_ADAM_BUMP", "1").strip() != "0"
 
 
 class Adam(torch.optim.Optimizer):
@@ -108,7 +112,12 @@
                 W16[i], any16 = w16.data_ptr(), True
         lr = self._lr_tensor(group, params[0].device)
         b1, b2 = group["betas"]
-        if any16:
+        tick = ops.ticket(self, params[0].device) if FUSE_ADAM_BUMP else None
+        if tick is not None:
+            _lib.check(_lib.load().sh_adam_step_ticket(n, P, G, M, V, S, W16 if any16 else None, N, _lib.ptr(lr), float(b1), float(b2),
+                                                       float(group["eps"]), float(group["weight_decay"]), _lib.ptr(tick),
+                                                       _lib.stream_ptr()), "sh_adam_step_ticket")
+        elif any16:
             _lib.check(_lib.load().sh_adam_step_bf16(n, P, G, M, V, S, W16, N, _lib.ptr(lr), float(b1), float(b2), float(group["eps"]),
                                                      float(group["weight_decay"]), _lib.stream_ptr()), "sh_adam_step_bf16")
         else:
diff --git a/semantichuman_amd/stack.py b/semantichuman_amd/stack.py
--- a/semantichuman_amd/stack.py
+++ b/semantichuman_amd/stack.py
@@ -17,6 +17,68 @@
 DEBUG_POISON = os.environ.get("SH_DEBUG_POISON", "0").strip() == "1"
 _P3_GROUPED = os.environ.get("SH_P3_GROUPED", "1").strip() != "0"
 _ALIGN = 64
+FUSE_FC_ACT = os.environ.get("SH_FUSE_FC_ACT", "1").strip() != "0"
+FUSE_LOSS_DPRE = os.environ.get("SH_FUSE_LOSS_DPRE", "1").strip() != "0"
+_BWD_G_IS_DPRE, _BWD_TR_DONE = 0x100, 0x200
+
+
+class BackwardLink:
+
+    def __init__(self, stack, B, c0, mma, need_x_grad, frozen, weights, out_layout):
+        self.stack, self.B, self.c0, self.mma, self.need_x_grad = stack, B, c0, mma, need_x_grad
+        self.frozen, self.weights, self.out_layout = frozen, weights, out_layout
+        self.last = stack.steps[-1]
+        self.state = None
+        self.p3 = None
+        self.exclusive = False
+
+    def usable(self) -> bool:
+        return self.last.kind == "conv" and self.out_layout == "bm"
+
+    def writes_image(self, p3) -> bool:
+        plan = self.stack._plan(self.B, self.c0)
+        return bool(self.mma == "planes3" and p3 is not None and plan["dpl_mask"] and self.last.cout % 4 == 0 and self.last.cout > 8)
+
+    def transposes(self, acts_fp32, work, in_layout):
+        st = self.stack
+        plan = st._plan(self.B, self.c0)
+        forms = st.forms(self.B, self.c0, self.mma, in_layout, acts_fp32, self.need_x_grad) if self.p3_on else np.zeros(len(st.steps), dtype=np.int32)
+        out = []
+        for i, s in enumerate(st.steps):
+            if s.kind != "conv" or not (i > 0 or self.need_x_grad):
+                continue
+            if (forms[i] & _lib.FORM["bwd_gimg"]) and not (forms[i] & _lib.FORM["bwd_thin"]):
+                continue
+            o = int(plan["wt_off"][i]) // 4
+            out.append((self.weights[s.param], work[o:o + s.cin * s.S * s.cout], s.S, s.cin, s.cout))
+        return out
+
+    def open(self, max_transposes):
+        st, plan = self.stack, self.stack._plan(self.B, self.c0)
+        p3, in_layout = self.p3, self.in_layout
+        dev = st.device
+        last = self.last
+        work = torch.empty(max(1, plan["b_total"]), dtype=torch.float32, device=dev)
+        if DEBUG_POISON:
+            work.fill_(float("nan"))
+        self.p3_on = self.mma == "planes3" and p3 is not None
+        gimg = torch.empty(max(256, plan["gpl_total"]), dtype=torch.uint8, device=dev) if self.p3_on else None
+        o = int(plan["dpre_last_off"])
+        dpre = work[o:o + (last.R + last.n_extra) * self.B * last.cout].view(last.R + last.n_extra, self.B, last.cout)
+        img = gimg[int(plan["dpl_off"]):] if self.writes_image(p3) else None
+        acts_fp32 = 2 if (self.p3_on and p3[0] is not None and not any(self.frozen)) else 1
+        tr = self.transposes(acts_fp32, work, in_layout)
+        if len(tr) > max_transposes:
+            tr = None
+        token = dpre[:last.R].permute(1, 0, 2)
+        self.state = (work, gimg, token, tr is not None)
+        return dpre, img, tr
+
+    def match(self, g):
+        stt = self.state
+        if stt is None or g.data_ptr() != stt[2].data_ptr() or g.shape != stt[2].shape or g.stride() != stt[2].stride():
+            return None
+        return stt
 
 
 def _round(n: int) -> int:
@@ -382,16 +444,19 @@
         return out, arena, p3
 
     def native_backward(self, x, in_layout, out_layout, arena, out, g, weights, need_x_grad, need_bias, mma: str = "exact", p3=None,
-                        frozen=None):
+                        frozen=None, linked=None):
         B = x.shape[0] if in_layout == "bm" else x.shape[1]
         rows0 = x.shape[1] if in_layout == "bm" else x.shape[0]
         c0 = x.shape[2]
         plan = self._plan(B, c0)
         n = len(self.steps)
         dev = x.device
-        work = torch.empty(max(1, plan["b_total"]), dtype=torch.float32, device=dev)
-        if DEBUG_POISON:
-            work.fill_(float("nan"))
+        if linked is not None:
+            work = linked[0]
+        else:
+            work = torch.empty(max(1, plan["b_total"]), dtype=torch.float32, device=dev)
+            if DEBUG_POISON:
+                work.fill_(float("nan"))
         flat = torch.empty(max(1, plan["p_total"]), dtype=torch.float32, device=dev)
         gx = ops.alloc(B, rows0, c0, in_layout, dev) if need_x_grad else None
         acts = plan["f_off"] + np.uint64(arena.data_ptr())
@@ -413,17 +478,22 @@
             inpl[1:] = (plan["pl_off"][:n - 1] + np.uint64(p3[0].data_ptr())) * plan["in_img"][1:]
             inpl_p = inpl.ctypes.data
         if mma == "planes3" and p3 is not None:
-            gimg = torch.empty(max(256, plan["gpl_total"]), dtype=torch.uint8, device=dev)
+            gimg = linked[1] if linked is not None else torch.empty(max(256, plan["gpl_total"]), dtype=torch.uint8, device=dev)
             gpl = (plan["gpl_off"] + np.uint64(gimg.data_ptr())) * plan["gpl_mask"]
             wf = (plan["wf3t_off"] + np.uint64(p3[1].data_ptr() + p3[2])) * plan["wf3t_mask"]
             gpl_p, wf3t_p = gpl.ctypes.data, wf.ctypes.data
             if plan["dpl_mask"]:
                 dpl = ctypes.c_void_p(gimg.data_ptr() + int(plan["dpl_off"]))
+        acts_fp32 = 2 if (inpl_p is not None and not any(frozen)) else 1
+        g_p = _lib.ptr(g)
+        if linked is not None:
+            acts_fp32 |= _BWD_G_IS_DPRE | (_BWD_TR_DONE if linked[3] else 0)
+            g_p = ctypes.c_void_p(int(wbase) + 4 * plan["dpre_last_off"])
         _lib.check(_lib.load().sh_stack_backward(
-            n, self._native_steps(), _lib.ptr(x), _LAYOUT_ID[in_layout], rows0, c0, B, acts.ctypes.data, _lib.ptr(g),
+            n, self._native_steps(), _lib.ptr(x), _LAYOUT_ID[in_layout], rows0, c0, B, acts.ctypes.data, g_p,
             _LAYOUT_ID[out_layout], self._ptr_array(weights), gin.ctypes.data, ctypes.c_void_p(int(wbase) + 4 * plan["dpre_last_off"]),
             wt.ctypes.data, ws.ctypes.data, plan["ws_bytes"].ctypes.data, dW.ctypes.data, db.ctypes.data, 1 if need_x_grad else 0,
-            _lib.mma_id(mma), gpl_p, dpl, wf3t_p, inpl_p, 2 if (inpl_p is not None and not any(frozen)) else 1, _lib.stream_ptr()),
+            _lib.mma_id(mma), gpl_p, dpl, wf3t_p, inpl_p, acts_fp32, _lib.stream_ptr()),
             "sh_stack_backward")
         grads = {}
         for j, shp in enumerate(plan["shapes"]):
@@ -767,6 +837,13 @@
             out, arena, ctx.p3 = stack.native_forward(x, in_layout, out_layout, weights, biases, ctx.mma, with_backward=need or ctx.needs_input_grad[3],
                                                       frozen=ctx.frozen)
             ctx.save_for_backward(x, out, arena, *weights)
+            ctx.link = None
+            if (FUSE_FC_ACT or FUSE_LOSS_DPRE) and need:
+                B = x.shape[0] if in_layout == "bm" else x.shape[1]
+                link = BackwardLink(stack, B, x.shape[2], ctx.mma, bool(ctx.needs_input_grad[3]), ctx.frozen, weights, out_layout)
+                if link.usable():
+                    link.p3, link.in_layout = ctx.p3, in_layout
+                    ctx.link = link
             return out
         out, acts = stack.run_forward(x, in_layout, out_layout, weights, biases, keep=need)
         ctx.acts = acts[:-1]
@@ -777,12 +854,22 @@
     def backward(ctx, g):
         stack = ctx.stack
         in_layout, out_layout = ctx.layouts
-        g = g.contiguous()
+        link = getattr(ctx, "link", None)
+        linked = link.match(g) if link is not None else None
+        if link is not None:
+            if linked is None and link.state is not None and link.exclusive:
+                raise RuntimeError("semantichuman_amd: the output of this stack fed a layer that folded the stack's last activation "
+                                   "derivative into its own backward kernel, and something else contributed to the same gradient; "
+                                   "set SH_FUSE_FC_ACT=0 for such a graph")
+            link.state = link.p3 = None
+            ctx.link = None
+        if linked is None:
+            g = g.contiguous()
         need_bias = [hb and ctx.needs_input_grad[5 + 2 * j] for j, hb in enumerate(ctx.has_bias)]
         if ctx.native:
             x, out, arena, *weights = ctx.saved_tensors
             gx, grads = stack.native_backward(x, in_layout, out_layout, arena, out, g, weights, ctx.needs_input_grad[3], need_bias,
-                                              ctx.mma, ctx.p3, ctx.frozen)
+                                              ctx.mma, ctx.p3, ctx.frozen, linked)
             ctx.p3 = None
         else:
             x, out, *weights = ctx.saved_tensors
```

After: 47920 (median of 6 runs). No clear change (+0.6%).
